# SuwoongHeo/neurecon

Hardware: AMD Instinct MI355X
Metric: rays/sec (4096 rays x 128 samples, 8-layer x256 SDF MLP) (higher is better)
Workload: dtype f16x3

## Files before the change

### include/neurecon_hip.h

```cpp
#ifndef NEURECON_HIP_H
#define NEURECON_HIP_H

#include <stddef.h>
#include <stdint.h>

#ifdef __cplusplus
extern "C" {
#endif

#define NR_OK 0
#define NR_ERR_ARG (-1)
#define NR_ERR_UNSUPPORTED (-2)
#define NR_ERR_HIP (-3)
#define NR_ERR_WORKSPACE (-4)

#define NR_PREC_FP32 0
#define NR_PREC_F16X3 1

#define NR_UPSAMPLE_OFFICIAL 0
#define NR_UPSAMPLE_DIRECT_USE 1
#define NR_UPSAMPLE_DIRECT_MORE 2

int nr_version(void);
const char* nr_last_error(void);
// ... 18 lines not shown
  int D;
  int W;
  int skip;
  int multires;
  int W_geo_feat;
  int precision;
  int siren;
} NrSdfDesc;

size_t nr_sdf_packed_bytes(const NrSdfDesc* d);
int nr_sdf_pack(const NrSdfDesc* d, const float* const* W, const float* const* b, void* packed, void* stream);
size_t nr_mlp_workspace_bytes(int with_backward);
int nr_sdf_forward(const NrSdfDesc* d, const void* packed, const float* pts, int64_t P, float* sdf, float* nabla,
                   float* feature, void* workspace, size_t workspace_bytes, void* stream);

typedef struct {
  int D;
  int W;
  int multires;
  int multires_view;
  int W_geo_feat;
  int precision;
  int no_view_dirs;
  int siren;
} NrRadDesc;

size_t nr_radiance_packed_bytes(const NrRadDesc* d);
int nr_radiance_pack(const NrRadDesc* d, const float* const* W, const float* const* b, void* packed, void* stream);
int nr_radiance_forward(const NrRadDesc* d, const void* packed, const float* x, const float* vdir, int64_t vdir_div,
                        const float* normals, const float* feature, int64_t P, float* rgb, void* stream);

typedef struct {
  const float* rays_o;
  const float* rays_d;
  int64_t n_rays;
  const NrSdfDesc* sdf;
  const void* sdf_packed;
  const NrRadDesc* rad;
  const void* rad_packed;
  float s;
  float obj_bounding_radius;
  float near_bypass;
  float far_bypass;
  int N_samples;
  int N_importance;
  int N_upsample_iters;
  int calc_normal;
  int white_bkgd;
  const float* t_coarse;
  const float* u_fine;
  float* rgb;
  float* depth;
  float* acc;
  float* normals;
  float* d_final;
  float* sdf_out;
  float* nablas_out;
  float* radiance_out;
  float* alpha_out;
  float* cdf_out;
  float* weights_out;
  const NrNerfDesc* nerf;
  const void* nerf_packed;
  int N_outside;
  const float* t_outside;
  float* sigma_out;
  float* radiance_bg_out;
  int upsample_algo;
  float fixed_s;
  int N_nograd_samples;
  const float* t_nograd;
  void* workspace;
  size_t workspace_bytes;
  const float* u_rand;
  const float* t_out_rand;
  const float* s_dev;
  int sample_only;
  float* d_all_out;
  int no_mid_skip;
  int no_defer;
  int64_t max_chunk_rays;
  size_t max_workspace_bytes;
  const void* fold_packed;
} NrNeusArgs;

#define NR_DEFAULT_WORKSPACE_BYTES ((size_t)4 << 30)
#define NR_MIN_CHUNK_RAYS 4096

size_t nr_neus_workspace_bytes(const NrNeusArgs* a);
int nr_neus_render(const NrNeusArgs* a, void* stream);

size_t nr_neus_fold_packed_bytes(const NrSdfDesc* sdf, const NrRadDesc* rad);
int nr_neus_fold_pack(const NrSdfDesc* sdf, const NrRadDesc* rad, const float* W8, const float* b8, const float* W0,
                      const float* b0, void* packed, void* stream);
int nr_neus_fold_forward(const NrSdfDesc* sdf, const void* sdf_packed, const NrRadDesc* rad, const void* rad_packed,
                         const void* fold_packed, const float* pts, const float* vdir, int64_t vdir_div,
                         const float* normals, int64_t P, float* u, float* sdf_out, float* rgb, void* stream);

typedef struct {
  const float* rays_o;
  const float* rays_d;
  int64_t n_rays;
  const NrSdfDesc* sdf;
  const void* sdf_packed;
  const NrRadDesc* rad;
  const void* rad_packed;
  float alpha_net, beta_net;
  float beta_plus_init;
  float eps;
  float near, far;
  float obj_bounding_radius;
  int use_sphere_bg;
  int N_samples, N_importance, max_upsample_steps, max_bisection_steps;
  int calc_normal, white_bkgd;
  const float* t_coarse;
  const float* t_init;
  const float* u_up;
  const float* u_fine;
  float* rgb;
  float* depth;
  float* acc;
  float* normals;
  float* d_vals;
  float* sdf_out;
  float* nablas_out;
  float* radiance_out;
  float* alpha_out;
  float* p_out;
  float* weights_out;
  float* sigma_out;
  float* beta_map;
  float* iter_usage;
  void* workspace;
  size_t workspace_bytes;
  int N_outside;
  const NrNerfDesc* nerf;
  const void* nerf_packed;
  const float* rs_out;
  float beta_plus_k;
  float* sigma_bg;
  float* radiance_bg;
  const float* u_rand;
  const float* u_out;
} NrVolsdfArgs;

size_t nr_volsdf_workspace_bytes(const NrVolsdfArgs* a);
int nr_volsdf_render(const NrVolsdfArgs* a, void* stream);

typedef struct {
  const float* rays_o;
  const float* rays_d;
  int64_t n_rays;
  int64_t rays_per_batch;
  const NrSdfDesc* sdf;
  const void* sdf_packed;
  const NrRadDesc* rad;
  const void* rad_packed;
  float logit_tau;
  float radius_of_interest;
  float interval;
  float too_close_threshold;
  float near_bypass, far_bypass;
  int N_steps, N_secant_steps, N_query, N_freespace;
  int normal_mode;
  int64_t rayschunk, netchunk;
  int calc_normal, white_bkgd;
  const float* t_march;
  const float* t_query;
  const float* t_free;
  float* rgb;
  float* depth;
  float* acc;
  float* normals;
  float* surface_points;
  uint8_t* mask_surface;
  float* depth_surface;
  float* radiance_out;
  float* sdf_out;
  float* nablas_out;
  float* alpha_out;
  float* weights_out;
  void* workspace;
  size_t workspace_bytes;
  const float* u_query;
  const float* u_free;
  int64_t shard_ray0;
  int64_t shard_row_rays;
  double* window_ss;
  int (*window_reduce)(void* user);
  void* window_user;
  int no_secant;
  float* d_all_out;
  int sample_only;
  int full_march;
} NrUnisurfArgs;

size_t nr_unisurf_workspace_bytes(const NrUnisurfArgs* a);
int nr_unisurf_render(const NrUnisurfArgs* a, void* stream);
int64_t nr_unisurf_window_count(const NrUnisurfArgs* a);

int nr_sample_pdf(const float* bins, const float* weights, int64_t R, int L, const float* u, int64_t u_stride, int N,
                  float* out, void* stream);

int nr_get_rays(const float* c2w, const float* K, int B, int H, int W, const int64_t* select_inds, int64_t N,
                float* rays_o, float* rays_d, void* stream);
int nr_gather_rows(const void* src, int64_t B, int64_t HW, int64_t row_bytes, const int64_t* idx, int64_t N, void* out,
                   void* stream);

size_t nr_sphere_trace_workspace_bytes(int64_t n_rays);
int nr_sphere_trace(const NrSdfDesc* d, const void* packed, const float* rays_o, const float* rays_d, int64_t n_rays,
                    float near, float far, const float* near_rays, const float* far_rays, int n_iters, float* d_pred,
                    float* pts, uint8_t* mask, void* workspace, size_t workspace_bytes, void* stream);
size_t nr_root_find_workspace_bytes(int64_t n_rays, int N_steps);
int nr_root_find(const NrSdfDesc* d, const void* packed, const float* rays_o, const float* rays_d, int64_t n_rays,
                 float near, float far, const float* near_rays, const float* far_rays, int N_steps,
                 const float* t_march, int N_secant_steps, int no_secant, float logit_tau, int fill_inf,
                 int full_march, float* d_pred, float* pts, uint8_t* mask, uint8_t* mask_sign_change, void* workspace,
                 size_t workspace_bytes, void* stream);
int nr_normalize3(const float* v, int64_t n, float* out, void* stream);
int nr_surface_finish(float* rgb, const float* nablas, const uint8_t* mask, int64_t n, float* normals, void* stream);

size_t nr_sdf_grid_workspace_bytes(int64_t n_points);
int nr_sdf_grid(const NrSdfDesc* d, const void* packed, double volume_size, int64_t N, int64_t i0, int64_t n,
                float* sdf, void* workspace, size_t workspace_bytes, void* stream);

int nr_mc_table(int8_t* tri, int32_t* counts);
size_t nr_mc_workspace_bytes(int64_t n0, int64_t n1, int64_t n2);
int nr_mc_count(const float* volume, int64_t n0, int64_t n1, int64_t n2, float level, void* workspace,
                size_t workspace_bytes, int64_t* totals, void* stream);
int nr_mc_emit(const float* volume, int64_t n0, int64_t n1, int64_t n2, float level, const double* spacing,
               const double* origin, double scale, const double* offset, void* workspace, size_t workspace_bytes,
               int64_t n_verts, int64_t n_faces, float* verts, int64_t verts_cap, int32_t* faces, int64_t faces_cap,
               void* stream);

size_t nr_mesh_workspace_bytes(int64_t V, int64_t F);
int nr_mesh_components(const int32_t* faces, int64_t F, int64_t V, int32_t* labels, int32_t* face_count,
                       int64_t* totals, void* workspace, size_t workspace_bytes, void* stream);
int nr_mesh_filter_count(const int32_t* faces, int64_t F, int64_t V, const uint8_t* vkeep, void* workspace,
                         size_t workspace_bytes, int64_t* totals, void* stream);
int nr_mesh_filter_emit(const int32_t* faces, int64_t F, int64_t V, const uint8_t* vkeep, void* workspace,
                        size_t workspace_bytes, int64_t Vk, int64_t Fk, int32_t* vsrc, int64_t vsrc_cap,
                        int32_t* faces_out, int64_t faces_cap, void* stream);

int nr_embed(const float* x, int64_t P, int nfreq, float* out, void* stream);
int nr_embed_jvp(const float* x, const float* v, int64_t P, int nfreq, float* out, void* stream);
int nr_embed_padded(const float* x, int64_t P, int nfreq, float* out, int ldo, void* stream);
int nr_embed_jvp_padded(const float* x, const float* v, int64_t P, int nfreq, float* out, int ldo, void* stream);
int nr_embed_vjp(const float* x, const float* e0, int ld0, const float* e1, int ld1, float s1, int64_t P, int nfreq,
                 float* out, void* stream);
int nr_softplus100(const float* z, int64_t n, float* h, float* s, void* stream);
int nr_scale_cols(const float* a, int64_t P, int lda, int col0, int ncols, const float* s, float scale, float* out,
                  void* stream);
int nr_softplus_adjoint(const float* hbar, int ldh, const float* s, const float* g, const float* zdot, int64_t P,
                        int n, float* zbar, void* stream);
size_t nr_colsum_workspace_bytes(int n);
int nr_colsum(const float* a, int64_t P, int n, float* out, void* workspace, size_t workspace_bytes, void* stream);
int nr_sine30(const float* z, int64_t n, float* h, float* s, void* stream);
int nr_sine_adjoint(const float* hbar, int ldh, const float* s, const float* h, const float* g, const float* zdot,
                    int64_t P, int n, float* zbar, void* stream);
int nr_mul(const float* a, const float* b, int64_t n, float* out, void* stream);
int nr_activation(float* y, float* g, int64_t n, int mode, void* stream);
#define NR_WN_MAX 16
typedef struct {
  const float* v;
  const float* g;
  float* w;
  float* norm;
  const float* grad_w;
  float* grad_v;
  float* grad_g;
  int rows;
  int cols;
} NrWnLayer;
int nr_weight_norm_fwd(const NrWnLayer* layers, int n, void* stream);
int nr_weight_norm_bwd(const NrWnLayer* layers, int n, void* stream);
#define NR_ADAM_MAX 64
typedef struct {
// ... 186 lines not shown
```

### neurecon_amd/_lib.py

```python
import ctypes
import os
import threading

import torch

HERE = os.path.dirname(os.path.abspath(__file__))
LIB_PATH = os.environ.get('NR_LIB', os.path.join(HERE, 'libnrhip.so'))

PREC_FP32 = 0
PREC_F16X3 = 1
UPSAMPLE = {'official_solution': 0, 'direct_use': 1, 'direct_more': 2}

_c_p = ctypes.c_void_p
_c_i = ctypes.c_int
_c_i64 = ctypes.c_int64
_c_f = ctypes.c_float
_c_d = ctypes.c_double
_c_sz = ctypes.c_size_t


class NrSdfDesc(ctypes.Structure):
    _fields_ = [('D', _c_i), ('W', _c_i), ('skip', _c_i), ('multires', _c_i), ('W_geo_feat', _c_i),
                ('precision', _c_i), ('siren', _c_i)]


class NrRadDesc(ctypes.Structure):
    _fields_ = [('D', _c_i), ('W', _c_i), ('multires', _c_i), ('multires_view', _c_i), ('W_geo_feat', _c_i),
                ('precision', _c_i), ('no_view_dirs', _c_i), ('siren', _c_i)]


class NrNerfDesc(ctypes.Structure):
    _fields_ = [('D', _c_i), ('W', _c_i), ('skip', _c_i), ('input_ch', _c_i), ('multires', _c_i),
                ('multires_view', _c_i), ('precision', _c_i)]


class NrNeusArgs(ctypes.Structure):
    _fields_ = [
        ('rays_o', _c_p), ('rays_d', _c_p), ('n_rays', _c_i64),
        ('sdf', ctypes.POINTER(NrSdfDesc)), ('sdf_packed', _c_p),
        ('rad', ctypes.POINTER(NrRadDesc)), ('rad_packed', _c_p),
        ('s', _c_f), ('obj_bounding_radius', _c_f), ('near_bypass', _c_f), ('far_bypass', _c_f),
        ('N_samples', _c_i), ('N_importance', _c_i), ('N_upsample_iters', _c_i), ('calc_normal', _c_i),
        ('white_bkgd', _c_i),
        ('t_coarse', _c_p), ('u_fine', _c_p),
        ('rgb', _c_p), ('depth', _c_p), ('acc', _c_p), ('normals', _c_p),
        ('d_final', _c_p), ('sdf_out', _c_p), ('nablas_out', _c_p), ('radiance_out', _c_p),
        ('alpha_out', _c_p), ('cdf_out', _c_p), ('weights_out', _c_p),
        ('nerf', ctypes.POINTER(NrNerfDesc)), ('nerf_packed', _c_p), ('N_outside', _c_i), ('t_outside', _c_p),
        ('sigma_out', _c_p), ('radiance_bg_out', _c_p),
        ('upsample_algo', _c_i), ('fixed_s', _c_f), ('N_nograd_samples', _c_i), ('t_nograd', _c_p),
        ('workspace', _c_p), ('workspace_bytes', _c_sz),
        ('u_rand', _c_p), ('t_out_rand', _c_p), ('s_dev', _c_p), ('sample_only', _c_i), ('d_all_out', _c_p),
        ('no_mid_skip', _c_i), ('no_defer', _c_i), ('max_chunk_rays', _c_i64), ('max_workspace_bytes', _c_sz),
        ('fold_packed', _c_p),
    ]


class NrVolsdfArgs(ctypes.Structure):
    _fields_ = [
        ('rays_o', _c_p), ('rays_d', _c_p), ('n_rays', _c_i64),
        ('sdf', ctypes.POINTER(NrSdfDesc)), ('sdf_packed', _c_p),
        ('rad', ctypes.POINTER(NrRadDesc)), ('rad_packed', _c_p),
        ('alpha_net', _c_f), ('beta_net', _c_f), ('beta_plus_init', _c_f), ('eps', _c_f),
        ('near', _c_f), ('far', _c_f), ('obj_bounding_radius', _c_f), ('use_sphere_bg', _c_i),
        ('N_samples', _c_i), ('N_importance', _c_i), ('max_upsample_steps', _c_i), ('max_bisection_steps', _c_i),
        ('calc_normal', _c_i), ('white_bkgd', _c_i),
        ('t_coarse', _c_p), ('t_init', _c_p), ('u_up', _c_p), ('u_fine', _c_p),
        ('rgb', _c_p), ('depth', _c_p), ('acc', _c_p), ('normals', _c_p),
        ('d_vals', _c_p), ('sdf_out', _c_p), ('nablas_out', _c_p), ('radiance_out', _c_p),
        ('alpha_out', _c_p), ('p_out', _c_p), ('weights_out', _c_p), ('sigma_out', _c_p),
        ('beta_map', _c_p), ('iter_usage', _c_p),
        ('workspace', _c_p), ('workspace_bytes', _c_sz),
        ('N_outside', _c_i), ('nerf', ctypes.POINTER(NrNerfDesc)), ('nerf_packed', _c_p), ('rs_out', _c_p),
        ('beta_plus_k', _c_f), ('sigma_bg', _c_p), ('radiance_bg', _c_p), ('u_rand', _c_p), ('u_out', _c_p),
    ]


class NrUnisurfArgs(ctypes.Structure):
    _fields_ = [
        ('rays_o', _c_p), ('rays_d', _c_p), ('n_rays', _c_i64), ('rays_per_batch', _c_i64),
        ('sdf', ctypes.POINTER(NrSdfDesc)), ('sdf_packed', _c_p),
        ('rad', ctypes.POINTER(NrRadDesc)), ('rad_packed', _c_p),
        ('logit_tau', _c_f), ('radius_of_interest', _c_f), ('interval', _c_f), ('too_close_threshold', _c_f),
        ('near_bypass', _c_f), ('far_bypass', _c_f),
        ('N_steps', _c_i), ('N_secant_steps', _c_i), ('N_query', _c_i), ('N_freespace', _c_i),
        ('normal_mode', _c_i), ('rayschunk', _c_i64), ('netchunk', _c_i64),
        ('calc_normal', _c_i), ('white_bkgd', _c_i),
        ('t_march', _c_p), ('t_query', _c_p), ('t_free', _c_p),
        ('rgb', _c_p), ('depth', _c_p), ('acc', _c_p), ('normals', _c_p),
        ('surface_points', _c_p), ('mask_surface', _c_p), ('depth_surface', _c_p),
        ('radiance_out', _c_p), ('sdf_out', _c_p), ('nablas_out', _c_p), ('alpha_out', _c_p), ('weights_out', _c_p),
        ('workspace', _c_p), ('workspace_bytes', _c_sz),
        ('u_query', _c_p), ('u_free', _c_p),
        ('shard_ray0', _c_i64), ('shard_row_rays', _c_i64), ('window_ss', _c_p), ('window_reduce', _c_p),
        ('window_user', _c_p), ('no_secant', _c_i), ('d_all_out', _c_p), ('sample_only', _c_i),
        ('full_march', _c_i),
    ]


WINDOW_REDUCE = ctypes.CFUNCTYPE(_c_i, _c_p)

TG_NONE, TG_SOFTPLUS, TG_MUL, TG_SPADJ, TG_RELUMASK = 0, 1, 3, 4, 5
BLK_X1, BLK_X2, BLK_Y, BLK_YB, BLK_Y2, BLK_Y3, BLK_A, BLK_G, BLK_ZD = 1, 2, 4, 8, 16, 32, 64, 128, 256
WG_BLK_A0, WG_BLK_A1, WG_BLK_B0, WG_BLK_B1 = 1, 2, 4, 8
WN_MAX = 16
ADAM_MAX = 64


class NrTrainGemm(ctypes.Structure):
    _fields_ = [
        ('op', _c_p), ('P', _c_i64),
        ('x1', _c_p), ('ld1', _c_i64), ('n1', _c_i),
        ('x2', _c_p), ('ld2', _c_i64), ('n2', _c_i),
        ('use_bias', _c_i), ('mode', _c_i), ('yscale', _c_f),
        ('y', _c_p), ('ldy', _c_i64), ('yb', _c_p), ('ldyb', _c_i64),
        ('y2', _c_p), ('ldy2', _c_i64), ('y3', _c_p), ('ldy3', _c_i64),
        ('a', _c_p), ('lda', _c_i64), ('g', _c_p), ('ldg', _c_i64), ('zd', _c_p), ('ldzd', _c_i64),
        ('g_row', _c_i), ('dot', _c_p), ('dot_bias', _c_f),
        ('head', _c_p), ('head_bias', _c_p), ('head_out', _c_p), ('blocked', _c_i),
        ('g_scaled', _c_i),
    ]


class NrWgrad(ctypes.Structure):
    _fields_ = [
        ('P', _c_i64), ('npairs', _c_i), ('a', _c_p * 2), ('lda', _c_i64 * 2), ('b', _c_p * 2), ('ldb', _c_i64 * 2),
        ('m', _c_i), ('n', _c_i), ('scale', _c_f), ('c', _c_p), ('ldc', _c_i64), ('colsum', _c_p),
        ('avec', _c_p), ('ldv', _c_i64), ('vec', _c_p), ('vec_scale', _c_f), ('workspace', _c_p),
        ('workspace_bytes', _c_sz), ('blocked', _c_i), ('fp32', _c_i),
    ]


class NrWnLayer(ctypes.Structure):
    _fields_ = [('v', _c_p), ('g', _c_p), ('w', _c_p), ('norm', _c_p), ('grad_w', _c_p), ('grad_v', _c_p),
                ('grad_g', _c_p), ('rows', _c_i), ('cols', _c_i)]


class NrAdamTensor(ctypes.Structure):
    _fields_ = [('param', _c_p), ('grad', _c_p), ('exp_avg', _c_p), ('exp_avg_sq', _c_p), ('n', _c_i64)]


class NrKernelStat(ctypes.Structure):
    _fields_ = [('name', ctypes.c_char * 32), ('launches', _c_i64), ('ms', ctypes.c_double),
                ('units', ctypes.c_double)]


_SIGS = {
    'nr_version': (_c_i, []),
    'nr_last_error': (ctypes.c_char_p, []),
    'nr_build_id': (ctypes.c_char_p, []),
    'nr_sdf_packed_bytes': (_c_sz, [ctypes.POINTER(NrSdfDesc)]),
    'nr_sdf_pack': (_c_i, [ctypes.POINTER(NrSdfDesc), ctypes.POINTER(_c_p), ctypes.POINTER(_c_p), _c_p, _c_p]),
    'nr_mlp_workspace_bytes': (_c_sz, [_c_i]),
    'nr_sdf_forward': (_c_i, [ctypes.POINTER(NrSdfDesc), _c_p, _c_p, _c_i64, _c_p, _c_p, _c_p, _c_p, _c_sz, _c_p]),
    'nr_radiance_packed_bytes': (_c_sz, [ctypes.POINTER(NrRadDesc)]),
    'nr_radiance_pack': (_c_i, [ctypes.POINTER(NrRadDesc), ctypes.POINTER(_c_p), ctypes.POINTER(_c_p), _c_p, _c_p]),
    'nr_radiance_forward': (_c_i, [ctypes.POINTER(NrRadDesc), _c_p, _c_p, _c_p, _c_i64, _c_p, _c_p, _c_i64, _c_p,
                                   _c_p]),
    'nr_nerf_packed_bytes': (_c_sz, [ctypes.POINTER(NrNerfDesc)]),
    'nr_nerf_pack': (_c_i, [ctypes.POINTER(NrNerfDesc), ctypes.POINTER(_c_p), ctypes.POINTER(_c_p), _c_p, _c_p]),
    'nr_nerf_forward': (_c_i, [ctypes.POINTER(NrNerfDesc), _c_p, _c_p, _c_p, _c_i64, _c_i64, _c_p, _c_p, _c_p]),
    'nr_nerf_train_fwd32': (_c_i, [ctypes.POINTER(NrNerfDesc), _c_p, _c_p, _c_p, _c_i64, ctypes.POINTER(_c_p), _c_p,
                                   _c_p, _c_p, _c_p, _c_p]),
    'nr_nerf_train_packed_bytes': (_c_sz, [ctypes.POINTER(NrNerfDesc)]),
    'nr_weight_norm_fwd': (_c_i, [ctypes.POINTER(NrWnLayer), _c_i, _c_p]),
    'nr_weight_norm_bwd': (_c_i, [ctypes.POINTER(NrWnLayer), _c_i, _c_p]),
    'nr_adam_step': (_c_i, [ctypes.POINTER(NrAdamTensor), _c_i, _c_i64, _c_d, _c_d, _c_d, _c_d, _c_d, _c_p]),
    'nr_nerf_train_pack': (_c_i, [ctypes.POINTER(NrNerfDesc), ctypes.POINTER(_c_p), ctypes.POINTER(_c_p), _c_p, _c_p]),
    'nr_nerf_train_bwd32': (_c_i, [ctypes.POINTER(NrNerfDesc), _c_p, _c_p, _c_p, ctypes.POINTER(_c_p), _c_p, _c_p,
                                   _c_i64, _c_p, _c_p, _c_p, ctypes.POINTER(_c_p), _c_p]),
    'nr_neus_workspace_bytes': (_c_sz, [ctypes.POINTER(NrNeusArgs)]),
    'nr_neus_render': (_c_i, [ctypes.POINTER(NrNeusArgs), _c_p]),
    'nr_neus_fold_packed_bytes': (_c_sz, [ctypes.POINTER(NrSdfDesc), ctypes.POINTER(NrRadDesc)]),
    'nr_neus_fold_pack': (_c_i, [ctypes.POINTER(NrSdfDesc), ctypes.POINTER(NrRadDesc), _c_p, _c_p, _c_p, _c_p, _c_p,
                                 _c_p]),
    'nr_neus_fold_forward': (_c_i, [ctypes.POINTER(NrSdfDesc), _c_p, ctypes.POINTER(NrRadDesc), _c_p, _c_p, _c_p, _c_p,
                                    _c_i64, _c_p, _c_i64, _c_p, _c_p, _c_p, _c_p]),
    'nr_volsdf_workspace_bytes': (_c_sz, [ctypes.POINTER(NrVolsdfArgs)]),
    'nr_volsdf_render': (_c_i, [ctypes.POINTER(NrVolsdfArgs), _c_p]),
    'nr_unisurf_workspace_bytes': (_c_sz, [ctypes.POINTER(NrUnisurfArgs)]),
    'nr_unisurf_render': (_c_i, [ctypes.POINTER(NrUnisurfArgs), _c_p]),
    'nr_unisurf_window_count': (_c_i64, [ctypes.POINTER(NrUnisurfArgs)]),
    'nr_sample_pdf': (_c_i, [_c_p, _c_p, _c_i64, _c_i, _c_p, _c_i64, _c_i, _c_p, _c_p]),
    'nr_get_rays': (_c_i, [_c_p, _c_p, _c_i, _c_i, _c_i, _c_p, _c_i64, _c_p, _c_p, _c_p]),
    'nr_gather_rows': (_c_i, [_c_p, _c_i64, _c_i64, _c_i64, _c_p, _c_i64, _c_p, _c_p]),
    'nr_sphere_trace_workspace_bytes': (_c_sz, [_c_i64]),
    'nr_sphere_trace': (_c_i, [ctypes.POINTER(NrSdfDesc), _c_p, _c_p, _c_p, _c_i64, ctypes.c_float, ctypes.c_float,
                               _c_p, _c_p, _c_i, _c_p, _c_p, _c_p, _c_p, _c_sz, _c_p]),
    'nr_radiance_train_fwd32': (_c_i, [ctypes.POINTER(NrRadDesc), _c_p, _c_p, _c_p, _c_i64, _c_i64, _c_p, _c_p, _c_p,
                                        _c_p, _c_p, _c_p]),
    'nr_root_find_workspace_bytes': (_c_sz, [_c_i64, _c_i]),
    'nr_root_find': (_c_i, [ctypes.POINTER(NrSdfDesc), _c_p, _c_p, _c_p, _c_i64, ctypes.c_float, ctypes.c_float, _c_p,
                            _c_p, _c_i, _c_p, _c_i, _c_i, ctypes.c_float, _c_i, _c_i, _c_p, _c_p, _c_p, _c_p, _c_p,
                            _c_sz, _c_p]),
    'nr_normalize3': (_c_i, [_c_p, _c_i64, _c_p, _c_p]),
    'nr_surface_finish': (_c_i, [_c_p, _c_p, _c_p, _c_i64, _c_p, _c_p]),
    'nr_sdf_grid_workspace_bytes': (_c_sz, [_c_i64]),
    'nr_sdf_grid': (_c_i, [ctypes.POINTER(NrSdfDesc), _c_p, ctypes.c_double, _c_i64, _c_i64, _c_i64, _c_p, _c_p,
                           _c_sz, _c_p]),
    'nr_mc_table': (_c_i, [_c_p, _c_p]),
    'nr_mc_workspace_bytes': (_c_sz, [_c_i64, _c_i64, _c_i64]),
    'nr_mc_count': (_c_i, [_c_p, _c_i64, _c_i64, _c_i64, _c_f, _c_p, _c_sz, _c_p, _c_p]),
    'nr_mc_emit': (_c_i, [_c_p, _c_i64, _c_i64, _c_i64, _c_f, ctypes.POINTER(_c_d), ctypes.POINTER(_c_d), _c_d,
                          ctypes.POINTER(_c_d), _c_p, _c_sz, _c_i64, _c_i64, _c_p, _c_i64, _c_p, _c_i64, _c_p]),
    'nr_mesh_workspace_bytes': (_c_sz, [_c_i64, _c_i64]),
    'nr_mesh_components': (_c_i, [_c_p, _c_i64, _c_i64, _c_p, _c_p, _c_p, _c_p, _c_sz, _c_p]),
    'nr_mesh_filter_count': (_c_i, [_c_p, _c_i64, _c_i64, _c_p, _c_p, _c_sz, _c_p, _c_p]),
    'nr_mesh_filter_emit': (_c_i, [_c_p, _c_i64, _c_i64, _c_p, _c_p, _c_sz, _c_i64, _c_i64, _c_p, _c_i64, _c_p,
                                   _c_i64, _c_p]),
    'nr_embed': (_c_i, [_c_p, _c_i64, _c_i, _c_p, _c_p]),
    'nr_embed_jvp': (_c_i, [_c_p, _c_p, _c_i64, _c_i, _c_p, _c_p]),
    'nr_embed_vjp': (_c_i, [_c_p, _c_p, _c_i, _c_p, _c_i, _c_f, _c_i64, _c_i, _c_p, _c_p]),
    'nr_embed_padded': (_c_i, [_c_p, _c_i64, _c_i, _c_p, _c_i, _c_p]),
    'nr_embed_jvp_padded': (_c_i, [_c_p, _c_p, _c_i64, _c_i, _c_p, _c_i, _c_p]),
    'nr_train_gemm': (_c_i, [ctypes.POINTER(NrTrainGemm), _c_i, _c_i, _c_i, _c_i, _c_p]),
    'nr_sdf_op_info': (_c_i, [ctypes.POINTER(NrSdfDesc), _c_i, ctypes.POINTER(_c_i64), ctypes.POINTER(_c_i),
                              ctypes.POINTER(_c_i)]),
    'nr_sdf_train_packed_bytes': (_c_sz, [ctypes.POINTER(NrSdfDesc)]),
    'nr_sdf_train_pack': (_c_i, [ctypes.POINTER(NrSdfDesc), ctypes.POINTER(_c_p), ctypes.POINTER(_c_p), _c_p, _c_p]),
    'nr_radiance_op_info': (_c_i, [ctypes.POINTER(NrRadDesc), _c_i, ctypes.POINTER(_c_i64), ctypes.POINTER(_c_i),
                                   ctypes.POINTER(_c_i)]),
    'nr_radiance_train_packed_bytes': (_c_sz, [ctypes.POINTER(NrRadDesc)]),
    'nr_radiance_train_pack': (_c_i, [ctypes.POINTER(NrRadDesc), ctypes.POINTER(_c_p), ctypes.POINTER(_c_p), _c_p,
                                      _c_p]),
    'nr_softplus100': (_c_i, [_c_p, _c_i64, _c_p, _c_p, _c_p]),
    'nr_scale_cols': (_c_i, [_c_p, _c_i64, _c_i, _c_i, _c_i, _c_p, _c_f, _c_p, _c_p]),
    'nr_softplus_adjoint': (_c_i, [_c_p, _c_i, _c_p, _c_p, _c_p, _c_i64, _c_i, _c_p, _c_p]),
    'nr_colsum_workspace_bytes': (_c_sz, [_c_i]),
    'nr_colsum': (_c_i, [_c_p, _c_i64, _c_i, _c_p, _c_p, _c_sz, _c_p]),
    'nr_sine30': (_c_i, [_c_p, _c_i64, _c_p, _c_p, _c_p]),
    'nr_sine_adjoint': (_c_i, [_c_p, _c_i, _c_p, _c_p, _c_p, _c_p, _c_i64, _c_i, _c_p, _c_p]),
    'nr_mul': (_c_i, [_c_p, _c_p, _c_i64, _c_p, _c_p]),
    'nr_activation': (_c_i, [_c_p, _c_p, _c_i64, _c_i, _c_p]),
    'nr_radiance_input': (_c_i, [_c_p, _c_p, _c_p, _c_p, _c_i64, _c_i, _c_i, _c_i, _c_p, _c_p]),
    'nr_neus_points': (_c_i, [_c_p, _c_p, _c_p, _c_i64, _c_i, _c_p, _c_p, _c_p, _c_p]),
    'nr_neus_composite_fwd': (_c_i, [_c_p, _c_p, _c_p, _c_p, _c_i64, _c_i, _c_i, _c_p, _c_p, _c_p, _c_p, _c_p, _c_p,
                                     _c_p]),
    'nr_neus_composite_bwd_workspace_bytes': (_c_sz, [_c_i64, _c_i]),
    'nr_neus_composite_bwd': (_c_i, [_c_p, _c_p, _c_p, _c_p, _c_i64, _c_i, _c_i, _c_p, _c_p, _c_p, _c_p, _c_p, _c_p,
                                     _c_p, _c_p, _c_sz, _c_p]),
    'nr_nerf_train_input': (_c_i, [_c_p, _c_p, _c_p, _c_i64, _c_i, _c_i, ctypes.c_float, _c_p, _c_p, _c_p, _c_p]),
    'nr_neus_composite_bg_fwd': (_c_i, [_c_p, _c_p, _c_p, _c_p, _c_p, _c_p, _c_p, _c_i64, _c_i, _c_i, _c_i, _c_p, _c_p,
                                        _c_p, _c_p, _c_p, _c_p, _c_p]),
    'nr_neus_composite_bg_bwd_workspace_bytes': (_c_sz, [_c_i64, _c_i, _c_i]),
    'nr_neus_composite_bg_bwd': (_c_i, [_c_p, _c_p, _c_p, _c_p, _c_p, _c_p, _c_p, _c_i64, _c_i, _c_i, _c_i, _c_p, _c_p,
                                        _c_p, _c_p, _c_p, _c_p, _c_p, _c_p, _c_p, _c_p, _c_sz, _c_p]),
    'nr_unisurf_composite_fwd': (_c_i, [_c_p, _c_p, _c_p, _c_i64, _c_i, _c_i, _c_p, _c_p, _c_p, _c_p, _c_p, _c_p]),
    'nr_unisurf_composite_bwd_workspace_bytes': (_c_sz, [_c_i64, _c_i]),
    'nr_unisurf_composite_bwd': (_c_i, [_c_p, _c_p, _c_p, _c_i64, _c_i, _c_i, _c_p, _c_p, _c_p, _c_p, _c_p, _c_p, _c_p,
                                        _c_sz, _c_p]),
    'nr_volsdf_composite_bg_fwd': (_c_i, [_c_p, _c_p, _c_p, _c_p, _c_p, _c_i64, _c_i, _c_i, _c_f, _c_i, _c_p, _c_p,
                                          _c_p, _c_i, _c_p, _c_p, _c_p, _c_p, _c_p, _c_p, _c_p, _c_p]),
    'nr_volsdf_composite_bg_bwd_workspace_bytes': (_c_sz, [_c_i64, _c_i, _c_i]),
    'nr_volsdf_composite_bg_bwd': (_c_i, [_c_p, _c_p, _c_p, _c_p, _c_p, _c_i64, _c_i, _c_i, _c_f, _c_i, _c_p, _c_p,
                                          _c_p, _c_i, _c_p, _c_p, _c_p, _c_p, _c_p, _c_p, _c_p, _c_p, _c_p, _c_p, _c_p,
                                          _c_sz, _c_p]),
    'nr_volsdf_nerf_input': (_c_i, [_c_p, _c_p, _c_p, _c_p, _c_i64, _c_i, _c_p, _c_p, _c_p]),
    'nr_volsdf_composite_fwd': (_c_i, [_c_p, _c_p, _c_p, _c_p, _c_p, _c_i64, _c_i, _c_i, _c_f, _c_i, _c_p, _c_p, _c_p,
                                       _c_p, _c_p, _c_p, _c_p, _c_p]),
    'nr_volsdf_composite_bwd_workspace_bytes': (_c_sz, [_c_i64, _c_i]),
# ... 96 lines not shown
```

### neurecon_amd/csrc/nr_capi.hip

```cpp
#include <algorithm>
#include <cmath>
#include <cstring>
#include <string>

#include "nr_common.h"
#include <cstdlib>
#include "nr_mlp.h"
#include "nr_tgemm.h"
#include "nr_neus.h"
#include "nr_volsdf.h"
#include "nr_unisurf.h"

namespace nr {

static thread_local std::string g_err;
void set_error(const std::string& msg) { g_err = msg; }

static size_t align256(size_t x) { return (x + 255) & ~(size_t)255; }
static int64_t chunk_bytes_host(int KB) { return (int64_t)(2 * KB + 1) * 1024; }

int check_sdf_desc(const NrSdfDesc* d) {
  NR_REQUIRE(d, NR_ERR_ARG, "null NrSdfDesc");
  if (d->siren) {
    NR_REQUIRE(d->D == 5 && d->W == 256 && d->skip < 0 && d->multires < 0 && d->W_geo_feat == 256,
// ... 11 lines not shown
  return NR_OK;
}

int check_rad_desc(const NrRadDesc* d) {
  NR_REQUIRE(d, NR_ERR_ARG, "null NrRadDesc");
  NR_REQUIRE((d->D == 4 || d->D == 5) && d->W == 256 && d->multires < 0 && d->W_geo_feat == 256 &&
                 d->multires_view <= 7,
             NR_ERR_UNSUPPORTED,
             "radiance net: only D=4 or 5, W=256, embed_multires=-1, embed_multires_view<=7, W_geo_feat=256");
  NR_REQUIRE(d->precision == NR_PREC_FP32 || d->precision == NR_PREC_F16X3, NR_ERR_UNSUPPORTED,
             "radiance net: unknown precision mode");
  return NR_OK;
}


SdfLayout sdf_layout(const NrSdfDesc& d) {
  SdfLayout L{};
  L.prec = d.precision;
  L.siren = d.siren ? 1 : 0;
  const int nops = L.siren ? kSirenOps : kSdfOps;
  const int* KB = L.siren ? kSirenKB : kSdfKB;
  const int* NBO = L.siren ? kSirenNBO : kSdfNBO;
  size_t off = 0;
  for (int i = 0; i < nops; ++i) {
    L.op_bytes[i] = (2 * KB[i] + 1) * 1024;
    L.op_off[i] = (uint32_t)off;
    off += (size_t)(NBO[i] / 2) * L.op_bytes[i];
  }
  static_assert(sdf_op_off(kSdfOps - 1) + (kSdfNBO[kSdfOps - 1] / 2) * (2 * kSdfKB[kSdfOps - 1] + 1) * 1024 > 0, "");
  L.scale_off = (uint32_t)off;
  off = align256(off + kSdfOps * 4);
  L.bound_off = (uint32_t)off;
  off = align256(off + kSdfOps * 8);
  L.w8row0_off = (uint32_t)off;
  off = align256(off + 256 * 4);
  L.misc_off = (uint32_t)off;
  off = align256(off + 16);
  L.total = (uint32_t)off;
  return L;
}

static int rad_small(const NrRadDesc& d) {
  return d.no_view_dirs ? 3 : 3 + (d.multires_view < 0 ? 3 : 3 + 6 * d.multires_view) + 3;
}

RadLayout rad_layout(const NrRadDesc& d) {
  RadLayout L{};
  L.prec = d.precision;
  L.n_small = rad_small(d);
  L.view = d.no_view_dirs ? 0 : 1;
  L.D = d.D;
  L.siren = d.siren ? 1 : 0;
  L.kbs = L.n_small <= 32 ? 2 : 4;
  size_t off = 0;
  for (int i = 0; i < L.D; ++i) {
    const int kb = i == 0 ? 16 + L.kbs : 16;
    L.op_bytes[i] = (2 * kb + 1) * 1024;
    L.op_off[i] = (uint32_t)off;
    off += 8 * (size_t)L.op_bytes[i];
  }
  L.scale_off = (uint32_t)off;
  off = align256(off + 5 * 4);
  L.bound_off = (uint32_t)off;
  off = align256(off + 5 * 2 * 4);
  L.head_off = (uint32_t)off;
  off = align256(off + (3 * 256 + 4) * 4);
  L.total = (uint32_t)off;
  return L;
}

bool fold_applies(const NrSdfDesc& sd, const NrRadDesc& rd) {
  return sd.precision == NR_PREC_F16X3 && !sd.siren && sd.W_geo_feat == 256 && rd.precision == NR_PREC_F16X3 &&
         !rd.siren && rd.D == 4 && rd.W_geo_feat == 256;
}

FoldLayout fold_layout(const RadLayout& RL) {
  FoldLayout F{};
  F.kbs = RL.kbs;
  size_t off = 0;
  F.f8_off = (uint32_t)off;
  off += 8 * (size_t)chunk_bytes_host(16);
  F.r0_off = (uint32_t)off;
  off += 8 * (size_t)chunk_bytes_host(RL.kbs);
  F.scale_off = (uint32_t)off;
  off = align256(off + 2 * 4);
  F.bound_off = (uint32_t)off;
  off = align256(off + 2 * 2 * 4);
  F.u_off = (uint32_t)off;
  off = align256(off + (256 * 256 + 256) * 4);
  F.total = (uint32_t)off;
  return F;
}

int check_nerf_desc(const NrNerfDesc* d) {
  NR_REQUIRE(d, NR_ERR_ARG, "null NrNerfDesc");
  NR_REQUIRE(d->D == 8 && d->W == 256 && d->skip == 4 && d->input_ch == 4 && d->multires == 10 &&
                 d->multires_view == 4,
             NR_ERR_UNSUPPORTED,
             "NeRF net: only the NeRF++ background configuration (D=8, W=256, skips=[4], input_ch=4, "
             "multires=10, multires_view=4, use_view_dirs) is implemented");
  NR_REQUIRE(d->precision == NR_PREC_FP32 || d->precision == NR_PREC_F16X3, NR_ERR_UNSUPPORTED,
             "NeRF net: unknown precision mode");
  return NR_OK;
}

static const int kNerfKB[kNerfOps] = {6, 16, 16, 16, 16, 22, 16, 16, 16, 18};
static const int kNerfNBO[kNerfOps] = {16, 16, 16, 16, 16, 16, 16, 16, 16, 8};

static int nerf_nbo(int i, int prec) { return (i == NF && prec == NR_PREC_F16X3) ? 18 : kNerfNBO[i]; }

NerfLayout nerf_layout(const NrNerfDesc& d) {
  NerfLayout L{};
  L.prec = d.precision;
  size_t off = 0;
  for (int i = 0; i < kNerfOps; ++i) {
    L.op_bytes[i] = (2 * kNerfKB[i] + 1) * 1024;
    L.op_off[i] = (uint32_t)off;
    off += (size_t)(nerf_nbo(i, d.precision) / 2) * L.op_bytes[i];
  }
  L.scale_off = (uint32_t)off;
  off = align256(off + kNerfOps * 4);
  L.bound_off = (uint32_t)off;
  off = align256(off + kNerfOps * 2 * 4);
  L.alpha_off = (uint32_t)off;
  off = align256(off + 257 * 4);
  L.rgb_off = (uint32_t)off;
  off = align256(off + (3 * 128 + 3) * 4);
  L.total = (uint32_t)off;
  return L;
}

static PackSeg seg(int nblk, int off, int nvalid) { return PackSeg{nblk, off, nvalid}; }
static PackOp mkop(const float* W, const float* bias, int rows, int ld, int tr, PackSeg o0, PackSeg o1, PackSeg i0,
                   PackSeg i1, float scale, int prec, float* wmax) {
  PackOp op{};
  op.W = W; op.bias = bias; op.wn = (int64_t)rows * ld; op.ld = ld; op.transpose = tr;
  op.out[0] = o0; op.out[1] = o1; op.in[0] = i0; op.in[1] = i1;
  op.scale = scale; op.prec = prec; op.wmax = wmax;
  return op;
}
static PackSeg none() { return PackSeg{0, 0, 0}; }

static size_t scratch_bytes() {
  int dev = 0, cus = 256;
  if (hipGetDevice(&dev) == hipSuccess) (void)hipDeviceGetAttribute(&cus, hipDeviceAttributeMultiprocessorCount, dev);
  return (size_t)cus * kScratchPerWG;
}

static int neus_chunk(const NrNeusArgs& a, const NeusPlan& pl, int64_t ray0, int R, hipStream_t st) {
  char* ws = (char*)a.workspace;
  const bool direct = a.upsample_algo != NR_UPSAMPLE_OFFICIAL;
  const int n_up = direct ? 0 : (a.N_upsample_iters > 0 ? a.N_importance / a.N_upsample_iters : 0);
  NeusChunk c{};
  c.R = R;
  c.N_samples = a.N_samples;
  c.n_up = n_up;
  c.n_iters = direct ? 0 : a.N_upsample_iters;
  c.S = direct ? a.N_samples + a.N_importance : a.N_samples + a.N_upsample_iters * n_up;
  c.n_imp = a.N_importance;
  c.n_nog = a.upsample_algo == NR_UPSAMPLE_DIRECT_MORE ? a.N_nograd_samples : 0;
  c.fixed_s = a.fixed_s;
  c.t_nog = a.t_nograd;
  auto F = [&](size_t o) { return (float*)(ws + o); };
  c.ro = F(pl.o_ro); c.rd = F(pl.o_rd); c.near = F(pl.o_near); c.far = F(pl.o_far);
  c.dv = F(pl.o_dv); c.sv = F(pl.o_sv); c.wtmp = F(pl.o_wtmp); c.dnew = F(pl.o_dnew); c.snew = F(pl.o_snew);
  c.pts = F(pl.o_pts); c.mids = F(pl.o_mids); c.dmid = F(pl.o_dmid);
  c.sdf_f = F(pl.o_sdf_f); c.nab_f = F(pl.o_nab_f);
  c.sdf_m = F(pl.o_sdf_m); c.nab_m = F(pl.o_nab_m); c.feat_m = F(pl.o_feat_m); c.rad_m = F(pl.o_rad_m);
  c.N_out = a.N_outside;
  c.r_obj = a.obj_bounding_radius;
  c.t_out = a.t_outside;
  c.d_out = F(pl.o_dout); c.x4 = F(pl.o_x4); c.sig_o = F(pl.o_sigo); c.rad_o = F(pl.o_rado);
// ... 41 lines not shown
    if ((rc = launch_sdf(SL, a.sdf_packed, c.pts_nog, (int64_t)c.n_nog * R, c.s_nog, nullptr, nullptr,
                         a.sdf->multires, nullptr, 0, st)))
      return rc;
  }
  if (direct) {
    ProfScope prof("neus_upsample", (double)R, st);
    const float* u = a.u_rand ? a.u_rand + ray0 * a.N_importance : a.u_fine;
    hipLaunchKernelGGL(neus_direct_upsample, grd, blk, 0, st, c, (int)(a.upsample_algo == NR_UPSAMPLE_DIRECT_MORE), u,
                       (int64_t)(a.u_rand ? a.N_importance : 0));
  }
  NR_HIP_CHECK(hipGetLastError());
  float* dvb[2] = {c.dv, F(pl.o_dv2)};
  float* svb[2] = {c.sv, F(pl.o_sv2)};
  int* idb[2] = {c.idv, fused ? (int*)(ws + pl.o_idv2) : nullptr};
  int cur = 0;
  auto merge = [&](int L) -> int {
    ProfScope prof("neus_merge", (double)R, st);
    const int64_t nt = (int64_t)(L + n_up) * R;
    hipLaunchKernelGGL(neus_merge, dim3((unsigned)((nt + 255) / 256)), dim3(256), 0, st, c, L, dvb[cur ^ 1],
                       svb[cur ^ 1], idb[cur ^ 1]);
    cur ^= 1;
    c.dv = dvb[cur];
    c.sv = svb[cur];
    c.idv = idb[cur];
    if (fused) c.sdf_f = c.sv;
    NR_HIP_CHECK(hipGetLastError());
    return NR_OK;
  };
  for (int it = 0; it < c.n_iters; ++it) {
    if (it > 0 && (rc = merge(a.N_samples + (it - 1) * n_up))) return rc;
    const int64_t slot0 = (int64_t)(a.N_samples + it * n_up) * R;
    NeusChunk cu = c;
    if (defer) cu.pts = c.pts + slot0 * 3;
    {
      ProfScope prof("neus_upsample", (double)R, st);
      const float* u = a.u_rand ? a.u_rand + ((int64_t)it * a.n_rays + ray0) * n_up : a.u_fine;
      const size_t lds1 = (5 * (size_t)c.S + 1) * sizeof(float);
      if (4 * lds1 <= 65536)
        hipLaunchKernelGGL((neus_upsample<4>), dim3((unsigned)((R + 3) / 4)), dim3(64), 4 * lds1, st, cu, it, u,
                           (int64_t)(a.u_rand ? n_up : 0));
      else
        hipLaunchKernelGGL((neus_upsample<1>), dim3((unsigned)R), dim3(64), lds1, st, cu, it, u,
                           (int64_t)(a.u_rand ? n_up : 0));
    }
    NR_HIP_CHECK(hipGetLastError());
    if ((rc = sample_sdf(cu.pts, (int64_t)n_up * R, c.snew, slot0))) return rc;
  }
  if (c.n_iters > 0 && (rc = merge(c.S - n_up))) return rc;
  if (defer) {
    const int64_t nslot = (int64_t)c.S * R;
    c.tshift = 0;
    NR_HIP_CHECK(hipMemsetAsync(c.nraw, 0, (size_t)nslot * 3 * sizeof(float), st));
    if (a.calc_normal && a.N_outside == 0) {
      NR_HIP_CHECK(hipMemsetAsync(c.tflag, 0, (size_t)nslot * sizeof(int), st));
      NR_HIP_CHECK(hipMemsetAsync(c.tcnt, 0, sizeof(int), st));
      const int64_t nq = (int64_t)(c.S - 1) * R;
      hipLaunchKernelGGL(neus_sample_need, dim3((unsigned)((nq + 255) / 256)), dim3(256), 0, st, c, a.s_dev, a.s);
      NR_HIP_CHECK(hipGetLastError());
      hipLaunchKernelGGL(neus_point_list, dim3((unsigned)((nslot + 1023) / 1024)), dim3(1024), 0, st, c, nslot);
      NR_HIP_CHECK(hipGetLastError());
      if ((rc = launch_sdf_deferred(SL, a.sdf_packed, c.pts, nslot, nullptr, c.nraw, a.sdf->multires, c.slabs, c.tiles,
                                    c.tcnt, 4, st)))
        return rc;
    }
  }
  if (a.sample_only) {
    hipLaunchKernelGGL(neus_write_dall, dim3((unsigned)(((int64_t)c.S * R + 255) / 256)), dim3(256), 0, st, c.dv,
                       (int64_t)R, c.S, ray0, a.d_all_out);
    NR_HIP_CHECK(hipGetLastError());
    return NR_OK;
  }
  {
    ProfScope prof("neus_points", (double)R, st);
    hipLaunchKernelGGL(neus_expand, dim3((unsigned)(((int64_t)c.S * R + 255) / 256)), dim3(256), 0, st, c,
                       (int)!(defer && a.N_outside > 0));
  }
  NR_HIP_CHECK(hipGetLastError());
  if (!fused && (rc = launch_sdf(SL, a.sdf_packed, c.pts, (int64_t)c.S * R, c.sdf_f, c.nab_f, nullptr,
                                 a.sdf->multires, mlp_ws, mlp_bytes, st)))
    return rc;
  const int64_t Pm = (int64_t)(c.S - 1) * R;
  const char* f8p = nullptr;
  const char* r0p = nullptr;
  if (a.fold_packed) {
    const FoldLayout FL = fold_layout(RL);
    f8p = (const char*)a.fold_packed + FL.f8_off;
    r0p = (const char*)a.fold_packed + FL.r0_off;
  }
  if (a.radiance_out || a.no_mid_skip) {
    if ((rc = launch_sdf(SL, a.sdf_packed, c.mids, Pm, c.sdf_m, c.nab_m, c.feat_m, a.sdf->multires, mlp_ws, mlp_bytes,
                         st, nullptr, 0, f8p)))
      return rc;
    if ((rc = launch_radiance(RL, a.rad_packed, c.mids, c.rd, 1, R, c.nab_m, c.feat_m, Pm, c.rad_m,
                              a.rad->multires_view, st, nullptr, r0p)))
      return rc;
  } else {
    char* wsb = (char*)a.workspace;
    int* cnt = (int*)(wsb + pl.o_mcnt);
    int* slot = (int*)(wsb + pl.o_mslot);
    float* midc = (float*)(wsb + pl.o_midc);
    float* vdc = (float*)(wsb + pl.o_mvd);
    float* radc = (float*)(wsb + pl.o_mrad);
    NR_HIP_CHECK(hipMemsetAsync(cnt, 0, sizeof(int), st));
    const dim3 g1((unsigned)((Pm + 255) / 256));
    hipLaunchKernelGGL(neus_mid_compact, dim3((unsigned)((Pm + 1023) / 1024)), dim3(1024), 0, st, c, a.s_dev, a.s, cnt,
                       slot, midc, vdc);
    NR_HIP_CHECK(hipGetLastError());
    if ((rc = launch_sdf(SL, a.sdf_packed, midc, Pm, c.sdf_m, c.nab_m, c.feat_m, a.sdf->multires, mlp_ws, mlp_bytes,
                         st, cnt, 1, f8p)))
      return rc;
    if ((rc = launch_radiance(RL, a.rad_packed, midc, vdc, 1, INT64_MAX, c.nab_m, c.feat_m, Pm, radc,
                              a.rad->multires_view, st, cnt, r0p)))
      return rc;
    hipLaunchKernelGGL(neus_mid_scatter, g1, dim3(256), 0, st, slot, radc, Pm, c.rad_m);
    NR_HIP_CHECK(hipGetLastError());
  }
  NeusOut o{ray0, a.rgb, a.depth, a.acc, a.normals, a.d_final, a.sdf_out, a.nablas_out,
            a.radiance_out, a.alpha_out, a.cdf_out, a.weights_out, a.sigma_out, a.radiance_bg_out};
  if (a.N_outside > 0) {
    hipLaunchKernelGGL(neus_outside_points, grd, blk, 0, st, c,
                       a.t_out_rand ? a.t_out_rand + ray0 * a.N_outside : (const float*)nullptr);
    NR_HIP_CHECK(hipGetLastError());
    const int64_t Po = (int64_t)(c.S - 1 + a.N_outside) * R;
    if (a.sigma_out || a.radiance_bg_out) {
      if ((rc = launch_nerf(nerf_layout(*a.nerf), a.nerf_packed, c.x4, c.rd, 1, R, Po, c.sig_o, c.rad_o, st)))
        return rc;
    } else {
      char* wsb = (char*)a.workspace;
      int* cnt = (int*)(wsb + pl.o_cnt);
      int* slot = (int*)(wsb + pl.o_slot);
      float* x4c = (float*)(wsb + pl.o_x4c);
      float* vdc = (float*)(wsb + pl.o_vdc);
      float* sigc = (float*)(wsb + pl.o_sigc);
      float* radc = (float*)(wsb + pl.o_radc);
      NR_HIP_CHECK(hipMemsetAsync(cnt, 0, sizeof(int), st));
      const dim3 g1((unsigned)((Po + 255) / 256));
      hipLaunchKernelGGL(neus_outside_compact, dim3((unsigned)((Po + 1023) / 1024)), dim3(1024), 0, st, c, cnt, slot,
                         x4c, vdc);
      NR_HIP_CHECK(hipGetLastError());
      if ((rc = launch_nerf(nerf_layout(*a.nerf), a.nerf_packed, x4c, vdc, 1, INT64_MAX, Po, sigc, radc, st, cnt)))
        return rc;
      hipLaunchKernelGGL(neus_outside_scatter, g1, dim3(256), 0, st, slot, sigc, radc, Po, c.sig_o, c.rad_o);
      NR_HIP_CHECK(hipGetLastError());
    }
    if (defer) {
      const int64_t nslot = (int64_t)c.S * R;
      c.tshift = 0;
      if (a.calc_normal) {
        NR_HIP_CHECK(hipMemsetAsync(c.tflag, 0, (size_t)nslot * sizeof(int), st));
        NR_HIP_CHECK(hipMemsetAsync(c.tcnt, 0, sizeof(int), st));
        hipLaunchKernelGGL(neus_sample_need_outside, dim3((unsigned)((nslot + 255) / 256)), dim3(256), 0, st, c,
                           a.s_dev, a.s);
        NR_HIP_CHECK(hipGetLastError());
        hipLaunchKernelGGL(neus_point_list, dim3((unsigned)((nslot + 1023) / 1024)), dim3(1024), 0, st, c, nslot);
        NR_HIP_CHECK(hipGetLastError());
        if ((rc = launch_sdf_deferred(SL, a.sdf_packed, c.pts, nslot, nullptr, c.nraw, a.sdf->multires, c.slabs,
                                      c.tiles, c.tcnt, 4, st)))
          return rc;
      }
      hipLaunchKernelGGL(neus_gather_nablas, dim3((unsigned)((nslot + 255) / 256)), dim3(256), 0, st, c);
      NR_HIP_CHECK(hipGetLastError());
    }
    ProfScope prof("neus_composite", (double)R, st);
    const int M = c.S - 1 + a.N_outside;
    const size_t lds1 = (6 * (size_t)M + 4 * (size_t)c.S) * sizeof(float);
    if (4 * lds1 <= 65536)
      hipLaunchKernelGGL((neus_composite_outside_w<4>), dim3((unsigned)((R + 3) / 4)), dim3(64), 4 * lds1, st, c, o,
                         a.s_dev, a.s, a.calc_normal, a.white_bkgd);
    else if (lds1 <= 65536)
      hipLaunchKernelGGL((neus_composite_outside_w<1>), dim3((unsigned)R), dim3(64), lds1, st, c, o, a.s_dev, a.s,
                         a.calc_normal, a.white_bkgd);
    else
      hipLaunchKernelGGL(neus_composite_outside, grd, blk, 0, st, c, o, a.s_dev, a.s, a.calc_normal, a.white_bkgd);
  } else {
    ProfScope prof("neus_composite", (double)R, st);
    const size_t lds1 = 9 * (size_t)c.S * sizeof(float);
    if (4 * lds1 <= 65536)
      hipLaunchKernelGGL((neus_composite<4>), dim3((unsigned)((R + 3) / 4)), dim3(64), 4 * lds1, st, c, o, a.s_dev, a.s,
                         a.calc_normal, a.white_bkgd);
    else
      hipLaunchKernelGGL((neus_composite<1>), dim3((unsigned)R), dim3(64), lds1, st, c, o, a.s_dev, a.s, a.calc_normal,
                         a.white_bkgd);
  }
  NR_HIP_CHECK(hipGetLastError());
  return NR_OK;
}

static int64_t neus_chunk_rays(const NrNeusArgs* a) {
  const int64_t n = a->n_rays > 0 ? a->n_rays : 1;
  int64_t cap = 16384;
  if (a->max_chunk_rays > 0)
    cap = std::min(cap, a->max_workspace_bytes ? a->max_chunk_rays : std::max<int64_t>(a->max_chunk_rays, NR_MIN_CHUNK_RAYS));
  const size_t budget = a->max_workspace_bytes ? a->max_workspace_bytes : NR_DEFAULT_WORKSPACE_BYTES;
  const bool defer = neus_deferred(*a, 16);
  NrNeusArgs q = *a;
  const size_t t1 = neus_plan(q, 1024).total, t2 = neus_plan(q, 2048).total;
  const size_t per_ray = (t2 - t1) / 1024 + 1, fixed = t1 > 1024 * per_ray ? t1 - 1024 * per_ray : 0;
  const int64_t fit = budget > fixed ? (int64_t)((budget - fixed) / per_ray) : 0;
  cap = std::min(cap, std::max<int64_t>(fit, 16));
  if (defer && n > 16 && n % 16) cap = std::min(cap, n / 16 * 16);
  if (n <= cap) return n;
  if (defer && cap >= 16) cap = cap / 16 * 16;
  return std::max<int64_t>(cap, 1);
}

static int volsdf_chunk(const NrVolsdfArgs& a, const VolPlan& pl, int64_t ray0, int R, hipStream_t st) {
  char* ws = (char*)a.workspace;
  auto F = [&](size_t o) { return (float*)(ws + o); };
  VolChunk c{};
  c.R = R;
  c.N0 = 4 * a.N_samples;
  c.N_up = 4 * a.N_samples;
  c.cap = c.N0 + a.max_upsample_steps * c.N_up;
  c.N_samples = a.N_samples;
  c.N_imp = a.N_importance;
  c.S = a.N_samples + a.N_importance;
  c.max_iter = a.max_upsample_steps;
  c.max_bisect = a.max_bisection_steps;
  c.alpha_net = a.alpha_net;
  c.beta_net = a.beta_net;
  c.beta_plus0 = a.beta_plus_init;
  c.eps = a.eps;
  c.near = a.near;
  c.far = a.far;
  c.r_bg = a.obj_bounding_radius;
  c.use_bg = a.use_sphere_bg;
  c.ro = F(pl.o_ro); c.rd = F(pl.o_rd);
  c.Ld[0] = F(pl.o_Ld0); c.Ld[1] = F(pl.o_Ld1); c.Ls[0] = F(pl.o_Ls0); c.Ls[1] = F(pl.o_Ls1);
  c.dnew[0] = F(pl.o_dn0); c.dnew[1] = F(pl.o_dn1);
  c.pts = F(pl.o_pts); c.sraw = F(pl.o_sraw);
  c.act[0] = (int*)(ws + pl.o_act0); c.act[1] = (int*)(ws + pl.o_act1); c.cnt = (int*)(ws + pl.o_cnt);
  c.beta = F(pl.o_beta); c.fine = F(pl.o_fine); c.usage = F(pl.o_usage); c.bmap = F(pl.o_bmap);
  c.d_all = F(pl.o_dall); c.pts_f = F(pl.o_ptsf); c.sdf_f = F(pl.o_sdff); c.nab_f = F(pl.o_nabf);
  c.feat_f = F(pl.o_featf); c.rad_f = F(pl.o_radf);
  c.t_coarse = a.t_coarse; c.t_init = a.t_init; c.u_up = a.u_up; c.u_fine = a.u_fine;
  c.N_out = a.N_outside > 0 ? a.N_outside : 0;
  c.u_rand = a.u_rand ? a.u_rand + ray0 * a.N_importance : nullptr;
  c.u_out = a.u_out && c.N_out > 0 ? a.u_out + ray0 * c.N_out : nullptr;
  c.beta_k = a.beta_plus_k;
  c.farr = F(pl.o_farr); c.bp0 = F(pl.o_bp0); c.rs_out = a.rs_out; c.d_out = F(pl.o_dout);
  c.x4 = F(pl.o_x4); c.sig_o = F(pl.o_sigo); c.rad_o = F(pl.o_rado);
  void* mlp_ws = ws + pl.o_mlp;
  const size_t mlp_bytes = a.workspace_bytes - pl.o_mlp;
  const SdfLayout SL = sdf_layout(*a.sdf);
  const RadLayout RL = rad_layout(*a.rad);
  const unsigned lds = (unsigned)pl.lds_bytes;
  const dim3 blk(64), grd((unsigned)R);
  int rc;
  NR_HIP_CHECK(hipMemsetAsync(c.cnt, 0, sizeof(int) * (a.max_upsample_steps + 1), st));
  {
    ProfScope prof("volsdf_prologue", (double)R, st);
    hipLaunchKernelGGL(volsdf_prologue, grd, blk, 0, st, c, a.rays_o + ray0 * 3, a.rays_d + ray0 * 3);
  }
  NR_HIP_CHECK(hipGetLastError());
  if ((rc = launch_sdf(SL, a.sdf_packed, c.pts, (int64_t)c.N0 * R, c.sraw, nullptr, nullptr, a.sdf->multires,
                       nullptr, 0, st)))
    return rc;
  {
    ProfScope prof("volsdf_first", (double)R, st);
    hipLaunchKernelGGL(volsdf_first, grd, blk, lds, st, c);
  }
  NR_HIP_CHECK(hipGetLastError());
  for (int it = 1; it <= a.max_upsample_steps; ++it) {
    if ((rc = launch_sdf(SL, a.sdf_packed, c.pts, (int64_t)c.N_up * R, c.sraw, nullptr, nullptr, a.sdf->multires,
                         nullptr, 0, st, c.cnt + (it - 1), c.N_up)))
      return rc;
    {
      ProfScope prof("volsdf_iter", (double)R, st);
      hipLaunchKernelGGL(volsdf_iter, grd, blk, lds, st, c, it);
    }
    NR_HIP_CHECK(hipGetLastError());
  }
  {
    ProfScope prof("volsdf_points", (double)R, st);
    hipLaunchKernelGGL(volsdf_points, grd, blk, lds, st, c);
  }
  NR_HIP_CHECK(hipGetLastError());
  const int64_t P = (int64_t)c.S * R;
  if ((rc = launch_sdf(SL, a.sdf_packed, c.pts_f, P, c.sdf_f, c.nab_f, c.feat_f, a.sdf->multires, mlp_ws, mlp_bytes,
                       st)))
    return rc;
  if ((rc = launch_radiance(RL, a.rad_packed, c.pts_f, c.rd, c.S, INT64_MAX, c.nab_f, c.feat_f, P, c.rad_f,
                            a.rad->multires_view, st)))
    return rc;
  if (c.N_out > 0) {
    {
      ProfScope prof("volsdf_outside", (double)R, st);
      hipLaunchKernelGGL(volsdf_outside, grd, blk, 0, st, c);
    }
    NR_HIP_CHECK(hipGetLastError());
    if ((rc = launch_nerf(nerf_layout(*a.nerf), a.nerf_packed, c.x4, c.rd, c.N_out, INT64_MAX,
                          (int64_t)c.N_out * R, c.sig_o, c.rad_o, st)))
      return rc;
  }
  VolOut o{ray0, a.rgb, a.depth, a.acc, a.normals, a.d_vals, a.sdf_out, a.nablas_out, a.radiance_out,
           a.alpha_out, a.p_out, a.weights_out, a.sigma_out, a.beta_map, a.iter_usage, a.sigma_bg, a.radiance_bg};
  {
    ProfScope prof("volsdf_composite", (double)R, st);
    hipLaunchKernelGGL(volsdf_composite, grd, blk, lds, st, c, o, a.calc_normal, a.white_bkgd);
  }
  NR_HIP_CHECK(hipGetLastError());
  return NR_OK;
}

static int64_t volsdf_chunk_rays(const NrVolsdfArgs* a) {
  const int64_t cap = 16384;
  return a->n_rays < cap ? (a->n_rays > 0 ? a->n_rays : 1) : cap;
}

static int check_volsdf(const NrVolsdfArgs* a) {
  NR_REQUIRE(a, NR_ERR_ARG, "nr_volsdf_render: null args");
  int rc = check_sdf_desc(a->sdf);
  if (rc) return rc;
  if ((rc = check_rad_desc(a->rad))) return rc;
  NR_REQUIRE(a->n_rays <= 0 || (a->rays_o && a->rays_d && a->rgb && a->depth && a->acc), NR_ERR_ARG,
             "nr_volsdf_render: null ray or output pointer");
  NR_REQUIRE(a->sdf_packed && a->rad_packed && a->t_coarse && a->t_init && a->u_up && a->u_fine, NR_ERR_ARG,
             "nr_volsdf_render: null argument");
  NR_REQUIRE(a->n_rays <= 0 || !a->calc_normal || a->normals, NR_ERR_ARG,
             "nr_volsdf_render: calc_normal needs normals output");
  NR_REQUIRE(a->N_samples >= 1 && a->N_importance >= 1 && a->max_upsample_steps >= 0 && a->max_bisection_steps >= 0,
             NR_ERR_ARG, "nr_volsdf_render: bad sample counts");
  NR_REQUIRE(4 * a->N_samples <= 1024 && a->N_importance <= 1024, NR_ERR_UNSUPPORTED,
             "nr_volsdf_render: 4*N_samples and N_importance must be <= 1024");
  NR_REQUIRE(a->beta_net > 0.f && (a->N_outside > 0 || a->beta_plus_init > 0.f), NR_ERR_ARG,
             "nr_volsdf_render: beta must be positive");
  if (a->N_outside > 0) {
    NR_REQUIRE(!a->use_sphere_bg, NR_ERR_ARG, "nr_volsdf_render: NeRF++ background excludes the builtin sphere");
    NR_REQUIRE(a->nerf && a->nerf_packed && a->rs_out && a->beta_plus_k > 0.f, NR_ERR_ARG,
               "nr_volsdf_render: N_outside > 0 needs nerf, nerf_packed, rs_out and beta_plus_k");
    if ((rc = check_nerf_desc(a->nerf))) return rc;
  }
  return NR_OK;
}

static int unisurf_chunk(const NrUnisurfArgs& a, const UniPlan& pl, int64_t ray0, int R, int64_t row_ray0, int nloc,
                         hipStream_t st) {
  char* ws = (char*)a.workspace;
  auto F = [&](size_t o) { return (float*)(ws + o); };
  UniChunk c{};
  c.R = R;
  c.N_steps = a.N_steps;
  c.N_query = a.N_query;
  c.N_free = a.N_freespace;
  c.P = a.N_query + a.N_freespace;
  c.logit_tau = a.logit_tau;
  c.interval = a.interval;
  c.too_close = a.too_close_threshold;
  c.near_bypass = a.near_bypass;
  c.far_bypass = a.far_bypass;
  c.r_interest = a.radius_of_interest;
  c.ro = F(pl.o_ro); c.rd = F(pl.o_rd); c.near = F(pl.o_near); c.far = F(pl.o_far); c.thr = F(pl.o_thr);
  c.pts_m = F(pl.o_ptsm); c.sm = F(pl.o_sm); c.sec = F(pl.o_sec); c.pts_s = F(pl.o_ptss); c.ss = F(pl.o_ss);
  c.d_all = F(pl.o_dall); c.pts_f = F(pl.o_ptsf); c.sdf_f = F(pl.o_sdff); c.nab_f = F(pl.o_nabf);
  c.feat_f = F(pl.o_featf); c.nrm_f = F(pl.o_nrmf); c.rad_f = F(pl.o_radf); c.wss = (double*)(ws + pl.o_wss);
  c.wsp = (double*)(ws + pl.o_wsp);
  c.netchunk = a.netchunk;
  const bool sharded = a.normal_mode == 1 && a.shard_row_rays > 0;
  if (a.normal_mode == 1) {
    unisurf_windows(a, c.rc_rays, c.nw_full, c.nw_row);
    c.row_rays = sharded ? a.shard_row_rays : (a.rays_per_batch > 0 ? a.rays_per_batch : a.n_rays);
    c.row_ray0 = row_ray0;
    c.nloc = nloc;
    if (sharded) c.wss = a.window_ss;
  }
  c.t_march = a.t_march; c.t_query = a.t_query; c.t_free = a.t_free;
  c.no_secant = a.no_secant;
  c.u_q = a.u_query ? a.u_query + ray0 * a.N_query : nullptr;
  c.u_f = a.u_free ? a.u_free + ray0 * a.N_freespace : nullptr;
  void* mlp_ws = ws + pl.o_mlp;
  const size_t mlp_bytes = a.workspace_bytes - pl.o_mlp;
  const SdfLayout SL = sdf_layout(*a.sdf);
  const RadLayout RL = rad_layout(*a.rad);
  const dim3 blk(64), grd((R + 63) / 64);
  const int64_t P = (int64_t)c.P * R;
  int rc;
  {
    ProfScope prof("unisurf_prologue", (double)R, st);
    hipLaunchKernelGGL(uni_prologue, grd, blk, 0, st, c, a.rays_o + ray0 * 3, a.rays_d + ray0 * 3);
  }
  NR_HIP_CHECK(hipGetLastError());
  if ((rc = run_march(SL, a.sdf_packed, a.sdf->multires, c, a.full_march != 0, (int*)(ws + pl.o_act0),
                      (int*)(ws + pl.o_act1), (int*)(ws + pl.o_acnt), F(pl.o_ptsc), F(pl.o_sc), st)))
    return rc;
  hipLaunchKernelGGL(uni_root, grd, blk, 0, st, c);
  NR_HIP_CHECK(hipGetLastError());
  for (int i = 0; i < (a.no_secant ? 0 : a.N_secant_steps); ++i) {
    if ((rc = launch_sdf(SL, a.sdf_packed, c.pts_s, R, c.ss, nullptr, nullptr, a.sdf->multires, nullptr, 0, st)))
      return rc;
    hipLaunchKernelGGL(uni_secant, grd, blk, 0, st, c, (int)(i == a.N_secant_steps - 1));
    NR_HIP_CHECK(hipGetLastError());
  }
  UniOut o{ray0, a.rgb, a.depth, a.acc, a.normals, a.surface_points, a.mask_surface, a.depth_surface,
           a.radiance_out, a.sdf_out, a.nablas_out, a.alpha_out, a.weights_out};
  hipLaunchKernelGGL(uni_samples, grd, blk, 0, st, c, o);
  NR_HIP_CHECK(hipGetLastError());
  if (a.d_all_out) {
    hipLaunchKernelGGL(neus_write_dall, dim3((unsigned)((P + 255) / 256)), dim3(256), 0, st, c.d_all, (int64_t)R, c.P,
                       ray0, a.d_all_out);
    NR_HIP_CHECK(hipGetLastError());
  }
  if (a.sample_only) return NR_OK;
  if ((rc = launch_sdf(SL, a.sdf_packed, c.pts_f, P, c.sdf_f, c.nab_f, c.feat_f, a.sdf->multires, mlp_ws, mlp_bytes,
                       st)))
    return rc;
  if (a.normal_mode == 1) {
    hipLaunchKernelGGL(uni_window_ss_part, dim3((unsigned)c.nw_row, (unsigned)(R / nloc), kWinSlices), dim3(256), 0,
                       st, c);
    NR_HIP_CHECK(hipGetLastError());
    hipLaunchKernelGGL(uni_window_ss_sum, dim3((unsigned)c.nw_row, (unsigned)(R / nloc)), dim3(64), 0, st, c);
    NR_HIP_CHECK(hipGetLastError());
    if (sharded) {
      const int rr = a.window_reduce(a.window_user);
      NR_REQUIRE(rr == 0, NR_ERR_ARG, "nr_unisurf_render: window_reduce callback failed");
    }
  }
  hipLaunchKernelGGL(uni_normalize, dim3((unsigned)((P + 255) / 256)), dim3(256), 0, st, c, a.normal_mode);
  NR_HIP_CHECK(hipGetLastError());
  if ((rc = launch_radiance(RL, a.rad_packed, c.pts_f, c.rd, 1, R, c.nrm_f, c.feat_f, P, c.rad_f,
                            a.rad->multires_view, st)))
    return rc;
  {
    ProfScope prof("unisurf_composite", (double)R, st);
    hipLaunchKernelGGL(uni_composite, grd, blk, 0, st, c, o, a.calc_normal, a.white_bkgd);
  }
  NR_HIP_CHECK(hipGetLastError());
  return NR_OK;
}

static int check_unisurf(const NrUnisurfArgs* a) {
  NR_REQUIRE(a, NR_ERR_ARG, "nr_unisurf_render: null args");
  int rc = check_sdf_desc(a->sdf);
  if (rc) return rc;
  if ((rc = check_rad_desc(a->rad))) return rc;
  NR_REQUIRE(a->n_rays <= 0 || (a->rays_o && a->rays_d && (a->sample_only ? a->d_all_out != nullptr
                                                                            : (a->rgb && a->depth && a->acc))),
             NR_ERR_ARG, "nr_unisurf_render: null ray or output pointer");
  NR_REQUIRE(!a->sample_only || a->shard_row_rays <= 0, NR_ERR_ARG,
             "nr_unisurf_render: sample_only is not a sharded render");
  NR_REQUIRE(a->sdf_packed && a->rad && (a->rad_packed || a->sample_only) && a->t_march && a->t_query && a->t_free,
             NR_ERR_ARG, "nr_unisurf_render: null argument");
  NR_REQUIRE(a->n_rays <= 0 || a->sample_only || !a->calc_normal || a->normals, NR_ERR_ARG,
             "nr_unisurf_render: calc_normal needs normals output");
  NR_REQUIRE(a->N_steps >= 2 && a->N_secant_steps >= 0 && a->N_query >= 1 && a->N_freespace >= 1, NR_ERR_ARG,
             "nr_unisurf_render: bad sample counts");
  NR_REQUIRE(a->normal_mode == 0 || a->normal_mode == 1, NR_ERR_ARG, "nr_unisurf_render: normal_mode must be 0|1");
  NR_REQUIRE(!a->u_query == !a->u_free, NR_ERR_ARG, "nr_unisurf_render: u_query and u_free go together");
  NR_REQUIRE(a->normal_mode == 0 || (a->rayschunk > 0 && a->netchunk > 0), NR_ERR_ARG,
             "nr_unisurf_render: rayschunk/netchunk must be positive");
  if (a->rays_per_batch > 0)
    NR_REQUIRE(a->n_rays % a->rays_per_batch == 0, NR_ERR_ARG, "nr_unisurf_render: n_rays % rays_per_batch != 0");
  NR_REQUIRE(unisurf_chunk_rays(*a) > 0, NR_ERR_UNSUPPORTED,
             "nr_unisurf_render: rayschunk too large for windowed normalisation unless netchunk % P == 0");
  if (a->shard_row_rays > 0) {
    NR_REQUIRE(a->normal_mode == 1 && a->window_ss && a->window_reduce, NR_ERR_ARG,
               "nr_unisurf_render: a sharded render needs normal_mode 1, window_ss and window_reduce");
    const int64_t nloc = a->rays_per_batch > 0 ? a->rays_per_batch : a->n_rays;
    NR_REQUIRE(a->shard_ray0 >= 0 && a->shard_ray0 + nloc <= a->shard_row_rays, NR_ERR_ARG,
               "nr_unisurf_render: shard outside its batch row");
  }
  return NR_OK;
}

}

using namespace nr;

extern "C" {

int nr_version(void) { return 1; }
#ifndef NR_BUILD_ID
#define NR_BUILD_ID "unknown-source00"
#endif
__attribute__((used)) static const char kBuildIdMarker[] = "NR_BUILD_ID=" NR_BUILD_ID;
const char* nr_build_id(void) { return kBuildIdMarker + 12; }
const char* nr_last_error(void) { return g_err.c_str(); }

size_t nr_sdf_packed_bytes(const NrSdfDesc* d) {
  if (check_sdf_desc(d)) return 0;
  return sdf_layout(*d).total;
}

int nr_sdf_pack(const NrSdfDesc* d, const float* const* W, const float* const* b, void* packed, void* stream) {
  int rc = check_sdf_desc(d);
  if (rc) return rc;
  NR_REQUIRE(W && b && packed, NR_ERR_ARG, "nr_sdf_pack: null argument");
  for (int l = 0; l <= d->D; ++l) NR_REQUIRE(W[l] && b[l], NR_ERR_ARG, "nr_sdf_pack: null layer pointer");
  hipStream_t st = (hipStream_t)stream;
  const SdfLayout L = sdf_layout(*d);
  char* P = (char*)packed;
  if (L.siren) {
    const int prec = d->precision;
    float* wmax = (float*)(P + L.scale_off);
    float* bound = (float*)(P + L.bound_off);
    PackOp ops[kSirenOps];
    ops[S0] = mkop(W[0], b[0], 256, 3, 0, seg(16, 0, 256), none(), seg(4, 0, 3), none(), 1.0f, prec, wmax + S0);
    for (int l = 1; l < 5; ++l)
      ops[S0 + l] = mkop(W[l], b[l], 256, 256, 0, seg(16, 0, 256), none(), seg(16, 0, 256), none(), 1.0f, prec,
                         wmax + S0 + l);
    ops[SF] = mkop(W[5], b[5], 257, 256, 0, seg(16, 1, 256), none(), seg(16, 0, 256), none(), 1.0f, prec, wmax + SF);
    for (int l = 4; l >= 1; --l)
      ops[SB4 + (4 - l)] = mkop(W[l], nullptr, 256, 256, 1, seg(16, 0, 256), none(), seg(16, 0, 256), none(), 1.0f,
                                prec, wmax + SB4 + (4 - l));
    ops[SB0] = mkop(W[0], nullptr, 256, 3, 1, seg(4, 0, 3), none(), seg(16, 0, 256), none(), 1.0f, prec, wmax + SB0);
    char* dst[kSirenOps];
    for (int i = 0; i < kSirenOps; ++i) {
      ops[i].bound = bound + 2 * i;
      dst[i] = P + L.op_off[i];
    }
    if ((rc = launch_pack_ops(ops, dst, kSirenOps, st))) return rc;
    if ((rc = launch_pack_vec(W[5], 0, 256, 256, P + L.w8row0_off, st))) return rc;
    return launch_pack_vec(b[5], 0, 1, 4, P + L.misc_off, st);
  }
  const int in0 = 39, n3 = 217;
  const float isq2 = 1.0f / 1.41421356237309504880f;
  const int prec = d->precision;
  float* wmax = (float*)(P + L.scale_off);
// ... 362 lines not shown
int nr_neus_render(const NrNeusArgs* a, void* stream) {
  NR_REQUIRE(a, NR_ERR_ARG, "nr_neus_render: null args");
  int rc = check_sdf_desc(a->sdf);
  if (rc) return rc;
  if ((rc = check_rad_desc(a->rad))) return rc;
  NR_REQUIRE(a->n_rays <= 0 || (a->rays_o && a->rays_d && (a->sample_only ? a->d_all_out != nullptr
                                                                            : (a->rgb && a->depth && a->acc))),
             NR_ERR_ARG, "nr_neus_render: null ray or output pointer");
  NR_REQUIRE(a->sdf_packed && a->rad && (a->rad_packed || a->sample_only) && a->t_coarse, NR_ERR_ARG,
             "nr_neus_render: null argument");
  NR_REQUIRE(!a->fold_packed || fold_applies(*a->sdf, *a->rad), NR_ERR_ARG,
             "nr_neus_render: a fold pack needs the f16x3 softplus SDF net and a f16x3 ReLU D=4 radiance net");
  NR_REQUIRE(a->N_samples >= 2, NR_ERR_ARG, "nr_neus_render: N_samples must be >= 2");
  NR_REQUIRE(a->n_rays <= 0 || a->sample_only || !a->calc_normal || a->normals, NR_ERR_ARG,
             "nr_neus_render: calc_normal needs normals output");
  NR_REQUIRE(a->N_outside >= 0, NR_ERR_ARG, "nr_neus_render: N_outside must be >= 0");
  if (a->N_outside > 0) {
    if ((rc = check_nerf_desc(a->nerf))) return rc;
    NR_REQUIRE(a->nerf_packed && a->t_outside, NR_ERR_ARG, "nr_neus_render: N_outside > 0 needs the NeRF++ net");
  }
  NR_REQUIRE(a->upsample_algo >= NR_UPSAMPLE_OFFICIAL && a->upsample_algo <= NR_UPSAMPLE_DIRECT_MORE, NR_ERR_ARG,
             "nr_neus_render: unknown upsample_algo");
  if (a->upsample_algo != NR_UPSAMPLE_OFFICIAL) {
    NR_REQUIRE(a->N_importance >= 1 && a->u_fine && a->fixed_s > 0.f, NR_ERR_ARG,
               "nr_neus_render: direct upsampling needs N_importance >= 1, u_fine and fixed_s > 0");
    NR_REQUIRE(a->upsample_algo != NR_UPSAMPLE_DIRECT_MORE || (a->N_nograd_samples >= 2 && a->t_nograd), NR_ERR_ARG,
               "nr_neus_render: direct_more needs N_nograd_samples >= 2 and t_nograd");
  } else if (a->N_upsample_iters > 0) {
    const int n_up = a->N_importance / a->N_upsample_iters;
    NR_REQUIRE(n_up >= 1 && n_up <= kMaxUp && a->u_fine, NR_ERR_UNSUPPORTED,
               "nr_neus_render: N_importance/N_upsample_iters must be in [1, 32]");
  }
  if (a->n_rays <= 0) return NR_OK;
  const int64_t Rc = neus_chunk_rays(a);
  const NeusPlan pl = neus_plan(*a, Rc);
  NR_REQUIRE(a->workspace && a->workspace_bytes >= pl.total, NR_ERR_WORKSPACE, "nr_neus_render: workspace too small");
  {
    const bool direct = a->upsample_algo != NR_UPSAMPLE_OFFICIAL;
    const int S = direct ? a->N_samples + a->N_importance
                         : a->N_samples + a->N_upsample_iters * (a->N_upsample_iters > 0 ? a->N_importance / a->N_upsample_iters : 0);
    int dev = 0, lds_max = 65536;
    NR_HIP_CHECK(hipGetDevice(&dev));
    NR_HIP_CHECK(hipDeviceGetAttribute(&lds_max, hipDeviceAttributeMaxSharedMemoryPerBlock, dev));
    NR_REQUIRE((size_t)9 * S * sizeof(float) <= (size_t)lds_max, NR_ERR_UNSUPPORTED,
               "nr_neus_render: N_samples + N_importance too large for the per-ray LDS staging of the compositing");
  }
  for (int64_t r0 = 0; r0 < a->n_rays; r0 += Rc) {
    const int R = (int)((a->n_rays - r0) < Rc ? (a->n_rays - r0) : Rc);
    if ((rc = neus_chunk(*a, pl, r0, R, (hipStream_t)stream))) return rc;
  }
  return NR_OK;
}

static int check_fold(const NrSdfDesc* sd, const NrRadDesc* rd) {
  int rc = check_sdf_desc(sd);
  if (rc) return rc;
  if ((rc = check_rad_desc(rd))) return rc;
  NR_REQUIRE(fold_applies(*sd, *rd), NR_ERR_UNSUPPORTED,
             "NeuS fold: needs the f16x3 softplus SDF net and a f16x3 ReLU D=4 radiance net");
  return NR_OK;
}

size_t nr_neus_fold_packed_bytes(const NrSdfDesc* sd, const NrRadDesc* rd) {
  if (!sd || !rd || check_sdf_desc(sd) || check_rad_desc(rd) || !fold_applies(*sd, *rd)) return 0;
  return fold_layout(rad_layout(*rd)).total;
}

int nr_neus_fold_pack(const NrSdfDesc* sd, const NrRadDesc* rd, const float* W8, const float* b8, const float* W0,
                      const float* b0, void* packed, void* stream) {
  int rc = check_fold(sd, rd);
  if (rc) return rc;
  NR_REQUIRE(W8 && b8 && W0 && b0 && packed, NR_ERR_ARG, "nr_neus_fold_pack: null argument");
  hipStream_t st = (hipStream_t)stream;
  const RadLayout RL = rad_layout(*rd);
  const FoldLayout F = fold_layout(RL);
  char* P = (char*)packed;
  const int ns = RL.n_small, ld0 = ns + 256;
  float* U = (float*)(P + F.u_off);
  float* bu = U + 256 * 256;
  if ((rc = nr_gemm32(W0 + ns, ld0, W8 + 256, 256, 0, nullptr, U, 256, 256, 256, 256, 0, stream))) return rc;
  if ((rc = nr_gemm32(b8 + 1, 256, W0 + ns, ld0, 1, b0, bu, 256, 1, 256, 256, 0, stream))) return rc;
  float* wmax = (float*)(P + F.scale_off);
  float* bound = (float*)(P + F.bound_off);
  PackOp ops[2];
  ops[0] = mkop(U, bu, 256, 256, 0, seg(16, 0, 256), none(), seg(16, 0, 256), none(), 1.0f, NR_PREC_F16X3, wmax);
  ops[1] = mkop(W0, nullptr, 256, ld0, 0, seg(16, 0, 256), none(), seg(RL.kbs, 0, ns), none(), 1.0f, NR_PREC_F16X3,
                wmax + 1);
  char* dst[2] = {P + F.f8_off, P + F.r0_off};
  for (int i = 0; i < 2; ++i) ops[i].bound = bound + 2 * i;
  return launch_pack_ops(ops, dst, 2, st);
}

int nr_neus_fold_forward(const NrSdfDesc* sd, const void* sdf_packed, const NrRadDesc* rd, const void* rad_packed,
                         const void* fold_packed, const float* pts, const float* vdir, int64_t vdir_div,
                         const float* normals, int64_t P, float* u, float* sdf_out, float* rgb, void* stream) {
  int rc = check_fold(sd, rd);
  if (rc) return rc;
  NR_REQUIRE(sdf_packed && rad_packed && fold_packed && pts && (rd->no_view_dirs || (vdir && normals)) && u &&
                 sdf_out && rgb && vdir_div > 0 && P >= 0,
             NR_ERR_ARG, "nr_neus_fold_forward: bad argument");
  const RadLayout RL = rad_layout(*rd);
  const FoldLayout F = fold_layout(RL);
  const char* fp = (const char*)fold_packed;
  if ((rc = launch_sdf(sdf_layout(*sd), sdf_packed, pts, P, sdf_out, nullptr, u, sd->multires, nullptr, 0,
                       (hipStream_t)stream, nullptr, 0, fp + F.f8_off)))
    return rc;
  return launch_radiance(RL, rad_packed, pts, vdir, vdir_div, INT64_MAX, normals, u, P, rgb, rd->multires_view,
                         (hipStream_t)stream, nullptr, fp + F.r0_off);
}

size_t nr_volsdf_workspace_bytes(const NrVolsdfArgs* a) {
  if (!a || check_volsdf(a)) return 0;
  return volsdf_plan(*a, volsdf_chunk_rays(a)).total;
}

int nr_volsdf_render(const NrVolsdfArgs* a, void* stream) {
  int rc = check_volsdf(a);
  if (rc) return rc;
  if (a->n_rays <= 0) return NR_OK;
  const int64_t Rc = volsdf_chunk_rays(a);
  const VolPlan pl = volsdf_plan(*a, Rc);
  NR_REQUIRE(a->workspace && a->workspace_bytes >= pl.total, NR_ERR_WORKSPACE,
             "nr_volsdf_render: workspace too small");
  int dev = 0, lds_max = 65536;
  NR_HIP_CHECK(hipGetDevice(&dev));
  NR_HIP_CHECK(hipDeviceGetAttribute(&lds_max, hipDeviceAttributeMaxSharedMemoryPerBlock, dev));
  NR_REQUIRE(pl.lds_bytes <= (size_t)lds_max, NR_ERR_UNSUPPORTED,
             "nr_volsdf_render: per-ray sample list does not fit in LDS (reduce N_samples or max_upsample_steps)");
  for (int64_t r0 = 0; r0 < a->n_rays; r0 += Rc) {
    const int R = (int)((a->n_rays - r0) < Rc ? (a->n_rays - r0) : Rc);
    if ((rc = volsdf_chunk(*a, pl, r0, R, (hipStream_t)stream))) return rc;
  }
  return NR_OK;
}

size_t nr_unisurf_workspace_bytes(const NrUnisurfArgs* a) {
  if (!a || check_unisurf(a)) return 0;
  return unisurf_plan(*a, unisurf_chunk_rays(*a)).total;
}

int64_t nr_unisurf_window_count(const NrUnisurfArgs* a) {
  if (!a || a->normal_mode != 1) return 0;
  int64_t rc_rays, nw_full, nw_row;
  unisurf_windows(*a, rc_rays, nw_full, nw_row);
  return nw_row;
}

int nr_unisurf_render(const NrUnisurfArgs* a, void* stream) {
  int rc = check_unisurf(a);
  if (rc) return rc;
  const bool sharded = a->shard_row_rays > 0;
  if (a->n_rays <= 0) {
    if (sharded) NR_REQUIRE(a->window_reduce(a->window_user) == 0, NR_ERR_ARG, "nr_unisurf_render: window_reduce failed");
    return NR_OK;
  }
  const int64_t Rc = unisurf_chunk_rays(*a);
  const UniPlan pl = unisurf_plan(*a, Rc);
  NR_REQUIRE(a->workspace && a->workspace_bytes >= pl.total, NR_ERR_WORKSPACE,
             "nr_unisurf_render: workspace too small");
  if (sharded)
    return unisurf_chunk(*a, pl, 0, (int)a->n_rays, a->shard_ray0,
                         (int)(a->rays_per_batch > 0 ? a->rays_per_batch : a->n_rays), (hipStream_t)stream);
  const int64_t per_b = (a->normal_mode == 1 && a->rays_per_batch > 0) ? a->rays_per_batch : a->n_rays;
  const int64_t span = a->normal_mode == 1 ? (a->rayschunk < per_b ? a->rayschunk : per_b) : per_b;
  for (int64_t b0 = 0; b0 < a->n_rays; b0 += per_b) {
    const int64_t b1 = b0 + per_b < a->n_rays ? b0 + per_b : a->n_rays;
    for (int64_t c0 = b0; c0 < b1; c0 += span) {
      const int64_t c1 = c0 + span < b1 ? c0 + span : b1;
      for (int64_t r0 = c0; r0 < c1; r0 += Rc) {
        const int R = (int)((c1 - r0) < Rc ? (c1 - r0) : Rc);
        if ((rc = unisurf_chunk(*a, pl, r0, R, r0 - b0, R, (hipStream_t)stream))) return rc;
      }
    }
  }
  return NR_OK;
}

int nr_sample_pdf(const float* bins, const float* weights, int64_t R, int L, const float* u, int64_t u_stride, int N,
                  float* out, void* stream) {
  NR_REQUIRE(bins && weights && u && out && L >= 2 && N >= 1 && u_stride >= 0, NR_ERR_ARG,
             "nr_sample_pdf: bad argument");
  if (R <= 0) return NR_OK;
  hipLaunchKernelGGL(sample_pdf_kernel, dim3((unsigned)((R + 255) / 256)), dim3(256), 0, (hipStream_t)stream, bins,
                     weights, R, L, u, u_stride, N, out);
  NR_HIP_CHECK(hipGetLastError());
  return NR_OK;
}

}
```

### neurecon_amd/csrc/nr_mlp.h

```cpp
#pragma once
#include "nr_common.h"

namespace nr {

constexpr int kWaves = 8;
constexpr int kThreads = 64 * kWaves;
constexpr int kTile = 16;
constexpr int kPointsPerWG = kTile * kWaves;
constexpr int kMaxChunkBytes = 48 * 1024;
constexpr size_t kScratchPerWG = (size_t)kWaves * 8 * 16 * 64 * 16;
constexpr int kSlabVB = 12;
constexpr int kSlab24Chunk = 2 * 64 * kSlabVB;
constexpr int kSlab24Layer = 8 * kSlab24Chunk;
constexpr int kSlabColBytes = 7 * kSlab24Layer + 16 * 64 * 16;

enum SdfOp { F0, F1, F2, F3, F4, F5, F6, F7, F8, B7, B6, B5, B4, B3, B2, B1, B0, kSdfOps };

constexpr int kSdfKB[kSdfOps] = {4, 16, 16, 16, 18, 16, 16, 16, 16, 16, 16, 16, 16, 14, 16, 16, 16};
constexpr int kSdfNBO[kSdfOps] = {16, 16, 16, 14, 16, 16, 16, 16, 16, 16, 16, 16, 18, 16, 16, 16, 4};
__host__ __device__ constexpr uint32_t sdf_op_off(int i) {
  uint32_t off = 0;
  for (int k = 0; k < i; ++k) off += (uint32_t)(kSdfNBO[k] / 2) * (2 * kSdfKB[k] + 1) * 1024;
  return off;
}
// ... 5 lines not shown

struct SdfLayout {
  uint32_t op_off[kSdfOps];
  uint32_t op_bytes[kSdfOps];
  uint32_t scale_off;
  uint32_t bound_off;
  uint32_t w8row0_off;
  uint32_t misc_off;
  uint32_t total;
  int prec;
  int siren;
};

struct RadLayout {
  uint32_t op_off[5];
  uint32_t op_bytes[5];
  uint32_t head_off;
  uint32_t scale_off;
  uint32_t bound_off;
  uint32_t total;
  int prec;
  int kbs;
  int n_small;
  int view;
  int D;
  int siren;
};

enum NerfOp { N0, N1, N2, N3, N4, N5, N6, N7, NF, NV, kNerfOps };

struct NerfLayout {
  uint32_t op_off[kNerfOps];
  uint32_t op_bytes[kNerfOps];
  uint32_t scale_off;
  uint32_t bound_off;
  uint32_t alpha_off;
  uint32_t rgb_off;
  uint32_t total;
  int prec;
};

enum NerfBwdOp { NBV, NBF, NB7, NB6, NB5, NB4, NB3, NB2, NB1, kNerfBwdOps };

struct NerfBwdLayout {
  uint32_t op_off[kNerfBwdOps];
  uint32_t op_bytes[kNerfBwdOps];
  uint32_t scale_off;
  uint32_t wr_off;
  uint32_t wa_off;
  uint32_t total;
};

struct PackSeg {
  int nblk;
  int off;
  int nvalid;
};

struct PackOp {
  const float* W;
  const float* bias;
  int64_t wn;
  int ld;
  int transpose;
  PackSeg out[2];
  PackSeg in[2];
  float scale;
  int prec;
  float* wmax;
  const float* aux;
  float* bound;
  const float* W2;
  const float* bias2;
  int64_t wn2;
  int ld2;
};

int launch_pack_op(const PackOp& op, char* dst, hipStream_t stream);
int launch_pack_ops(const PackOp* ops, char* const* dst, int nops, hipStream_t stream);
int launch_pack_vec(const float* src, int off, int nvalid, int n, char* dst, hipStream_t stream);
int launch_sdf(const SdfLayout& L, const void* packed, const float* pts, int64_t P, float* sdf, float* nabla,
               float* feature, int nfreq, void* ws, size_t ws_bytes, hipStream_t stream,
               const int* P_dev = nullptr, int P_mult = 0,
               const void* f8_alt = nullptr);
int launch_sdf_deferred(const SdfLayout& L, const void* packed, const float* pts, int64_t P, float* sdf, float* nabla,
                        int nfreq, float4* slabs, const int* tiles, const int* n_tiles, int stage, hipStream_t stream);
int launch_nerf(const NerfLayout& L, const void* packed, const float* x4, const float* vdir, int64_t vdiv,
                int64_t vmod, int64_t P, float* sigma, float* rgb, hipStream_t stream,
                const int* P_dev = nullptr);
int launch_radiance(const RadLayout& L, const void* packed, const float* x, const float* vdir, int64_t vdiv,
                    int64_t vmod, const float* normals, const float* feature, int64_t P, float* rgb, int nfreq_view,
                    hipStream_t stream, const int* P_dev = nullptr,
                    const void* r0_fold = nullptr);

struct FoldLayout {
  uint32_t f8_off, r0_off;
  uint32_t scale_off;
  uint32_t bound_off;
  uint32_t u_off;
  uint32_t total;
  int kbs;
};
FoldLayout fold_layout(const RadLayout& RL);
bool fold_applies(const NrSdfDesc& sd, const NrRadDesc& rd);

int launch_radiance_train32(const RadLayout& L, const void* packed, const float* feat, const float* small,
                            int64_t ld_small, int n_small, int64_t P, float* const* h, float* rgb, hipStream_t stream);
int launch_nerf_train32_fwd(const NerfLayout& L, const void* packed, const float* xe, const float* ve, int64_t P,
                            float* const* h, float* feat, float* hv, float* sigma, float* rgb, hipStream_t stream);
int launch_nerf_train32_bwd(const NerfBwdLayout& B, const void* packed, const float* rgb, const float* hv,
                            const float* const* h, const float* g_rgb, const float* g_sigma, int64_t P, float* g3,
                            float* ghv, float* g_feat, float* const* gz, hipStream_t stream,
                            bool f16x3 = false);
SdfLayout sdf_layout(const NrSdfDesc& d);
RadLayout rad_layout(const NrRadDesc& d);
int check_sdf_desc(const NrSdfDesc* d);
int check_rad_desc(const NrRadDesc* d);

}
```

### neurecon_amd/csrc/nr_mlp.hip

```cpp
#include <algorithm>
#include <type_traits>
#include "nr_common.h"
#include "nr_mlp.h"
#include "nr_tgemm.h"

namespace nr {

using lds_ptr = __attribute__((address_space(3))) void*;

__device__ __forceinline__ void glds16(const char* gsrc, uint32_t lds_addr) {
  unsigned keep;
  asm volatile(
      "s_mov_b32 %0, m0\n\t"
      "s_mov_b32 m0, %2\n\t"
      "s_nop 0\n\t"
      "global_load_lds_dwordx4 %1, off\n\t"
      "s_mov_b32 m0, %0"
      : "=&s"(keep)
      : "v"(gsrc), "s"(lds_addr)
      : "memory");
}

__device__ __forceinline__ void glds16s(const char* sbase, uint32_t voff, uint32_t lds_addr) {
  unsigned keep;
// ... 635 lines not shown
  return __builtin_ldexpf(1.0f, 14 - __builtin_amdgcn_frexp_expf(M));
}
template <bool DERIV>
__device__ __forceinline__ void softplus3(float z, float& y, float& s) {
  const float t = z * 100.0f;
  const bool lin = t > 20.0f;
  const float ex = __builtin_amdgcn_exp2f(t * 1.44269504088896341f);
  const float u = 1.0f + ex;
  const float yy = __builtin_amdgcn_logf(u) * (0.693147180559945309f * 0.01f);
  y = lin ? z : yy;
  if constexpr (DERIV) s = lin ? 1.0f : ex * __builtin_amdgcn_rcpf(u);
}
__device__ __forceinline__ void softplus1(float z, float& y, float& s) {
  const float t = z * 144.269504088896341f;
  const float ex = __builtin_amdgcn_exp2f(t);
  const float u = ex + 1.0f;
  const bool lin = t > 28.8539008f;
  y = lin ? z : __builtin_amdgcn_logf(u) * (0.693147180559945309f * 0.01f);
  s = lin ? 1.0f : ex * __builtin_amdgcn_rcpf(u);
}
template <bool DERIV>
__device__ __forceinline__ void softplus_pk(float z0, float z1, float& y0, float& y1, float& s0, float& s1) {
  float d0, d1;
  softplus1(z0, y0, d0);
  softplus1(z1, y1, d1);
  if constexpr (DERIV) {
    s0 = d0;
    s1 = d1;
  }
}
__device__ __forceinline__ float4 fma4s(f32x4 a, float m, float4 b) {
  return make_float4(__builtin_fmaf(a[0], m, b.x), __builtin_fmaf(a[1], m, b.y), __builtin_fmaf(a[2], m, b.z),
                     __builtin_fmaf(a[3], m, b.w));
}

using gf4 = __attribute__((address_space(1))) f32x4;

constexpr int kNC = 1;
constexpr int kW4 = 8 / kNC;
constexpr int kT4 = 64 * kW4;
constexpr int kWPE = kW4 / 4;
constexpr int kSlabW = 2 * kNC * 1024;
constexpr int kSlab4 = kW4 * kSlabW;
constexpr int kLoad = 8;
static_assert(kLoad >= 1 && kLoad <= kW4, "loader waves");

typedef uint32_t u32x3 __attribute__((ext_vector_type(3)));
struct Pend4 {
  float4* base;
  uint32_t o[4];
  float4 v[4];
  int n;
  bool nt;
  bool b96;
  __device__ __forceinline__ int flush() {
    int issued = 0;
    if (base) {
      issued = n;
#pragma unroll
      for (int i = 0; i < 4; ++i) {
        if (i < n) {
          if (b96) {
            const uint32_t off = o[i];
            const u32x3 d = {__float_as_uint(v[i].x), __float_as_uint(v[i].y), __float_as_uint(v[i].z)};
            if (nt) asm volatile("global_store_dwordx3 %0, %1, %2 nt\n\ts_nop 1" : : "v"(off), "v"(d), "s"(base) : "memory");
            else asm volatile("global_store_dwordx3 %0, %1, %2\n\ts_nop 1" : : "v"(off), "v"(d), "s"(base) : "memory");
          } else {
            const uint32_t off = o[i] * 16u;
            const f32x4 d = tof(v[i]);
            if (nt) asm volatile("global_store_dwordx4 %0, %1, %2 nt\n\ts_nop 1" : : "v"(off), "v"(d), "s"(base) : "memory");
            else asm volatile("global_store_dwordx4 %0, %1, %2\n\ts_nop 1" : : "v"(off), "v"(d), "s"(base) : "memory");
          }
        }
      }
      base = nullptr;
    }
    return issued;
  }
  __device__ __forceinline__ void put(float4* b, int cnt, bool nontemporal, bool bytes96 = false) {
    base = b;
    n = cnt;
    nt = nontemporal;
    b96 = bytes96;
  }
};

constexpr int kSlabRing = 3;
constexpr int kFwdRing = 4;
constexpr bool kSlabNT = true;
constexpr bool kFeatNT = false;

template <int CBMAX, int RING = 3, int NW = kW4>
struct WStream4 {
  static_assert(RING == 3 || RING == 4, "weight ring depth");
  static constexpr int kRingN = RING;
  static constexpr int kLd = NW == kW4 ? kLoad : NW;
  char* lds;
  char* slab;
  int cur;
  int es;
  int er;
  int prev;
  __device__ __forceinline__ static int wave_id() { return __builtin_amdgcn_readfirstlane(threadIdx.x >> 6); }
  __device__ __forceinline__ static int next3(int i) { return i == 2 ? 0 : i + 1; }
  __device__ __forceinline__ static int nextr(int i) { return i == RING - 1 ? 0 : i + 1; }
  __device__ __forceinline__ int ahead_slot() const { return cur == 0 ? RING - 1 : cur - 1; }
  template <int BYTES>
  __device__ __forceinline__ static constexpr int pieces() { return (BYTES / 1024 + kLd - 1) / kLd; }
  __device__ __forceinline__ static int loader() { return wave_id() - (NW - kLd); }
  template <int BYTES>
  __device__ __forceinline__ static int npieces() { return loader() >= 0 ? pieces<BYTES>() : 0; }
  template <int BYTES>
  __device__ __forceinline__ void dma(const char* gsrc, int slot) {
    constexpr int NB = BYTES / 1024, NPW = pieces<BYTES>();
    const int wave = loader();
    if (wave < 0) return;
    const uint32_t voff = (threadIdx.x & 63) * 16;
    const int first = __builtin_amdgcn_readfirstlane(min(wave * NPW, NB - NPW));
    const char* g = uniform_ptr(gsrc) + first * 1024;
    const uint32_t base =
        __builtin_amdgcn_readfirstlane(lds_u32(lds) + (uint32_t)(slot * CBMAX) + (uint32_t)(first * 1024));
#pragma unroll
    for (int j = 0; j < NPW; j += 4) {
      const char* gj = g + j * 1024;
      const uint32_t mj = base + j * 1024;
      if (NPW - j >= 4)
        asm volatile(
            "s_mov_b32 m0, %2\n\ts_nop 0\n\t"
            "global_load_lds_dwordx4 %0, %1\n\t"
            "global_load_lds_dwordx4 %0, %1 offset:1024\n\t"
            "global_load_lds_dwordx4 %0, %1 offset:2048\n\t"
            "global_load_lds_dwordx4 %0, %1 offset:3072"
            :
            : "v"(voff), "s"(gj), "s"(mj)
            : "memory", "m0");
      else if (NPW - j == 3)
        asm volatile(
            "s_mov_b32 m0, %2\n\ts_nop 0\n\t"
            "global_load_lds_dwordx4 %0, %1\n\t"
            "global_load_lds_dwordx4 %0, %1 offset:1024\n\t"
            "global_load_lds_dwordx4 %0, %1 offset:2048"
            :
            : "v"(voff), "s"(gj), "s"(mj)
            : "memory", "m0");
      else if (NPW - j == 2)
        asm volatile(
            "s_mov_b32 m0, %2\n\ts_nop 0\n\t"
            "global_load_lds_dwordx4 %0, %1\n\t"
            "global_load_lds_dwordx4 %0, %1 offset:1024"
            :
            : "v"(voff), "s"(gj), "s"(mj)
            : "memory", "m0");
      else
        glds16m(gj, voff, mj);
    }
  }
  template <int B0, int B1>
  __device__ __forceinline__ void start(const char* g0, const char* g1) {
    static_assert(RING == 3, "start: the first RING - 1 chunks");
    cur = 0;
    es = 0;
    er = 0;
    prev = 0;
    dma<B0>(g0, 0);
    dma<B1>(g1, 1);
    wait_vmcnt(npieces<B1>());
// ... 38 lines not shown
    uint32_t off = er * kSlab4 + wave_id() * kSlabW;
    asm volatile("" : "+s"(off));
    return (const float4*)(slab + off);
  }
  __device__ __forceinline__ void slab_consumed() { er = next3(er); }
  __device__ __forceinline__ const float4* buf() const {
    uint32_t off = cur * CBMAX;
    asm volatile("" : "+s"(off));
    return (const float4*)(lds + off);
  }
  __device__ __forceinline__ void flip(int n) {
    if constexpr (RING == 4) {
      wait_vmcnt(n + prev);
      prev = n;
    } else {
      wait_vmcnt(n);
    }
    __syncthreads();
    cur = nextr(cur);
  }
  __device__ __forceinline__ void flip_nowait() {
    __syncthreads();
    cur = nextr(cur);
  }
};

__device__ __forceinline__ f16x8 rd_frag(const float4* __restrict__ A, int i, int lane) {
  return as_h8(A[i * 64 + lane]);
}
template <int NS, class Stage>
__device__ __forceinline__ void mma4(const float4* __restrict__ A, const f16x8 (&bh)[kNC][12],
                                     const f16x8 (&bl)[kNC][12], f32x4 (&acc)[kNC][2], int lane, Stage&& stage) {
  f16x8 nh0 = rd_frag(A, 0, lane), nl0 = rd_frag(A, 1, lane);
  f16x8 nh1 = rd_frag(A, NS * 2, lane), nl1 = rd_frag(A, NS * 2 + 1, lane);
#pragma unroll
  for (int s = 0; s < NS; ++s) {
    const f16x8 h0 = nh0, l0 = nl0, h1 = nh1, l1 = nl1;
    if (s + 1 < NS) {
      nh0 = rd_frag(A, (s + 1) * 2, lane);
      nl0 = rd_frag(A, (s + 1) * 2 + 1, lane);
      nh1 = rd_frag(A, (NS + s + 1) * 2, lane);
      nl1 = rd_frag(A, (NS + s + 1) * 2 + 1, lane);
    }
    stage(s);
#pragma unroll
    for (int q = 0; q < kNC; ++q) {
      acc[q][0] = mfma16h(l0, bh[q][s], acc[q][0]);
      acc[q][1] = mfma16h(l1, bh[q][s], acc[q][1]);
      acc[q][0] = mfma16h(h0, bl[q][s], acc[q][0]);
      acc[q][1] = mfma16h(h1, bl[q][s], acc[q][1]);
      acc[q][0] = mfma16h(h0, bh[q][s], acc[q][0]);
      acc[q][1] = mfma16h(h1, bh[q][s], acc[q][1]);
    }
    if (s + 1 < NS) __builtin_amdgcn_sched_group_barrier(0x100, 4, 0);
    __builtin_amdgcn_sched_group_barrier(0x008, 6 * kNC, 0);
    __builtin_amdgcn_sched_barrier(0);
  }
}

struct Z4 {
  float4 z[kNC][2];
  float4 aux[2];
};

constexpr float kT = 144.26944f;
constexpr float kC = 0.0069314749f;

#ifdef NR_EXP_STAMPS
constexpr int kStampPh = 6;
__device__ unsigned long long g_nr_stamps[2048 * 8 * kStampPh];
__device__ __forceinline__ unsigned long long* stamp_lds() {
  __shared__ unsigned long long s_stamp[kW4 * kStampPh];
  return s_stamp;
}
__device__ __forceinline__ uint64_t stamp_now() { return __builtin_amdgcn_s_memtime(); }
__device__ __forceinline__ void stamp_add(int ph, uint64_t dt) {
  if ((threadIdx.x & 63) == 0) stamp_lds()[(threadIdx.x >> 6) * kStampPh + ph] += dt;
}
#define NR_STAMP(var) const uint64_t var = stamp_now()
#else
#define NR_STAMP(var)
#endif

template <int KB, int NBO, int NXT_CB, bool AUX, bool TS, class WS, class Pre, class Epi>
__device__ __forceinline__ void op4(WS& ws, const char* __restrict__ op, const char* nxt, const f16x8 (&bh)[kNC][12],
                                    const f16x8 (&bl)[kNC][12], const float (&xinv)[kNC], Pend4& pd, Pre&& pre,
                                    Epi&& epi, int lane) {
  constexpr int CB = chunk_bytes(KB);
  constexpr int NCH = NBO / 2;
  constexpr int LA = WS::kRingN - 1;
  static_assert(NCH >= 2, "the 2-ahead stream needs >= 2 chunks per op");
  const int g = lane >> 4;
  Z4 zq{};
#pragma unroll
  for (int c = 0; c < NCH; ++c) {
    const char* opc = op;
    const char* nxc = nxt;
    asm volatile("" : "+s"(opc), "+s"(nxc));
    NR_STAMP(t0);
    int npend = 0;
    if (c + LA < NCH) {
      ws.template issue<CB>(opc + (c + LA) * CB);
      npend = WS::template npieces<CB>();
    } else if (nxc) {
      ws.template issue<NXT_CB>(nxc + (c + LA - NCH) * NXT_CB);
      npend = WS::template npieces<NXT_CB>();
    }
    npend += pre(c);
    npend += pd.flush();
    NR_STAMP(t1);
    const float4* A = ws.buf();
    f32x4 acc[kNC][2] = {};
    mma4<KB / 2>(A, bh, bl, acc, lane, [&](int st) {
      if (c > 0) {
#pragma unroll
        for (int e = 0; e < 8; ++e)
          if (e * (KB / 2) / 8 == st) epi(c - 1, zq, e);
      }
    });
    NR_STAMP(t2);
    float wi = A[2 * KB * 64 + 8].x;
    if constexpr (TS) wi *= kT;
    const float4 b0 = A[2 * KB * 64 + (TS ? 24 : 0) + g], b1 = A[2 * KB * 64 + (TS ? 28 : 4) + g];
#pragma unroll
    for (int q = 0; q < kNC; ++q) {
      const float inv = xinv[q] * wi;
      zq.z[q][0] = fma4s(acc[q][0], inv, b0);
      zq.z[q][1] = fma4s(acc[q][1], inv, b1);
    }
    if constexpr (AUX) {
      zq.aux[0] = A[2 * KB * 64 + 16 + g];
      zq.aux[1] = A[2 * KB * 64 + 20 + g];
    }
#ifdef NR_EXP_STAMPS
    wait_vmcnt(npend);
    NR_STAMP(t3);
    ws.flip(npend);
    NR_STAMP(t4);
    stamp_add(0, t1 - t0);
    stamp_add(1, t2 - t1);
    stamp_add(2, t3 - t2);
    stamp_add(3, t4 - t3);
    stamp_add(4, 1);
#else
    ws.flip(npend);
#endif
  }
  pd.flush();
#pragma unroll
  for (int e = 0; e < 8; ++e) epi(NCH - 1, zq, e);
}

template <bool NABLA>
__device__ __forceinline__ void sp_pair(const Z4& zz, int q, int k, float4 (&y)[2], float4& s0, float4& s1) {
  const int o = k >> 1;
  const float4 z = zz.z[q][o];
  float4& s = o ? s1 : s0;
  if ((k & 1) == 0) softplus_pk<NABLA>(z.x, z.y, y[o].x, y[o].y, s.x, s.y);
  else softplus_pk<NABLA>(z.z, z.w, y[o].z, y[o].w, s.z, s.w);
}
__device__ __forceinline__ float4 mul4(float4 a, float4 b) { return make_float4(a.x * b.x, a.y * b.y, a.z * b.z, a.w * b.w); }
__device__ __forceinline__ uint32_t opaque_lane(int lane) {
  uint32_t l = (uint32_t)lane;
  asm volatile("" : "+v"(l));
  return l;
}
__device__ __forceinline__ void pend_chunk(Pend4& pd, float4* base, int first_blk, int lane, bool nt) {
  const uint32_t l = opaque_lane(lane);
#pragma unroll
// ... 14 lines not shown
}
__device__ __forceinline__ float4 unpack24_mul(uint32_t w0, uint32_t w1, uint32_t w2, float4 g) {
  const float u0 = (float)(w0 & 0xFFFFFFu);
  const float u1 = (float)(__builtin_amdgcn_alignbit(w1, w0, 24) & 0xFFFFFFu);
  const float u2 = (float)(__builtin_amdgcn_alignbit(w2, w1, 16) & 0xFFFFFFu);
  const float u3 = (float)(w2 >> 8);
  constexpr float k = 1.0f / 8388608.0f;
  return make_float4(__builtin_fmaf(-(g.x * k), u0, g.x), __builtin_fmaf(-(g.y * k), u1, g.y),
                     __builtin_fmaf(-(g.z * k), u2, g.z), __builtin_fmaf(-(g.w * k), u3, g.w));
}


template <bool NABLA>
struct FwdEpi4 {
  static constexpr int NV = 8 * kNC;
  f16x8 (&oh)[kNC][12];
  f16x8 (&ol)[kNC][12];
  const float (&sc)[kNC];
  float4* sl;
  float (&mrun)[kNC];
  Pend4& pd;
  int lane;
  float e[NV], L[NV], m[NV];
  __device__ __forceinline__ static float zval(const Z4& zz, int i) {
    const float4 v = zz.z[i >> 3][(i >> 2) & 1];
    const int r = i & 3;
    return r == 0 ? v.x : (r == 1 ? v.y : (r == 2 ? v.z : v.w));
  }
  __device__ __forceinline__ void operator()(int c, const Z4& zz, int st) {
    if (st == 0) {
#pragma unroll
      for (int i = 0; i < NV; ++i) e[i] = fminf(zval(zz, i), 126.0f);
    } else if (st == 1) {
#pragma unroll
      for (int i = 0; i < NV; ++i) e[i] = __builtin_amdgcn_exp2f(e[i]);
    } else if (st == 2) {
#pragma unroll
      for (int i = 0; i < NV; ++i) e[i] = e[i] + 1.0f;
#pragma unroll
      for (int i = 0; i < NV / 2; ++i) L[i] = __builtin_amdgcn_logf(e[i]);
    } else if (st == 3) {
#pragma unroll
      for (int i = NV / 2; i < NV; ++i) L[i] = __builtin_amdgcn_logf(e[i]);
      if constexpr (NABLA) {
#pragma unroll
        for (int i = 0; i < NV / 2; ++i) e[i] = __builtin_amdgcn_rcpf(e[i]);
      }
    } else if (st == 4) {
#pragma unroll
      for (int i = 0; i < NV; ++i) m[i] = fmaxf(L[i], zval(zz, i));
      if constexpr (NABLA) {
#pragma unroll
        for (int i = NV / 2; i < NV; ++i) e[i] = __builtin_amdgcn_rcpf(e[i]);
      }
    } else if (st == 5) {
#pragma unroll
      for (int q = 0; q < kNC; ++q) {
        const int i = 8 * q;
        float r = mrun[q];
        r = __builtin_fmaxf(r, __builtin_fmaxf(m[i + 0], m[i + 1]));
        r = __builtin_fmaxf(r, __builtin_fmaxf(m[i + 2], m[i + 3]));
        r = __builtin_fmaxf(r, __builtin_fmaxf(m[i + 4], m[i + 5]));
        r = __builtin_fmaxf(r, __builtin_fmaxf(m[i + 6], m[i + 7]));
        mrun[q] = r;
      }
      if constexpr (NABLA) {
#pragma unroll
        for (int q = 0; q < kNC; ++q)
#pragma unroll
          for (int o = 0; o < 2; ++o) {
            const int i = (2 * q + o) * 4;
            pd.v[kNC * o + q] = pack24(e[i], e[i + 1], e[i + 2], e[i + 3]);
          }
      }
    } else if (st == 6) {
      split8a(make_float4(m[0], m[1], m[2], m[3]), make_float4(m[4], m[5], m[6], m[7]), sc[0] * kC, oh[0][c],
              ol[0][c]);
    } else {
      if constexpr (NABLA) pend_chunk24(pd, sl, c, lane, kSlabNT);
    }
  }
};

template <bool NABLA, bool FEAT>
struct F7Epi4 {
  f16x8 (&oh)[kNC][12];
  f16x8 (&ol)[kNC][12];
  const float (&sc)[kNC];
  float4* g7;
  float (&mrun)[kNC];
  float (&sdf_part)[kNC];
  Pend4& pd;
  int lane;
  float4 y[kNC][2], s[kNC][2];
  __device__ __forceinline__ void operator()(int c, const Z4& zz, int st) {
    const int q = st >> 2, k = st & 3;
    if (q < kNC) sp_pair<NABLA>(zz, q, k, y[q], s[q][0], s[q][1]);
    if (q < kNC && k == 3) {
      const float4 w0 = zz.aux[0], w1 = zz.aux[1];
      float sp = sdf_part[q];
      sp = fmaf(y[q][0].x, w0.x, sp); sp = fmaf(y[q][0].y, w0.y, sp);
      sp = fmaf(y[q][0].z, w0.z, sp); sp = fmaf(y[q][0].w, w0.w, sp);
      sp = fmaf(y[q][1].x, w1.x, sp); sp = fmaf(y[q][1].y, w1.y, sp);
      sp = fmaf(y[q][1].z, w1.z, sp); sp = fmaf(y[q][1].w, w1.w, sp);
      sdf_part[q] = sp;
      if constexpr (NABLA) {
        pd.v[q] = mul4(w0, s[q][0]);
        pd.v[kNC + q] = mul4(w1, s[q][1]);
      }
      if constexpr (FEAT) {
        mrun[q] = amax8(mrun[q], y[q][0], y[q][1]);
        split8a(y[q][0], y[q][1], sc[q], oh[q][c], ol[q][c]);
      }
    }
    if constexpr (NABLA)
      if (st == 7) pend_chunk(pd, g7, 2 * c, lane, kFeatNT);
  }
};

template <int NMAIN, class WS>
struct BwdEpi4 {
  f16x8 (&oh)[kNC][12];
  f16x8 (&ol)[kNC][12];
  const float (&sc)[kNC];
  WS& ws;
  float4* park;
  int park_blk;
  float (&mrun)[kNC];
  Pend4& pd;
  int lane;
  int plane;
  float4 y[kNC][2];
  __device__ __forceinline__ void operator()(int c, const Z4& zz, int st) {
    if (2 * c < NMAIN) {
      const int q = st >> 2, k = st & 3;
      if (q >= kNC) return;
      if (k < 2) {
        const uint4 sw = *(const uint4*)((const char*)ws.slab_read() + ((kNC * k + q) * 64 + lane) * 16);
        y[q][k] = unpack24_mul(sw.x, sw.y, sw.z, zz.z[q][k]);
      } else if (k == 2) {
        mrun[q] = amax8(mrun[q], y[q][0], y[q][1]);
      } else {
        split8a(y[q][0], y[q][1], sc[q], oh[q][c], ol[q][c]);
        if (q == kNC - 1) ws.slab_consumed();
      }
    } else if (st == 7) {
#pragma unroll
      for (int q = 0; q < kNC; ++q) {
        pd.v[q] = zz.z[q][0];
        pd.v[kNC + q] = zz.z[q][1];
      }
      pend_chunk(pd, park, park_blk + 2 * c - NMAIN, plane, false);
    }
  }
};

struct NoPre4 {
  __device__ __forceinline__ int operator()(int) const { return 0; }
};

template <bool NABLA, bool FEAT, int STAGE_>
__global__ __attribute__((amdgpu_flat_work_group_size(STAGE_ == 3 ? 256 : kT4, STAGE_ == 3 ? 256 : kT4),
                          amdgpu_waves_per_eu(kWPE, kWPE)))
void sdf4_kernel(SdfKArgs a) {
  constexpr int STAGE = STAGE_ == 3 ? 0 : (STAGE_ == 4 ? 2 : STAGE_);
  constexpr bool COMPACT = STAGE_ == 4;
  constexpr int NW = STAGE_ == 3 ? 4 : kW4;
  static_assert(STAGE_ != 3 || (!NABLA && !FEAT), "narrow tiles: forward-only launches");
  static_assert(STAGE == 0 || (NABLA && !FEAT), "deferred nablas: no feature");
  constexpr int PPW = 16 * kNC * NW;
  constexpr int CB = chunk_bytes(18);
  constexpr int C16 = chunk_bytes(16), C4 = chunk_bytes(4), C14 = chunk_bytes(14), C18 = chunk_bytes(18);
  static_assert((size_t)kW4 * kNC * kSlabColBytes <= kScratchPerWG, "per-workgroup slab scratch");
  constexpr bool SLABS = NABLA && STAGE != 1;
  constexpr int RING = SLABS ? 3 : kFwdRing;
  __shared__ __attribute__((aligned(16))) char smem[RING * CB + (SLABS ? kSlabRing * kSlab4 : 0)];
  static_assert(RING * CB + (SLABS ? kSlabRing * kSlab4 : 0) <= 160 * 1024, "LDS budget");
  WStream4<CB, RING, NW> ws{smem, SLABS ? smem + RING * CB : nullptr, 0, 0, 0, 0};
  const int lane = threadIdx.x & 63, wave = __builtin_amdgcn_readfirstlane(threadIdx.x >> 6);
  const int j = lane & 15, g = lane >> 4;
  const char* W = a.packed;
  auto OP = [&](int i) {
    const char* w = W;
    asm volatile("" : "+s"(w));
    return w + sdf_op_off(i);
  };
  auto OPF8 = [&]() {
    const char* w = a.f8_alt;
    asm volatile("" : "+s"(w));
    return w ? w : OP(F8);
  };
  const float b8 = *(const float*)(W + a.L.misc_off);
  float4* escr = uniform_ptr((float4*)((char*)a.scratch + (size_t)(blockIdx.x * kW4 + wave) * (kNC * kSlabColBytes)));
  auto slab = [&](int l) {
    char* e = (char*)escr;
    asm volatile("" : "+s"(e));
    return (float4*)(e + l * kNC * kSlab24Layer);
  };

#ifdef NR_EXP_STAMPS
  if ((threadIdx.x & 63) == 0)
    for (int i = 0; i < kStampPh; ++i) stamp_lds()[wave * kStampPh + i] = 0;
#endif
  if constexpr (STAGE == 2) ws.template start<C16, C16>(OP(B7), OP(B7) + C16);
  else if constexpr (RING == 4) ws.template start<C4, C4, C4>(OP(F0), OP(F0) + C4, OP(F0) + 2 * C4);
  else ws.template start<C4, C4>(OP(F0), OP(F0) + C4);
  Pend4 pd{};
  NoPre4 nopre;
  const float kSpSlack = 0.0070f;

  const int64_t Pn = COMPACT      ? ((int64_t)(*a.n_tiles) + 15) / 16 * 16
                     : STAGE == 2 ? (int64_t)(*a.n_tiles) * kPointsPerWG / kW4
                                  : (a.P_dev ? min(a.P, (int64_t)(*a.P_dev) * a.P_mult) : a.P);
  for (int64_t base = (int64_t)blockIdx.x * PPW; base < Pn; base += (int64_t)gridDim.x * PPW) {
    const bool has_next = base + (int64_t)gridDim.x * PPW < Pn;
    int64_t p0 = base + wave * 16 * kNC;
    int plane = lane;
    uint32_t soff = 0;
    int64_t pl = 0;
    bool listed = true;
    if constexpr (COMPACT) {
      const int64_t n = *a.n_tiles;
      const int64_t w0 = p0 < n ? p0 : n - 16;
      const int e = a.tiles[w0 + j];
      const int e0 = __builtin_amdgcn_readfirstlane(a.tiles[w0]);
      listed = p0 < n && e >= 0;
      pl = e >= 0 ? e : e0;
      const uint32_t rt = (uint32_t)((pl >> 4) - (e0 >> 4)), js = (uint32_t)(pl & 15);
      plane = (int)(rt * (uint32_t)(kSlabColBytes / 16) + js + 16u * (uint32_t)g);
      soff = rt * (uint32_t)kSlabColBytes + (js + 16u * (uint32_t)g) * (uint32_t)kSlabVB;
      escr = uniform_ptr((float4*)((char*)a.slabs + (size_t)(e0 >> 4) * kSlabColBytes));
    } else if constexpr (STAGE == 2) {
      const int64_t ti = min(p0 / 16, (int64_t)(*a.n_tiles) - 1);
      const int64_t tile = a.tiles[ti];
      escr = uniform_ptr((float4*)((char*)a.slabs + (size_t)tile * kSlabColBytes));
      p0 = p0 / 16 < (int64_t)(*a.n_tiles) ? tile * 16 : a.P;
    } else if constexpr (STAGE == 1) {
      escr = uniform_ptr((float4*)((char*)a.slabs + (size_t)(p0 / 16) * kSlabColBytes));
    }
    const int64_t Pv = STAGE == 2 ? a.P : Pn;
    int64_t pq[kNC];
    bool valid[kNC];
    float xs[kNC][3];
#pragma unroll
    for (int q = 0; q < kNC; ++q) {
      const int64_t p = p0 + 16 * q + j;
      if constexpr (COMPACT) {
        valid[q] = listed;
        pq[q] = pl;
      } else {
        valid[q] = p < Pv;
        pq[q] = valid[q] ? p : Pv - 1;
      }
      xs[q][0] = a.pts[pq[q] * 3 + 0];
      xs[q][1] = a.pts[pq[q] * 3 + 1];
      xs[q][2] = a.pts[pq[q] * 3 + 2];
    }
    float4 E[kNC][4];
    float mE[kNC], xinv[kNC];
    f16x8 Uh[kNC][12], Ul[kNC][12], Vh[kNC][12], Vl[kNC][12];
    float mrun[kNC], m_in[kNC];
    auto next_scales = [&](int kb, float extra, const float (&floor_max)[kNC], float (&sc)[kNC]) {
      const float4 v = ws.buf()[2 * kb * 64 + 8];
#pragma unroll
      for (int q = 0; q < kNC; ++q) sc[q] = bound_scale(fmaxf(fmaf(v.y, m_in[q], v.z) + extra, floor_max[q]));
    };
    auto finish = [&](const float (&sc)[kNC], float mscale = 1.0f) {
#pragma unroll
      for (int q = 0; q < kNC; ++q) {
        m_in[q] = max4_groups(mrun[q]) * mscale;
        mrun[q] = 0.0f;
        xinv[q] = 1.0f / sc[q];
      }
    };
    float zero2[kNC];
#pragma unroll
    for (int q = 0; q < kNC; ++q) zero2[q] = 0.0f;
    if constexpr (STAGE != 2) {
#pragma unroll
    for (int q = 0; q < kNC; ++q) {
#pragma unroll
      for (int b = 0; b < 4; ++b) {
        const int f = 16 * b + 4 * g;
        E[q][b] = make_float4(embed_feature(f + 0, xs[q][0], xs[q][1], xs[q][2], a.nfreq),
                              embed_feature(f + 1, xs[q][0], xs[q][1], xs[q][2], a.nfreq),
                              embed_feature(f + 2, xs[q][0], xs[q][1], xs[q][2], a.nfreq),
                              embed_feature(f + 3, xs[q][0], xs[q][1], xs[q][2], a.nfreq));
      }
      mE[q] = max4_groups(amax8(amax8(0.0f, E[q][0], E[q][1]), E[q][2], E[q][3]));
      const float sE = bound_scale(mE[q]);
// ... 3 lines not shown
    }
    float4* epark = slab(7);
    if constexpr (NABLA) {
      const uint32_t l = opaque_lane(lane);
#pragma unroll
      for (int q = 0; q < kNC; ++q)
#pragma unroll
        for (int b = 0; b < 4; ++b) {
          const uint32_t off = (((12 + b) * kNC + q) * 64 + l) * 16u;
          const f32x4 d = tof(E[q][b]);
          asm volatile("global_store_dwordx4 %0, %1, %2\n\ts_nop 1" : : "v"(off), "v"(d), "s"(epark) : "memory");
        }
    }
#pragma unroll
    for (int q = 0; q < kNC; ++q) {
      mrun[q] = 0.0f;
      m_in[q] = mE[q];
    }
    auto fwd_epi = [&](f16x8(&oh)[kNC][12], f16x8(&ol)[kNC][12], const float (&sc)[kNC], float4* sl) {
      return FwdEpi4<NABLA>{oh, ol, sc, sl, mrun, pd, lane};
    };

    {
      float sc[kNC];
      next_scales(4, kSpSlack, zero2, sc);
      op4<4, 16, C16, false, true>(ws, OP(F0), OP(F1), Uh, Ul, xinv, pd, nopre, fwd_epi(Vh, Vl, sc, slab(0)), lane);
      finish(sc, kC);
    }
    {
      float sc[kNC];
      next_scales(16, kSpSlack, zero2, sc);
      op4<16, 16, C16, false, true>(ws, OP(F1), OP(F2), Vh, Vl, xinv, pd, nopre, fwd_epi(Uh, Ul, sc, slab(1)), lane);
      finish(sc, kC);
    }
    {
      float sc[kNC];
      next_scales(16, kSpSlack, zero2, sc);
      op4<16, 16, C16, false, true>(ws, OP(F2), OP(F3), Uh, Ul, xinv, pd, nopre, fwd_epi(Vh, Vl, sc, slab(2)), lane);
      finish(sc, kC);
    }
    {
      float sc[kNC];
      next_scales(16, kSpSlack, mE, sc);
      op4<16, 14, C18, false, true>(ws, OP(F3), OP(F4), Vh, Vl, xinv, pd, nopre, fwd_epi(Uh, Ul, sc, slab(3)), lane);
      if constexpr (NABLA) {
        asm volatile("s_waitcnt vmcnt(0)" ::: "memory");
#pragma unroll
        for (int q = 0; q < kNC; ++q)
#pragma unroll
          for (int b = 0; b < 4; ++b) E[q][b] = fromf(*((const gf4*)epark + ((12 + b) * kNC + q) * 64 + lane));
      }
#pragma unroll
      for (int q = 0; q < kNC; ++q) {
        split8a(E[q][0], E[q][1], sc[q], Uh[q][7], Ul[q][7]);
        split8a(E[q][2], E[q][3], sc[q], Uh[q][8], Ul[q][8]);
        mrun[q] = fmaxf(mrun[q], mE[q] * (1.0f / kC));
      }
      finish(sc, kC);
    }
    {
      float sc[kNC];
      next_scales(18, kSpSlack, zero2, sc);
      op4<18, 16, C16, false, true>(ws, OP(F4), OP(F5), Uh, Ul, xinv, pd, nopre, fwd_epi(Vh, Vl, sc, slab(4)), lane);
      finish(sc, kC);
    }
    {
      float sc[kNC];
      next_scales(16, kSpSlack, zero2, sc);
      op4<16, 16, C16, false, true>(ws, OP(F5), OP(F6), Vh, Vl, xinv, pd, nopre, fwd_epi(Uh, Ul, sc, slab(5)), lane);
      finish(sc, kC);
    }
    {
      float sc[kNC];
      next_scales(16, kSpSlack, zero2, sc);
      op4<16, 16, C16, false, true>(ws, OP(F6), OP(F7), Uh, Ul, xinv, pd, nopre, fwd_epi(Vh, Vl, sc, slab(6)), lane);
      finish(sc, kC);
    }
    float sdf_part[kNC];
#pragma unroll
    for (int q = 0; q < kNC; ++q) sdf_part[q] = 0.0f;
    {
      float sc[kNC];
      next_scales(16, kSpSlack, zero2, sc);
      F7Epi4<NABLA, FEAT> epi{Uh, Ul, sc, slab(7), mrun, sdf_part, pd, lane};
      constexpr int NXT = ((NABLA && STAGE == 0) || FEAT) ? C16 : C4;
      const char* n;
      if constexpr (FEAT) n = OPF8();
      else n = (NABLA && STAGE == 0) ? OP(B7) : (has_next ? OP(F0) : nullptr);
      op4<16, 16, NXT, true, false>(ws, OP(F7), n, Vh, Vl, xinv, pd, nopre, epi, lane);
      finish(sc);
    }
#pragma unroll
    for (int q = 0; q < kNC; ++q) {
      const float sdf = wave_sum4(sdf_part[q]) + b8;
      if (valid[q] && g == 0) a.sdf[p0 + 16 * q + j] = sdf;
    }
    if constexpr (FEAT) {
      const int64_t pf = p0 < Pn ? p0 : Pn - 1;
      float4* fb = uniform_ptr((float4*)(a.feature + pf * 256));
      uint32_t frow[kNC];
#pragma unroll
      for (int q = 0; q < kNC; ++q) frow[q] = (uint32_t)(pq[q] - pf);
      auto epi = [&](int c, const Z4& zz, int st) {
        if (st != 7) return;
#pragma unroll
        for (int q = 0; q < kNC; ++q) {
          pd.v[2 * q] = zz.z[q][0];
          pd.v[2 * q + 1] = zz.z[q][1];
          const uint32_t r = opaque_lane(frow[q] * 64 + g);
          pd.o[2 * q] = r + (2 * c) * 4;
          pd.o[2 * q + 1] = r + (2 * c + 1) * 4;
        }
        pd.put(fb, 2 * kNC, kFeatNT);
      };
      constexpr int NXT = NABLA ? C16 : C4;
      const char* n = NABLA ? OP(B7) : (has_next ? OP(F0) : nullptr);
      op4<16, 16, NXT, false, false>(ws, OPF8(), n, Uh, Ul, xinv, pd, nopre, epi, lane);
    }
    }
    if constexpr (NABLA && STAGE == 1) {
      pd.flush();
    }
    if constexpr (NABLA && STAGE != 1) {
      pd.flush();
      asm volatile("s_waitcnt vmcnt(0)" ::: "memory");
      float4* g7 = slab(7);
#pragma unroll
      for (int q = 0; q < kNC; ++q) {
        float4 G[16];
#pragma unroll
        for (int b = 0; b < 16; ++b) G[b] = fromf(*((const gf4*)g7 + (kNC * b + q) * 64 + (COMPACT ? plane : lane)));
        float m = 0.0f;
#pragma unroll
        for (int b = 0; b < 16; b += 2) m = amax8(m, G[b], G[b + 1]);
        m_in[q] = max4_groups(m);
        mrun[q] = 0.0f;
        const float sc = bound_scale(m_in[q]);
#pragma unroll
        for (int s = 0; s < 8; ++s) split8a(G[2 * s], G[2 * s + 1], sc, Uh[q][s], Ul[q][s]);
        xinv[q] = 1.0f / sc;
      }
      float4* park = slab(7);
      if constexpr (COMPACT) ws.stage_slab(slab(6), 0, soff);
      else ws.stage_slab(slab(6), 0);
      auto bwd = [&](auto kb_tag, auto nbo_tag, auto nmain_tag, auto nxt_tag, int opi, const char* nxt,
                     f16x8(&ih)[kNC][12], f16x8(&il)[kNC][12], f16x8(&oh)[kNC][12], f16x8(&ol)[kNC][12], int lcur,
                     int park_blk, int lnext) {
        constexpr int KBo = decltype(kb_tag)::value, NBOo = decltype(nbo_tag)::value;
        constexpr int NMAIN = decltype(nmain_tag)::value, NXC = decltype(nxt_tag)::value;
        float sc[kNC];
        next_scales(KBo, 0.0f, zero2, sc);
        auto pre = [&](int c) -> int {
          if constexpr (COMPACT) {
            if (2 * (c + 1) < NMAIN) return ws.stage_slab(slab(lcur), c + 1, soff);
            if (c + 1 == NBOo / 2 && lnext >= 0) return ws.stage_slab(slab(lnext), 0, soff);
          } else {
            if (2 * (c + 1) < NMAIN) return ws.stage_slab(slab(lcur), c + 1);
            if (c + 1 == NBOo / 2 && lnext >= 0) return ws.stage_slab(slab(lnext), 0);
          }
          return 0;
        };
        BwdEpi4<NMAIN, decltype(ws)> epi{oh, ol, sc, ws, park, park_blk, mrun, pd, lane, COMPACT ? plane : lane};
        op4<KBo, NBOo, NXC, false, false>(ws, OP(opi), nxt, ih, il, xinv, pd, pre, epi, lane);
        finish(sc);
      };
      using I0 = std::integral_constant<int, 0>;
      using I4 = std::integral_constant<int, 4>;
// ... 338 lines not shown
    const int q = st >> 2, k = st & 3;
    if (q >= kNC) return;
    if (k < 2) {
      const float4 z = zz.z[q][k];
      y[q][k] = make_float4(fmaxf(z.x, 0.0f), fmaxf(z.y, 0.0f), fmaxf(z.z, 0.0f), fmaxf(z.w, 0.0f));
    } else if (k == 2) {
      mrun[q] = amax8(mrun[q], y[q][0], y[q][1]);
    } else {
      split8a(y[q][0], y[q][1], sc[q], oh[q][c], ol[q][c]);
    }
  }
};

struct HeadEpi4 {
  const float* head;
  float (&part)[kNC][3];
  int g;
  float4 y[kNC][2];
  __device__ __forceinline__ void operator()(int c, const Z4& zz, int st) {
    const int q = st >> 2, k = st & 3;
    if (q >= kNC) return;
    if (k < 2) {
      const float4 z = zz.z[q][k];
      y[q][k] = make_float4(fmaxf(z.x, 0.0f), fmaxf(z.y, 0.0f), fmaxf(z.z, 0.0f), fmaxf(z.w, 0.0f));
    } else {
#pragma unroll
      for (int o = 0; o < 3; ++o) {
        if ((o == 0) != (k == 2)) continue;
        float p = part[q][o];
        const uint32_t lo = opaque_lane(4 * g);
#pragma unroll
        for (int b = 0; b < 2; ++b) {
          const float4 w = *(const float4*)(head + lo + o * 256 + 16 * (2 * c + b));
          p = fmaf(y[q][b].x, w.x, p);
          p = fmaf(y[q][b].y, w.y, p);
          p = fmaf(y[q][b].z, w.z, p);
          p = fmaf(y[q][b].w, w.w, p);
        }
        asm volatile("" : "+v"(p));
        part[q][o] = p;
      }
    }
  }
};

struct FoldEpi4 {
  f16x8 (&oh)[kNC][12];
  f16x8 (&ol)[kNC][12];
  const float (&sc)[kNC];
  float (&mrun)[kNC];
  const float4 (&u)[kNC][16];
  float4 y[kNC][2];
  __device__ __forceinline__ void operator()(int c, const Z4& zz, int st) {
    const int q = st >> 2, k = st & 3;
    if (q >= kNC) return;
    if (k < 2) {
      const float4 z = zz.z[q][k], v = u[q][2 * c + k];
      y[q][k] = make_float4(fmaxf(z.x + v.x, 0.0f), fmaxf(z.y + v.y, 0.0f), fmaxf(z.z + v.z, 0.0f),
                            fmaxf(z.w + v.w, 0.0f));
    } else if (k == 2) {
      mrun[q] = amax8(mrun[q], y[q][0], y[q][1]);
    } else {
      split8a(y[q][0], y[q][1], sc[q], oh[q][c], ol[q][c]);
    }
  }
};

template <int KBS, bool FOLD>
__global__ __attribute__((amdgpu_flat_work_group_size(kT4, kT4), amdgpu_waves_per_eu(kWPE, kWPE)))
void rad4_kernel(RadKArgs a) {
  constexpr int KF = FOLD ? 0 : 16;
  constexpr int K0 = KF + KBS;
  constexpr int C0 = chunk_bytes(K0), C16 = chunk_bytes(16);
  constexpr int CM = C0 > C16 ? C0 : C16;
  __shared__ __attribute__((aligned(16))) char smem[kRing * CM + (3 * 256 + 4) * 4];
  static_assert(kRing * CM + (3 * 256 + 4) * 4 <= 160 * 1024, "LDS budget");
  WStream4<CM> ws{smem, nullptr, 0, 0, 0};
  float* head = (float*)(smem + kRing * CM);
  const int lane = threadIdx.x & 63, wave = __builtin_amdgcn_readfirstlane(threadIdx.x >> 6);
  const int j = lane & 15, g = lane >> 4;
  const RadLayout& L = a.L;
  const char* W = a.packed;
  auto OP = [&](int i) {
    const char* w = FOLD && i == 0 ? a.r0_fold : W;
    asm volatile("" : "+s"(w));
    return FOLD && i == 0 ? w : w + L.op_off[i];
  };
  const bool view = L.view != 0;
  {
    const float* hsrc = (const float*)(W + L.head_off);
    for (int i = threadIdx.x; i < 3 * 256 + 4; i += kT4) head[i] = hsrc[i];
  }
  ws.template start<C0, C0>(OP(0), OP(0) + C0);
  Pend4 pd{};
  NoPre4 nopre;
  const int64_t Pn = a.P_dev ? min(a.P, (int64_t)*a.P_dev) : a.P;
  for (int64_t base = (int64_t)blockIdx.x * kPointsPerWG; base < Pn; base += (int64_t)gridDim.x * kPointsPerWG) {
    const bool has_next = base + (int64_t)gridDim.x * kPointsPerWG < Pn;
    const int64_t p0 = base + wave * 16 * kNC;
    f16x8 Uh[kNC][12], Ul[kNC][12], Vh[kNC][12], Vl[kNC][12];
    float m_in[kNC], xinv[kNC], mrun[kNC];
    float4 ufold[kNC][FOLD ? 16 : 1];
    float umax[kNC];
    bool valid[kNC];
#pragma unroll
    for (int q = 0; q < kNC; ++q) {
      const int64_t p = p0 + 16 * q + j;
      valid[q] = p < Pn;
      const int64_t pc = valid[q] ? p : Pn - 1;
      const int64_t pv = (pc / a.vdiv) % a.vmod;
      float xs[3], vs[3] = {0.f, 0.f, 0.f}, ns[3] = {0.f, 0.f, 0.f};
#pragma unroll
      for (int c = 0; c < 3; ++c) {
        xs[c] = a.x[pc * 3 + c];
        if (view) {
          vs[c] = a.vdir[pv * 3 + c];
          ns[c] = a.normals[pc * 3 + c];
        }
      }
      float4 X[K0];
      const int gq = (int)opaque_lane(g);
#pragma unroll
      for (int b = 0; b < KBS; ++b) {
        const int f = 16 * b + 4 * gq;
        X[KF + b] = make_float4(rad_small_feature(f, xs, vs, ns, a.nfreq_view, view),
                                rad_small_feature(f + 1, xs, vs, ns, a.nfreq_view, view),
                                rad_small_feature(f + 2, xs, vs, ns, a.nfreq_view, view),
                                rad_small_feature(f + 3, xs, vs, ns, a.nfreq_view, view));
      }
      if constexpr (FOLD) {
#pragma unroll
        for (int b = 0; b < 16; ++b) ufold[q][b] = *(const float4*)(a.feature + pc * 256 + 16 * b + 4 * g);
        float mu = 0.0f;
#pragma unroll
        for (int b = 0; b < 16; b += 2) mu = amax8(mu, ufold[q][b], ufold[q][b + 1]);
        umax[q] = max4_groups(mu);
      } else {
#pragma unroll
        for (int b = 0; b < 16; ++b) X[b] = *(const float4*)(a.feature + pc * 256 + 16 * b + 4 * g);
        umax[q] = 0.0f;
      }
      float m = 0.0f;
#pragma unroll
      for (int b = 0; b < K0; b += 2) m = amax8(m, X[b], X[b + 1]);
      m_in[q] = max4_groups(m);
      const float s = bound_scale(m_in[q]);
#pragma unroll
      for (int k = 0; k < K0 / 2; ++k) split8a(X[2 * k], X[2 * k + 1], s, Uh[q][k], Ul[q][k]);
      xinv[q] = 1.0f / s;
      mrun[q] = 0.0f;
    }
    auto next_scales = [&](int kb, float (&sc)[kNC]) {
      const float4 v = ws.buf()[2 * kb * 64 + 8];
#pragma unroll
      for (int q = 0; q < kNC; ++q) sc[q] = bound_scale(fmaf(v.y, m_in[q], v.z));
    };
    auto finish = [&](const float (&sc)[kNC]) {
#pragma unroll
      for (int q = 0; q < kNC; ++q) {
        m_in[q] = max4_groups(mrun[q]);
        mrun[q] = 0.0f;
        xinv[q] = 1.0f / sc[q];
      }
    };
    {
      float sc[kNC];
      if constexpr (FOLD) {
        const float4 v = ws.buf()[2 * K0 * 64 + 8];
#pragma unroll
// ... 1159 lines not shown
  for (int off = 32; off > 0; off >>= 1) {
    best = fmaxf(best, __shfl_xor(best, off));
    bb = fmaxf(bb, __shfl_xor(bb, off));
    m = fmaxf(m, __shfl_xor(m, off));
  }
  if (lane == 0) {
    red[0][wave] = m;
    red[1][wave] = best;
    red[2][wave] = bb;
  }
  __syncthreads();
  if (threadIdx.x == 0) {
    float a = 0.0f, b = 0.0f, c = 0.0f;
    for (int w = 0; w < 4; ++w) {
      a = fmaxf(a, red[0][w]);
      b = fmaxf(b, red[1][w]);
      c = fmaxf(c, red[2][w]);
    }
    if (op.prec == NR_PREC_F16X3) *op.wmax = a;
    if (op.bound) {
      op.bound[0] = b;
      op.bound[1] = c;
    }
  }
}

__global__ void pack_vec_kernel(const float* __restrict__ src, int off, int nvalid, int n, float* __restrict__ dst) {
  const int e = blockIdx.x * blockDim.x + threadIdx.x;
  if (e >= n) return;
  dst[e] = e < nvalid ? src[off + e] : 0.0f;
}

int launch_pack_ops(const PackOp* ops, char* const* dst, int nops, hipStream_t stream) {
  for (int b0 = 0; b0 < nops; b0 += kPackBatch) {
    const int nb = std::min(kPackBatch, nops - b0);
    PackBatch pb{};
    int64_t nmax = 0;
    for (int i = 0; i < nb; ++i) {
      const PackOp& op = ops[b0 + i];
      NR_REQUIRE(op.prec != NR_PREC_F16X3 || op.wmax, NR_ERR_ARG, "pack: f16x3 needs a max-|W| word");
      const int KB = op.in[0].nblk + op.in[1].nblk;
      const int NBO = op.out[0].nblk + op.out[1].nblk;
      pb.op[i] = op;
      pb.dst[i] = (uint32_t*)dst[b0 + i];
      pb.n[i] = (int64_t)(NBO / 2) * (2 * KB + 1) * 256;
      nmax = std::max(nmax, pb.n[i]);
    }
    int gmax = 1;
    for (int i = 0; i < nb; ++i)
      gmax = std::max(gmax, ((pb.op[i].out[0].nblk + pb.op[i].out[1].nblk) * 16 + kPackRowsPerWG - 1) / kPackRowsPerWG);
    NR_REQUIRE(gmax <= 32, NR_ERR_UNSUPPORTED, "pack: more than 512 output rows in one op");
    hipLaunchKernelGGL(pack_rows_kernel, dim3(gmax, nb), dim3(1024), 0, stream, pb);
    NR_HIP_CHECK(hipGetLastError());
    hipLaunchKernelGGL(pack_final_kernel, dim3(nb), dim3(256), 0, stream, pb);
    NR_HIP_CHECK(hipGetLastError());
    hipLaunchKernelGGL(pack_ops_kernel, dim3((unsigned)((nmax + 255) / 256), nb), dim3(256), 0, stream, pb);
    NR_HIP_CHECK(hipGetLastError());
  }
  return NR_OK;
}

int launch_pack_op(const PackOp& op, char* dst, hipStream_t stream) { return launch_pack_ops(&op, &dst, 1, stream); }

int launch_pack_vec(const float* src, int off, int nvalid, int n, char* dst, hipStream_t stream) {
  hipLaunchKernelGGL(pack_vec_kernel, dim3((n + 255) / 256), dim3(256), 0, stream, src, off, nvalid, n, (float*)dst);
  NR_HIP_CHECK(hipGetLastError());
  return NR_OK;
}

static int cu_count() {
  int dev = 0, cus = 256;
  if (hipGetDevice(&dev) == hipSuccess) (void)hipDeviceGetAttribute(&cus, hipDeviceAttributeMultiprocessorCount, dev);
  return cus;
}

static int grid_for(int64_t P, int ppw = kPointsPerWG) {
  const int cus = cu_count();
  const int64_t need = (P + ppw - 1) / ppw;
  return (int)(need < cus ? (need > 0 ? need : 1) : cus);
}

int launch_sdf(const SdfLayout& L, const void* packed, const float* pts, int64_t P, float* sdf, float* nabla,
               float* feature, int nfreq, void* ws, size_t ws_bytes, hipStream_t stream, const int* P_dev,
               int P_mult, const void* f8_alt) {
  if (P <= 0) return NR_OK;
  const int grid = grid_for(P);
  NR_REQUIRE(!f8_alt || (feature && L.prec == NR_PREC_F16X3 && !L.siren), NR_ERR_ARG,
             "sdf: an op in F8's place needs the f16x3 softplus net and a feature buffer");
  SdfKArgs a{(const char*)packed, L, pts, P, sdf, nabla, feature, (float4*)ws, nfreq, P_dev, P_mult, nullptr, nullptr,
             nullptr, (const char*)f8_alt};
  ProfScope prof(nabla ? (feature ? "sdf_nabla_feat" : "sdf_nabla") : (feature ? "sdf_feat" : "sdf_fwd"), (double)P,
                 stream, P_dev, P_mult);
  if (L.siren) {
    if (nabla) {
      const size_t need = (size_t)grid * kScratchPerWG;
      NR_REQUIRE(ws && ws_bytes >= need, NR_ERR_WORKSPACE, "sdf nabla workspace too small");
      if (L.prec == NR_PREC_F16X3)
        hipLaunchKernelGGL((siren_sdf_kernel<NR_PREC_F16X3, true>), dim3(grid), dim3(kThreads), 0, stream, a);
      else hipLaunchKernelGGL((siren_sdf_kernel<NR_PREC_FP32, true>), dim3(grid), dim3(kThreads), 0, stream, a);
    } else {
      if (L.prec == NR_PREC_F16X3)
        hipLaunchKernelGGL((siren_sdf_kernel<NR_PREC_F16X3, false>), dim3(grid), dim3(kThreads), 0, stream, a);
      else hipLaunchKernelGGL((siren_sdf_kernel<NR_PREC_FP32, false>), dim3(grid), dim3(kThreads), 0, stream, a);
    }
    NR_HIP_CHECK(hipGetLastError());
    return NR_OK;
  }
  if (nabla) {
    const size_t need = (size_t)grid * kScratchPerWG;
    NR_REQUIRE(ws && ws_bytes >= need, NR_ERR_WORKSPACE, "sdf nabla workspace too small");
    if (L.prec == NR_PREC_F16X3) {
      if (feature) hipLaunchKernelGGL((sdf4_kernel<true, true, 0>), dim3(grid), dim3(kT4), 0, stream, a);
      else hipLaunchKernelGGL((sdf4_kernel<true, false, 0>), dim3(grid), dim3(kT4), 0, stream, a);
    }
    else hipLaunchKernelGGL((sdf_kernel<NR_PREC_FP32, true>), dim3(grid), dim3(kThreads), 0, stream, a);
  } else {
    if (L.prec == NR_PREC_F16X3) {
      if (feature) hipLaunchKernelGGL((sdf4_kernel<false, true, 0>), dim3(grid), dim3(kT4), 0, stream, a);
      else if (P <= (int64_t)64 * cu_count())
        hipLaunchKernelGGL((sdf4_kernel<false, false, 3>), dim3(grid_for(P, 64)), dim3(256), 0, stream, a);
      else hipLaunchKernelGGL((sdf4_kernel<false, false, 0>), dim3(grid), dim3(kT4), 0, stream, a);
    }
    else hipLaunchKernelGGL((sdf_kernel<NR_PREC_FP32, false>), dim3(grid), dim3(kThreads), 0, stream, a);
  }
  NR_HIP_CHECK(hipGetLastError());
  return NR_OK;
}

int launch_sdf_deferred(const SdfLayout& L, const void* packed, const float* pts, int64_t P, float* sdf, float* nabla,
                        int nfreq, float4* slabs, const int* tiles, const int* n_tiles, int stage, hipStream_t stream) {
  if (P <= 0) return NR_OK;
  NR_REQUIRE(L.prec == NR_PREC_F16X3 && !L.siren, NR_ERR_UNSUPPORTED, "deferred nablas: f16x3 softplus nets");
  SdfKArgs a{(const char*)packed, L, pts, P, sdf, nabla, nullptr, nullptr, nfreq, nullptr, 0, slabs, tiles, n_tiles};
  if (stage == 1) {
    ProfScope prof("sdf_nabla_fwd", (double)P, stream);
    hipLaunchKernelGGL((sdf4_kernel<true, false, 1>), dim3(grid_for(P)), dim3(kT4), 0, stream, a);
  } else if (stage == 2) {
    ProfScope prof("sdf_nabla_bwd", (double)P, stream, n_tiles, 16);
    hipLaunchKernelGGL((sdf4_kernel<true, false, 2>), dim3(grid_for(P)), dim3(kT4), 0, stream, a);
  } else {
    NR_REQUIRE(stage == 4, NR_ERR_ARG, "deferred nablas: bad stage");
    ProfScope prof("sdf_nabla_bwd", (double)P, stream, n_tiles, 1);
    hipLaunchKernelGGL((sdf4_kernel<true, false, 4>), dim3(grid_for(P)), dim3(kT4), 0, stream, a);
  }
  NR_HIP_CHECK(hipGetLastError());
  return NR_OK;
}

int launch_nerf(const NerfLayout& L, const void* packed, const float* x4, const float* vdir, int64_t vdiv,
                int64_t vmod, int64_t P, float* sigma, float* rgb, hipStream_t stream, const int* P_dev) {
  if (P <= 0) return NR_OK;
  const int grid = grid_for(P);
  NerfKArgs a{(const char*)packed, L, x4, vdir, vdiv, vmod, P, sigma, rgb, P_dev};
  ProfScope prof("nerf", (double)P, stream, P_dev, 1);
  if (L.prec == NR_PREC_F16X3) hipLaunchKernelGGL(nerf4_kernel, dim3(grid), dim3(kT4), 0, stream, a);
  else hipLaunchKernelGGL((nerf_kernel<NR_PREC_FP32>), dim3(grid), dim3(kThreads), 0, stream, a);
  NR_HIP_CHECK(hipGetLastError());
  return NR_OK;
}

int launch_nerf_train32_fwd(const NerfLayout& L, const void* packed, const float* xe, const float* ve, int64_t P,
                            float* const* h, float* feat, float* hv, float* sigma, float* rgb, hipStream_t stream) {
  if (P <= 0) return NR_OK;
  NR_REQUIRE(L.prec == NR_PREC_FP32, NR_ERR_ARG, "nerf train forward: needs the fp32 render pack");
  NerfTrainFwdArgs a{};
  a.packed = (const char*)packed;
  a.L = L;
  a.xe = xe;
  a.ve = ve;
  a.P = P;
  for (int i = 0; i < 8; ++i) a.h[i] = h[i];
  a.feat = feat;
  a.hv = hv;
  a.sigma = sigma;
  a.rgb = rgb;
  ProfScope prof("nerf_train32_fwd", (double)P, stream);
  hipLaunchKernelGGL(nerf_train32_fwd_kernel, dim3(grid_for(P)), dim3(kThreads), 0, stream, a);
  NR_HIP_CHECK(hipGetLastError());
  return NR_OK;
}

int launch_nerf_train32_bwd(const NerfBwdLayout& B, const void* packed, const float* rgb, const float* hv,
                            const float* const* h, const float* g_rgb, const float* g_sigma, int64_t P, float* g3,
                            float* ghv, float* g_feat, float* const* gz, hipStream_t stream,
                            bool f16x3) {
  if (P <= 0) return NR_OK;
  NerfTrainBwdArgs a{};
  a.packed = (const char*)packed;
  a.B = B;
  a.rgb = rgb;
  a.hv = hv;
  for (int i = 0; i < 8; ++i) a.h[i] = h[i];
  a.g_rgb = g_rgb;
  a.g_sigma = g_sigma;
  a.P = P;
  a.g3 = g3;
  a.ghv = ghv;
  a.g_feat = g_feat;
  for (int i = 0; i < 8; ++i) a.gz[i] = gz[i];
  ProfScope prof("nerf_train32_bwd", (double)P, stream);
  if (f16x3) hipLaunchKernelGGL(nerf_train32_bwd_kernel<NR_PREC_F16X3>, dim3(grid_for(P)), dim3(kThreads), 0, stream, a);
  else hipLaunchKernelGGL(nerf_train32_bwd_kernel<NR_PREC_FP32>, dim3(grid_for(P)), dim3(kThreads), 0, stream, a);
  NR_HIP_CHECK(hipGetLastError());
  return NR_OK;
}

int launch_radiance_train32(const RadLayout& L, const void* packed, const float* feat, const float* small,
                            int64_t ld_small, int n_small, int64_t P, float* const* h, float* rgb, hipStream_t stream) {
  if (P <= 0) return NR_OK;
  if (L.prec != NR_PREC_FP32 || L.siren || L.D != 4 || (L.kbs != 2 && L.kbs != 4)) {
    set_error("nr_radiance_train_fwd32: needs the fp32 pack of a ReLU D=4 radiance net");
    return NR_ERR_UNSUPPORTED;
  }
  RadTrainArgs a{(const char*)packed, L, feat, small, ld_small, n_small, P, {h[0], h[1], h[2], h[3]}, rgb};
  ProfScope prof("radiance_train32", (double)P, stream);
  if (L.kbs == 2) hipLaunchKernelGGL((radiance_train32_kernel<2>), dim3(grid_for(P)), dim3(kThreads), 0, stream, a);
  else hipLaunchKernelGGL((radiance_train32_kernel<4>), dim3(grid_for(P)), dim3(kThreads), 0, stream, a);
  NR_HIP_CHECK(hipGetLastError());
  return NR_OK;
}

int launch_radiance(const RadLayout& L, const void* packed, const float* x, const float* vdir, int64_t vdiv,
                    int64_t vmod, const float* normals, const float* feature, int64_t P, float* rgb, int nfreq_view,
                    hipStream_t stream, const int* P_dev, const void* r0_fold) {
  if (P <= 0) return NR_OK;
  const int grid = grid_for(P);
  NR_REQUIRE(!r0_fold || (L.prec == NR_PREC_F16X3 && !L.siren && L.D == 4), NR_ERR_ARG,
             "radiance: the folded layer 0 needs the f16x3 ReLU D=4 net");
  RadKArgs a{(const char*)packed, L, x, vdir, vdiv, vmod, normals, feature, P, rgb, nfreq_view, P_dev,
             (const char*)r0_fold};
  ProfScope prof("radiance", (double)P, stream, P_dev, 1);
  const bool h3 = L.prec == NR_PREC_F16X3;
#define NR_RAD_LAUNCH(KBS, ACT, D)                                                                            \
  do {                                                                                                        \
    if (h3) hipLaunchKernelGGL((radiance_kernel<NR_PREC_F16X3, KBS, ACT, D>), dim3(grid), dim3(kThreads), 0, \
                               stream, a);                                                                    \
    else hipLaunchKernelGGL((radiance_kernel<NR_PREC_FP32, KBS, ACT, D>), dim3(grid), dim3(kThreads), 0,     \
                            stream, a);                                                                       \
  } while (0)
  if (L.kbs != 2 && L.kbs != 4) {
    set_error("radiance: unsupported small-input block count");
    return NR_ERR_UNSUPPORTED;
  }
  if (h3 && !L.siren && L.D == 4) {
    if (r0_fold) {
      if (L.kbs == 2) hipLaunchKernelGGL((rad4_kernel<2, true>), dim3(grid), dim3(kT4), 0, stream, a);
      else hipLaunchKernelGGL((rad4_kernel<4, true>), dim3(grid), dim3(kT4), 0, stream, a);
    } else if (L.kbs == 2) hipLaunchKernelGGL((rad4_kernel<2, false>), dim3(grid), dim3(kT4), 0, stream, a);
    else hipLaunchKernelGGL((rad4_kernel<4, false>), dim3(grid), dim3(kT4), 0, stream, a);
  } else if (!L.siren && L.D == 4) {
    if (L.kbs == 2) NR_RAD_LAUNCH(2, ACT_RELU, 4); else NR_RAD_LAUNCH(4, ACT_RELU, 4);
  } else if (!L.siren && L.D == 5) {
    if (L.kbs == 2) NR_RAD_LAUNCH(2, ACT_RELU, 5); else NR_RAD_LAUNCH(4, ACT_RELU, 5);
  } else if (L.D == 4) {
    if (L.kbs == 2) NR_RAD_LAUNCH(2, ACT_SINE, 4); else NR_RAD_LAUNCH(4, ACT_SINE, 4);
  } else {
    if (L.kbs == 2) NR_RAD_LAUNCH(2, ACT_SINE, 5); else NR_RAD_LAUNCH(4, ACT_SINE, 5);
  }
#undef NR_RAD_LAUNCH
  NR_HIP_CHECK(hipGetLastError());
  return NR_OK;
}

}

#ifdef NR_EXP_STAMPS
extern "C" int nr_exp_stamps(unsigned long long* out, int n) {
  return hipMemcpyFromSymbol(out, HIP_SYMBOL(nr::g_nr_stamps), sizeof(unsigned long long) * (size_t)n) == hipSuccess
             ? nr::kW4 * nr::kStampPh
             : -1;
}
#endif
```

### neurecon_amd/frameworks/neus.py

```python
import copy
import ctypes
import math
from collections import OrderedDict

import numpy as np
import torch
import torch.nn as nn
import torch.nn.functional as F

from .. import _lib as L
from ..base import ImplicitSurface, NeRF, RadianceNet, _no_training, check_view_dirs, wants_graph
from .. import rend_util


class NeuS(nn.Module):

    def __init__(self, variance_init=0.05, speed_factor=1.0, input_ch=3, W_geo_feat=-1, use_outside_nerf=False,
                 obj_bounding_radius=1.0, surface_cfg=dict(), radiance_cfg=dict()):
        super().__init__()
        self.ln_s = nn.Parameter(data=torch.Tensor([-np.log(variance_init) / speed_factor]), requires_grad=True)
        self.speed_factor = speed_factor
        self.implicit_surface = ImplicitSurface(W_geo_feat=W_geo_feat, input_ch=input_ch,
                                                obj_bounding_size=obj_bounding_radius, **surface_cfg)
        if W_geo_feat < 0:
# ... 29 lines not shown

def _neus_uniforms(B, N, batched, rayschunk, direct, n_iters, n_up, N_importance, N_outside, dev):
    pre = [B] if batched else []
    rd = 1 + len(pre) if not direct else len(pre)
    ups, outs = [], []
    for r0 in range(0, N, rayschunk):
        nc = min(rayschunk, N - r0)
        if direct:
            ups.append(rend_util.uniform([*pre, nc, N_importance], dev))
        elif n_iters > 0:
            ups.append(torch.stack([rend_util.uniform([*pre, nc, n_up], dev) for _ in range(n_iters)], 0))
        if N_outside > 0:
            outs.append(rend_util.to_device(rend_util.uniform([*pre, nc, N_outside]).float(), dev))
    u = None
    if ups:
        u = torch.cat(ups, rd)
        u = (u.reshape(B * N, N_importance) if direct else u.reshape(n_iters, B * N, n_up)).contiguous()
    t_out = torch.cat(outs, len(pre)).reshape(B * N, N_outside).contiguous() if outs else None
    return u, t_out


def volume_render(rays_o, rays_d, model, obj_bounding_radius=1.0, batched=False, batched_info={},
                  calc_normal=False, use_view_dirs=True, rayschunk=65536, netchunk=1048576, white_bkgd=False,
                  near_bypass=None, far_bypass=None, detailed_output=True, show_progress=False, perturb=False,
                  fixed_s_recp=1 / 64., N_samples=64, N_importance=64, N_outside=0,
                  upsample_algo='official_solution', N_nograd_samples=2048, N_upsample_iters=4,
                  skip_zero_alpha=True, defer_sample_nablas=True, max_workspace_gb=None, fold_feature=True,
                  **dummy_kwargs):
    L.require_gpu(rays_o, 'rays_o')
    if wants_graph(model):
        return _train_render(rays_o, rays_d, model, obj_bounding_radius=obj_bounding_radius, batched=batched,
                             calc_normal=calc_normal, use_view_dirs=use_view_dirs, rayschunk=rayschunk,
                             white_bkgd=white_bkgd, near_bypass=near_bypass, far_bypass=far_bypass,
                             detailed_output=detailed_output, perturb=perturb, fixed_s_recp=fixed_s_recp,
                             N_samples=N_samples, N_importance=N_importance, N_outside=N_outside,
                             upsample_algo=upsample_algo, N_nograd_samples=N_nograd_samples,
                             N_upsample_iters=N_upsample_iters)
    if upsample_algo not in L.UPSAMPLE:
        raise NotImplementedError(upsample_algo)
    direct = upsample_algo != 'official_solution'
    check_view_dirs(model, use_view_dirs)
    dev = rays_o.device
    if batched:
        B = rays_d.shape[0]
        prefix = [B, -1]
    else:
        prefix = [-1]
    ro = rays_o.reshape(-1, 3).float().contiguous()
    rd = rays_d.reshape(-1, 3).float().contiguous()
    n = ro.shape[0]
    if direct:
        n_up = N_importance
        S = N_samples + N_importance
    else:
        n_up = N_importance // N_upsample_iters if N_upsample_iters > 0 else 0
        S = N_samples + N_upsample_iters * n_up
    M = S - 1 + N_outside

    sdf_desc, sdf_packed = model.implicit_surface.nr_packed(dev)
    rad_desc, rad_packed = model.radiance_net.nr_packed(dev)
    s_dev = model.forward_s().detach().float().reshape(-1)[:1].contiguous()
    t_coarse = _linspace_table(N_samples, dev)
    u_fine = _linspace_table(max(n_up, 1), dev)

    rgb = torch.empty(n, 3, device=dev)
    depth = torch.empty(n, device=dev)
    acc = torch.empty(n, device=dev)
    normals = torch.empty(n, 3, device=dev) if calc_normal else None
    det = {}
    if detailed_output:
        det = dict(implicit_nablas=torch.empty(n, S, 3, device=dev), implicit_surface=torch.empty(n, S, device=dev),
                   radiance=torch.empty(n, M, 3, device=dev), alpha=torch.empty(n, M, device=dev),
                   cdf=torch.empty(n, S, device=dev), visibility_weights=torch.empty(n, M, device=dev),
                   d_final=torch.empty(n, M, device=dev))
        if N_outside > 0:
            det['sigma_out'] = torch.empty(n, M, device=dev)
            det['radiance_out'] = torch.empty(n, M, 3, device=dev)
    a = L.NrNeusArgs()
    a.rays_o, a.rays_d, a.n_rays = L.ptr(ro), L.ptr(rd), n
    a.sdf, a.sdf_packed = ctypes.pointer(sdf_desc), L.ptr(sdf_packed)
    a.rad, a.rad_packed = ctypes.pointer(rad_desc), L.ptr(rad_packed)
    fold_packed = model.radiance_net.nr_fold_packed(model.implicit_surface, dev) if fold_feature else None
    a.fold_packed = L.ptr(fold_packed)
    a.s, a.s_dev = 0.0, L.ptr(s_dev)
    a.no_mid_skip = 0 if skip_zero_alpha else 1
    a.no_defer = 0 if defer_sample_nablas else 1
    a.max_chunk_rays = int(rayschunk) if rayschunk else 0
    a.max_workspace_bytes = L.workspace_budget_bytes(max_workspace_gb)
    a.obj_bounding_radius = float(obj_bounding_radius)
    a.near_bypass = float('nan') if near_bypass is None else float(near_bypass)
    a.far_bypass = float('nan') if far_bypass is None else float(far_bypass)
    a.N_samples, a.N_importance, a.N_upsample_iters = N_samples, N_importance, N_upsample_iters
    a.calc_normal, a.white_bkgd = int(bool(calc_normal)), int(bool(white_bkgd))
    a.t_coarse, a.u_fine = L.ptr(t_coarse), L.ptr(u_fine)
    a.upsample_algo = L.UPSAMPLE[upsample_algo]
    a.fixed_s = 1. / fixed_s_recp
    if upsample_algo == 'direct_more':
        t_nograd = _linspace_table(N_nograd_samples, dev)
        a.N_nograd_samples, a.t_nograd = N_nograd_samples, L.ptr(t_nograd)
    a.rgb, a.depth, a.acc, a.normals = L.ptr(rgb), L.ptr(depth), L.ptr(acc), L.ptr(normals)
    a.d_final = L.ptr(det.get('d_final'))
    a.sdf_out = L.ptr(det.get('implicit_surface'))
    a.nablas_out = L.ptr(det.get('implicit_nablas'))
    a.radiance_out = L.ptr(det.get('radiance'))
    a.alpha_out = L.ptr(det.get('alpha'))
    a.cdf_out = L.ptr(det.get('cdf'))
    a.weights_out = L.ptr(det.get('visibility_weights'))
    if N_outside > 0:
        if not hasattr(model, 'nerf_outside'):
            raise ValueError('N_outside > 0 needs a model built with use_outside_nerf=True')
        nerf_desc, nerf_packed = model.nerf_outside.nr_packed(dev)
        t_out = _linspace_table(N_outside + 2, dev)
        a.nerf, a.nerf_packed = ctypes.pointer(nerf_desc), L.ptr(nerf_packed)
        a.N_outside, a.t_outside = N_outside, L.ptr(t_out)
        a.sigma_out, a.radiance_bg_out = L.ptr(det.get('sigma_out')), L.ptr(det.get('radiance_out'))
    if perturb:
        B = rays_d.shape[0] if batched else 1
        u_rand, t_out_rand = _neus_uniforms(B, n // B, batched, int(rayschunk), direct, N_upsample_iters, n_up,
                                            N_importance, N_outside, dev)
        a.u_rand, a.t_out_rand = L.ptr(u_rand), L.ptr(t_out_rand)
    lib = L.lib()
    ws_bytes = lib.nr_neus_workspace_bytes(ctypes.byref(a))
    ws = L.workspace(dev, ws_bytes)
    a.workspace, a.workspace_bytes = L.ptr(ws), ws_bytes
    L.check(lib.nr_neus_render(ctypes.byref(a), L.stream_of(dev)))

    ret = OrderedDict([('rgb', rgb.reshape(*prefix, 3)), ('depth_volume', depth.reshape(prefix)),
                       ('mask_volume', acc.reshape(prefix))])
    if calc_normal:
        ret['normals_volume'] = normals.reshape(*prefix, 3)
    if detailed_output:
        ret['implicit_nablas'] = det['implicit_nablas'].reshape(*prefix, S, 3)
        ret['implicit_surface'] = det['implicit_surface'].reshape(*prefix, S)
        ret['radiance'] = det['radiance'].reshape(*prefix, M, 3)
        ret['alpha'] = det['alpha'].reshape(*prefix, M)
        ret['cdf'] = det['cdf'].reshape(*prefix, S)
        ret['visibility_weights'] = det['visibility_weights'].reshape(*prefix, M)
        ret['d_final'] = det['d_final'].reshape(*prefix, M)
        if N_outside > 0:
            ret['sigma_out'] = det['sigma_out'].reshape(*prefix, M)
            ret['radiance_out'] = det['radiance_out'].reshape(*prefix, M, 3)
    return ret['rgb'], ret['depth_volume'], ret


def _sample_depths(ro, rd, model, dev, obj_bounding_radius, batched, B, rayschunk, near_bypass, far_bypass, perturb,
                   fixed_s_recp, N_samples, N_importance, upsample_algo, N_nograd_samples, N_upsample_iters,
                   N_outside=0):
    direct = upsample_algo != 'official_solution'
    n = ro.shape[0]
    n_up = N_importance if direct else (N_importance // N_upsample_iters if N_upsample_iters > 0 else 0)
    S = N_samples + (N_importance if direct else N_upsample_iters * n_up)
    sdf_desc, sdf_packed = model.implicit_surface.nr_packed(dev)
    rad_desc = model.radiance_net.nr_desc()
    d_all = torch.empty(n, S, device=dev)
    a = L.NrNeusArgs()
    a.rays_o, a.rays_d, a.n_rays = L.ptr(ro), L.ptr(rd), n
    a.sdf, a.sdf_packed = ctypes.pointer(sdf_desc), L.ptr(sdf_packed)
    a.rad, a.rad_packed = ctypes.pointer(rad_desc), None
    a.obj_bounding_radius = float(obj_bounding_radius)
    a.near_bypass = float('nan') if near_bypass is None else float(near_bypass)
    a.far_bypass = float('nan') if far_bypass is None else float(far_bypass)
    a.N_samples, a.N_importance, a.N_upsample_iters = N_samples, N_importance, N_upsample_iters
    t_coarse = _linspace_table(N_samples, dev)
    u_fine = _linspace_table(max(n_up, 1), dev)
    a.t_coarse, a.u_fine = L.ptr(t_coarse), L.ptr(u_fine)
    a.upsample_algo = L.UPSAMPLE[upsample_algo]
# ... 226 lines not shown
```

### neurecon_amd/frameworks/unisurf.py

```python
import copy
import ctypes
from collections import OrderedDict

import numpy as np
import torch
import torch.nn as nn
import torch.nn.functional as F

from .. import _lib as L
from .. import rend_util
from ..base import ImplicitSurface, RadianceNet, check_view_dirs, wants_graph
from .neus import _linspace_table

N_STEPS = 256
N_SECANT_STEPS = 8


class UNISURF(nn.Module):

    def __init__(self, input_ch=3, W_geo_feat=-1, surface_cfg=dict(), radiance_cfg=dict()):
        super().__init__()
        self.implicit_surface = ImplicitSurface(input_ch=input_ch, W_geo_feat=W_geo_feat, **surface_cfg)
        if W_geo_feat < 0:
            W_geo_feat = self.implicit_surface.W
        self.radiance_net = RadianceNet(W_geo_feat=W_geo_feat, **radiance_cfg)

    def forward(self, x, view_dirs):
        occ, nablas, geometry_feature = self.implicit_surface.forward_with_nablas(x)
        normals = F.normalize(nablas)
        radiances = self.radiance_net.forward(x, view_dirs, normals, geometry_feature)
        return radiances, occ, nablas

    @staticmethod
    def get_surface_from_opacity(opacity, eps=1e-4):
        if isinstance(opacity, torch.Tensor):
            opacity = torch.clamp(opacity, min=eps, max=1 - eps)
            imp_surface = torch.log(opacity / (1 - opacity))
        else:
            opacity = np.clip(opacity, a_min=eps, a_max=1 - eps)
            imp_surface = np.log(opacity / (1 - opacity))
        return (-1.) * imp_surface

    @staticmethod
    def get_opacity_from_surface(imp_surface):
        if isinstance(imp_surface, torch.Tensor):
            odds = torch.exp(-1. * imp_surface)
        else:
            odds = np.exp(-1. * imp_surface)
        return odds / (1 + odds)


def _unisurf_uniforms(B, N, batched, rayschunk, N_query, N_freespace, dev):
    pre = [B] if batched else []
    uq, uf = [], []
    for r0 in range(0, N, rayschunk):
        nc = min(rayschunk, N - r0)
        uq.append(rend_util.uniform([*pre, nc, N_query], dev))
        uf.append(rend_util.uniform([*pre, nc, N_freespace], dev))
    cat = lambda xs, k: torch.cat(xs, len(pre)).reshape(B * N, k).float().contiguous()
    return cat(uq, N_query), cat(uf, N_freespace)


def _window_reducer(window_ss, group=None):
    import torch.distributed as dist

    def cb(_user):
        try:
            dist.all_reduce(window_ss, op=dist.ReduceOp.SUM, group=group)
            return 0
        except Exception as e:
            print(f'neurecon_amd: window_reduce failed: {e!r}')
            return 1
    return L.WINDOW_REDUCE(cb)


def volume_render(rays_o, rays_d, model, batched=False, batched_info={}, calc_normal=False, logit_tau=0.0,
                  use_view_dirs=True, method='secant', rayschunk=65536, netchunk=1048576, white_bkgd=False,
                  near_bypass=None, far_bypass=None, detailed_output=True, show_progress=False,
                  radius_of_interest=4.0, perturb=False, interval=1.0, too_close_threshold=0.1, N_query=64,
                  N_freespace=32, shard=None, _sample_only=False, _full_march=False, **dummy_kwargs):
    L.require_gpu(rays_o, 'rays_o')
    if wants_graph(model) and not _sample_only:
        if shard is not None:
            raise NotImplementedError('neurecon_amd: a UNISURF training render runs on the whole batch per rank '
                                      '(DDP); shard= is for render-mode frame sharding')
        return _train_render(rays_o, rays_d, model, batched=batched, calc_normal=calc_normal, logit_tau=logit_tau,
                             use_view_dirs=use_view_dirs, method=method, rayschunk=rayschunk, netchunk=netchunk,
                             white_bkgd=white_bkgd, near_bypass=near_bypass, far_bypass=far_bypass,
                             detailed_output=detailed_output, radius_of_interest=radius_of_interest, perturb=perturb,
                             interval=interval, too_close_threshold=too_close_threshold, N_query=N_query,
                             N_freespace=N_freespace)
    check_view_dirs(model, use_view_dirs)
    dev = rays_o.device
    if batched:
        B, N = rays_d.shape[0], rays_d.reshape(rays_d.shape[0], -1, 3).shape[1]
        prefix = [B, -1]
    else:
        N = rays_d.reshape(-1, 3).shape[0]
        prefix = [-1]
    ro = rays_o.reshape(-1, 3).float().contiguous()
    rd = rays_d.reshape(-1, 3).float().contiguous()
    n = ro.shape[0]
    P = N_query + N_freespace

    sdf_desc, sdf_packed = model.implicit_surface.nr_packed(dev)
    rad_desc, rad_packed = model.radiance_net.nr_packed(dev)
    t_march = _linspace_table(N_STEPS, dev)
    t_query = _linspace_table(N_query + (1 if perturb else 0), dev)
    t_free = _linspace_table(N_freespace + (1 if perturb else 0), dev)

    rgb = torch.empty(n, 3, device=dev) if not _sample_only else None
    depth = torch.empty(n, device=dev) if not _sample_only else None
    acc = torch.empty(n, device=dev) if not _sample_only else None
    normals = torch.empty(n, 3, device=dev) if calc_normal and not _sample_only else None
    det = {}
    if _sample_only:
        det = dict(surface_points=torch.empty(n, 3, device=dev),
                   mask_surface=torch.empty(n, dtype=torch.bool, device=dev), depth_surface=torch.empty(n, device=dev),
                   d_all=torch.empty(n, P, device=dev))
    elif detailed_output:
        det = dict(surface_points=torch.empty(n, 3, device=dev), mask_surface=torch.empty(n, dtype=torch.bool,
                                                                                           device=dev),
                   depth_surface=torch.empty(n, device=dev), radiance=torch.empty(n, P, 3, device=dev),
                   implicit_surface=torch.empty(n, P, device=dev), implicit_nablas=torch.empty(n, P, 3, device=dev),
                   alpha=torch.empty(n, P, device=dev), visibility_weights=torch.empty(n, P, device=dev))
    a = L.NrUnisurfArgs()
    a.rays_o, a.rays_d, a.n_rays, a.rays_per_batch = L.ptr(ro), L.ptr(rd), n, N
    a.sdf, a.sdf_packed = ctypes.pointer(sdf_desc), L.ptr(sdf_packed)
    a.rad, a.rad_packed = ctypes.pointer(rad_desc), L.ptr(rad_packed)
    a.logit_tau = float(logit_tau)
    a.radius_of_interest, a.interval = float(radius_of_interest), float(interval)
    a.too_close_threshold = float(too_close_threshold)
    a.near_bypass = float('nan') if near_bypass is None else float(near_bypass)
    a.far_bypass = float('nan') if far_bypass is None else float(far_bypass)
    a.N_steps, a.N_secant_steps, a.N_query, a.N_freespace = N_STEPS, N_SECANT_STEPS, N_query, N_freespace
    a.no_secant = int(method != 'secant')
    a.normal_mode = 1 if batched else 0
    a.rayschunk, a.netchunk = int(rayschunk), int(netchunk)
    a.calc_normal, a.white_bkgd = int(bool(calc_normal)), int(bool(white_bkgd))
    a.full_march = int(bool(_full_march))
    a.t_march, a.t_query, a.t_free = L.ptr(t_march), L.ptr(t_query), L.ptr(t_free)
    a.rgb, a.depth, a.acc, a.normals = L.ptr(rgb), L.ptr(depth), L.ptr(acc), L.ptr(normals)
    a.surface_points = L.ptr(det.get('surface_points'))
    a.mask_surface = L.ptr(det.get('mask_surface'))
    a.depth_surface = L.ptr(det.get('depth_surface'))
    a.radiance_out = L.ptr(det.get('radiance'))
    a.sdf_out = L.ptr(det.get('implicit_surface'))
    a.nablas_out = L.ptr(det.get('implicit_nablas'))
    a.alpha_out = L.ptr(det.get('alpha'))
    a.weights_out = L.ptr(det.get('visibility_weights'))
    if _sample_only:
        a.d_all_out, a.sample_only = L.ptr(det['d_all']), 1
    if perturb:
        B = rays_d.shape[0] if batched else 1
        u_q, u_f = _unisurf_uniforms(B, n // B, batched, int(rayschunk), N_query, N_freespace, dev)
        a.u_query, a.u_free = L.ptr(u_q), L.ptr(u_f)
    lib = L.lib()
    keep = None
    if shard is not None and batched:
        ray0, row_rays, group = shard
        a.shard_ray0, a.shard_row_rays = int(ray0), int(row_rays)
        B = rays_d.shape[0]
        window_ss = torch.zeros(B, max(int(lib.nr_unisurf_window_count(ctypes.byref(a))), 1), 3,
                                dtype=torch.float64, device=dev)
        keep = _window_reducer(window_ss, group)
        a.window_ss, a.window_reduce = L.ptr(window_ss), ctypes.cast(keep, ctypes.c_void_p)
    ws_bytes = lib.nr_unisurf_workspace_bytes(ctypes.byref(a))
    if ws_bytes == 0:
        raise NotImplementedError('neurecon_amd: ' + lib.nr_last_error().decode())
    ws = L.workspace(dev, ws_bytes)
    a.workspace, a.workspace_bytes = L.ptr(ws), ws_bytes
    L.check(lib.nr_unisurf_render(ctypes.byref(a), L.stream_of(dev)))
    del keep
    if _sample_only:
        return det

    ret = OrderedDict([('rgb', rgb.reshape(*prefix, 3)), ('depth_volume', depth.reshape(prefix)),
                       ('mask_volume', acc.reshape(prefix))])
    if calc_normal:
        ret['normals_volume'] = normals.reshape(*prefix, 3)
    if detailed_output:
        ret['surface_points'] = det['surface_points'].reshape(*prefix, 3)
        ret['mask_surface'] = det['mask_surface'].reshape(prefix)
        ret['depth_surface'] = det['depth_surface'].reshape(prefix)
        ret['radiance'] = det['radiance'].reshape(*prefix, P, 3)
        ret['implicit_surface'] = det['implicit_surface'].reshape(*prefix, P)
        ret['implicit_nablas'] = det['implicit_nablas'].reshape(*prefix, P, 3)
        ret['alpha'] = det['alpha'].reshape(*prefix, P)
        ret['visibility_weights'] = det['visibility_weights'].reshape(*prefix, P)
    return ret['rgb'], ret['depth_volume'], ret


def _window_normalize(nab, batched, B, rayschunk, netchunk):
    if not batched:
        return F.normalize(nab, dim=-1)
    P = nab.shape[1]
    x = nab.reshape(B, -1, P, 3)
    outs = []
    for r0 in range(0, x.shape[1], rayschunk):
        seg = x[:, r0:r0 + rayschunk].reshape(B, -1, 3)
        parts = [F.normalize(seg[:, i:i + netchunk], dim=1) for i in range(0, seg.shape[1], netchunk)]
        outs.append(torch.cat(parts, 1).reshape(B, -1, P, 3))
    return torch.cat(outs, 1).reshape(-1, P, 3)


def _train_render(rays_o, rays_d, model, batched, calc_normal, logit_tau, use_view_dirs, method, rayschunk, netchunk,
                  white_bkgd, near_bypass, far_bypass, detailed_output, radius_of_interest, perturb, interval,
                  too_close_threshold, N_query, N_freespace):
    from .. import training as T
    check_view_dirs(model, use_view_dirs)
    dev = rays_o.device
    B = rays_d.shape[0] if batched else 1
# ... 139 lines not shown
```

### neurecon_amd/frameworks/volsdf.py

```python
import copy
import ctypes
from collections import OrderedDict

import numpy as np
import torch
import torch.nn as nn
import torch.nn.functional as F

from .. import _lib as L
from .. import rend_util
from ..base import ImplicitSurface, NeRF, RadianceNet, check_view_dirs, wants_graph
from .neus import _linspace_table


class VolSDF(nn.Module):

    def __init__(self, beta_init=0.1, speed_factor=1.0, input_ch=3, W_geo_feat=-1, obj_bounding_radius=3.0,
                 use_nerfplusplus=False, surface_cfg=dict(), radiance_cfg=dict()):
        super().__init__()
        self.speed_factor = speed_factor
        ln_beta_init = np.log(beta_init) / self.speed_factor
        self.ln_beta = nn.Parameter(data=torch.Tensor([ln_beta_init]), requires_grad=True)
        self.use_sphere_bg = not use_nerfplusplus
        self.obj_bounding_radius = obj_bounding_radius
        self.implicit_surface = ImplicitSurface(W_geo_feat=W_geo_feat, input_ch=input_ch,
                                                obj_bounding_size=obj_bounding_radius, **surface_cfg)
        if W_geo_feat < 0:
            W_geo_feat = self.implicit_surface.W
        self.radiance_net = RadianceNet(W_geo_feat=W_geo_feat, **radiance_cfg)
        if use_nerfplusplus:
            self.nerf_outside = NeRF(input_ch=4, multires=10, multires_view=4, use_view_dirs=True)

    def forward_ab(self):
        beta = torch.exp(self.ln_beta * self.speed_factor)
        return 1. / beta, beta

    def forward_surface(self, x):
        sdf = self.implicit_surface.forward(x)
        if self.use_sphere_bg:
            return torch.min(sdf, self.obj_bounding_radius - x.norm(dim=-1))
        return sdf

    def forward_surface_with_nablas(self, x):
        sdf, nablas, h = self.implicit_surface.forward_with_nablas(x)
        if self.use_sphere_bg:
            d_bg = self.obj_bounding_radius - x.norm(dim=-1)
            outside = d_bg < sdf
            sdf[outside] = d_bg[outside]
        return sdf, nablas, h

    def forward(self, x, view_dirs):
        sdf, nablas, geometry_feature = self.forward_surface_with_nablas(x)
        radiances = self.radiance_net.forward(x, view_dirs, nablas, geometry_feature)
        return radiances, sdf, nablas


def _host_ab(model):
    with torch.no_grad():
        beta = torch.exp(model.ln_beta.detach().float().cpu() * model.speed_factor)
        alpha = 1. / beta
    return float(alpha.reshape(-1)[0]), float(beta.reshape(-1)[0])


def _beta_plus_init(far, n_init, eps):
    far_t = far * torch.ones([1])
    return float(torch.sqrt((far_t ** 2) / (4 * (n_init - 1) * np.log(1 + eps))).reshape(-1)[0])


def _outside_radii(n, r, device):
    t = torch.linspace(0, 1, n + 2)[..., 1:-1].float()
    return (r / torch.flip(t, dims=[-1])).contiguous().to(device)


def _volsdf_uniforms(B, N, batched, rayschunk, N_importance, N_outside, dev):
    pre = [B] if batched else []
    uf, uo = [], []
    for r0 in range(0, N, rayschunk):
        nc = min(rayschunk, N - r0)
        uf.append(rend_util.uniform([(B if batched else 1) * nc, N_importance], dev).reshape(*pre, nc, N_importance))
        if N_outside > 0:
            uo.append(rend_util.uniform([*pre, nc, N_outside], dev))
    u_rand = rend_util.to_device(torch.cat(uf, len(pre)).reshape(-1, N_importance).float(), dev)
    u_rand = torch.sort(u_rand, dim=-1).values.contiguous()
    u_out = rend_util.to_device(torch.cat(uo, len(pre)).reshape(-1, N_outside).float(), dev).contiguous() if uo else None
    return u_rand, u_out


def volume_render(rays_o, rays_d, model, near=0.0, far=6.0, obj_bounding_radius=3.0, batched=False,
                  batched_info={}, calc_normal=False, use_view_dirs=True, rayschunk=65536, netchunk=1048576,
                  white_bkgd=False, use_nerfplusplus=False, detailed_output=True, show_progress=False,
                  perturb=False, N_samples=128, N_importance=64, N_outside=32, max_upsample_steps=5,
                  max_bisection_steps=10, epsilon=0.1, _uniforms=None, **dummy_kwargs):
    L.require_gpu(rays_o, 'rays_o')
    if wants_graph(model):
        return _train_render(rays_o, rays_d, model, near=near, far=far, obj_bounding_radius=obj_bounding_radius,
                             batched=batched, calc_normal=calc_normal, use_view_dirs=use_view_dirs, rayschunk=rayschunk,
                             white_bkgd=white_bkgd, use_nerfplusplus=use_nerfplusplus, detailed_output=detailed_output,
                             perturb=perturb, N_samples=N_samples, N_importance=N_importance, N_outside=N_outside,
                             max_upsample_steps=max_upsample_steps, max_bisection_steps=max_bisection_steps,
                             epsilon=epsilon)
    check_view_dirs(model, use_view_dirs)
    dev = rays_o.device
    prefix = [rays_d.shape[0], -1] if batched else [-1]
    ro = rays_o.reshape(-1, 3).float().contiguous()
    rd = rays_d.reshape(-1, 3).float().contiguous()
    n = ro.shape[0]
    S = N_samples + N_importance
    N0 = 4 * N_samples
    No = int(N_outside) if use_nerfplusplus else 0
    M = S + No

    sdf_desc, sdf_packed = model.implicit_surface.nr_packed(dev)
    rad_desc, rad_packed = model.radiance_net.nr_packed(dev)
    alpha_net, beta_net = _host_ab(model)
    t_coarse = _linspace_table(N_samples, dev)
    t_init = _linspace_table(N0, dev)
    u_up = _linspace_table(N0 + 2, dev)
    u_fine = _linspace_table(N_importance, dev)

    rgb = torch.empty(n, 3, device=dev)
    depth = torch.empty(n, device=dev)
    acc = torch.empty(n, device=dev)
    normals = torch.empty(n, 3, device=dev) if calc_normal else None
    det = {}
    if detailed_output:
        det = dict(implicit_surface=torch.empty(n, S, device=dev), implicit_nablas=torch.empty(n, S, 3, device=dev),
                   radiance=torch.empty(n, M, 3, device=dev), alpha=torch.empty(n, M - 1, device=dev),
                   p_i=torch.empty(n, M - 1, device=dev), visibility_weights=torch.empty(n, M - 1, device=dev),
                   d_vals=torch.empty(n, M, device=dev), sigma=torch.empty(n, M, device=dev),
                   beta_map=torch.empty(n, device=dev), iter_usage=torch.empty(n, device=dev))
        if No > 0:
            det['sigma_out'] = torch.empty(n, No, device=dev)
            det['radiance_out'] = torch.empty(n, No, 3, device=dev)
    a = L.NrVolsdfArgs()
    a.rays_o, a.rays_d, a.n_rays = L.ptr(ro), L.ptr(rd), n
    a.sdf, a.sdf_packed = ctypes.pointer(sdf_desc), L.ptr(sdf_packed)
    a.rad, a.rad_packed = ctypes.pointer(rad_desc), L.ptr(rad_packed)
    a.alpha_net, a.beta_net = alpha_net, beta_net
    a.beta_plus_init = _beta_plus_init(far, N0, epsilon) if No == 0 else 0.0
    if No > 0:
        nerf_desc, nerf_packed = model.nerf_outside.nr_packed(dev)
        a.N_outside = No
        a.nerf, a.nerf_packed = ctypes.pointer(nerf_desc), L.ptr(nerf_packed)
        rs_out = _outside_radii(No, float(obj_bounding_radius), dev)
        a.rs_out = L.ptr(rs_out)
        a.beta_plus_k = float(np.float32(4 * (N0 - 1) * np.log(1 + epsilon)))
    a.eps = float(epsilon)
    a.near, a.far = float(near), float(far)
    a.obj_bounding_radius = float(obj_bounding_radius) if No > 0 else float(model.obj_bounding_radius)
    a.use_sphere_bg = int(bool(model.use_sphere_bg))
    a.N_samples, a.N_importance = N_samples, N_importance
    a.max_upsample_steps, a.max_bisection_steps = max_upsample_steps, max_bisection_steps
    a.calc_normal, a.white_bkgd = int(bool(calc_normal)), int(bool(white_bkgd))
    a.t_coarse, a.t_init, a.u_up, a.u_fine = L.ptr(t_coarse), L.ptr(t_init), L.ptr(u_up), L.ptr(u_fine)
    a.rgb, a.depth, a.acc, a.normals = L.ptr(rgb), L.ptr(depth), L.ptr(acc), L.ptr(normals)
    a.d_vals = L.ptr(det.get('d_vals'))
    a.sdf_out = L.ptr(det.get('implicit_surface'))
    a.nablas_out = L.ptr(det.get('implicit_nablas'))
    a.radiance_out = L.ptr(det.get('radiance'))
    a.alpha_out = L.ptr(det.get('alpha'))
    a.p_out = L.ptr(det.get('p_i'))
    a.weights_out = L.ptr(det.get('visibility_weights'))
    a.sigma_out = L.ptr(det.get('sigma'))
    a.beta_map = L.ptr(det.get('beta_map'))
    a.iter_usage = L.ptr(det.get('iter_usage'))
    a.sigma_bg = L.ptr(det.get('sigma_out'))
    a.radiance_bg = L.ptr(det.get('radiance_out'))
    if perturb:
        if _uniforms is None:
            Bn = rays_d.shape[0] if batched else 1
            _uniforms = _volsdf_uniforms(Bn, n // Bn, batched, int(rayschunk), N_importance, No, dev)
        u_rand, u_out = _uniforms
        a.u_rand, a.u_out = L.ptr(u_rand), L.ptr(u_out)
    lib = L.lib()
    ws_bytes = lib.nr_volsdf_workspace_bytes(ctypes.byref(a))
    if ws_bytes == 0:
        raise NotImplementedError('neurecon_amd: ' + lib.nr_last_error().decode())
    ws = torch.empty(ws_bytes, dtype=torch.uint8, device=dev)
    a.workspace, a.workspace_bytes = L.ptr(ws), ws_bytes
    L.check(lib.nr_volsdf_render(ctypes.byref(a), L.stream_of(dev)))

    ret = OrderedDict([('rgb', rgb.reshape(*prefix, 3)), ('depth_volume', depth.reshape(prefix)),
                       ('mask_volume', acc.reshape(prefix))])
    if calc_normal:
        ret['normals_volume'] = normals.reshape(*prefix, 3)
    if detailed_output:
        ret['implicit_surface'] = det['implicit_surface'].reshape(*prefix, S)
        ret['implicit_nablas'] = det['implicit_nablas'].reshape(*prefix, S, 3)
        ret['radiance'] = det['radiance'].reshape(*prefix, M, 3)
        ret['alpha'] = det['alpha'].reshape(*prefix, M - 1)
        ret['p_i'] = det['p_i'].reshape(*prefix, M - 1)
        ret['visibility_weights'] = det['visibility_weights'].reshape(*prefix, M - 1)
        ret['d_vals'] = det['d_vals'].reshape(*prefix, M)
        ret['sigma'] = det['sigma'].reshape(*prefix, M)
        ret['beta_map'] = det['beta_map'].reshape(*prefix, 1)
        ret['iter_usage'] = det['iter_usage'].reshape(prefix)
        if No > 0:
            ret['sigma_out'] = det['sigma_out'].reshape(*prefix, No)
            ret['radiance_out'] = det['radiance_out'].reshape(*prefix, No, 3)
    return ret['rgb'], ret['depth_volume'], ret


def _train_render(rays_o, rays_d, model, near=0.0, far=6.0, obj_bounding_radius=3.0, batched=False, calc_normal=False,
                  use_view_dirs=True, rayschunk=65536, white_bkgd=False, use_nerfplusplus=False, detailed_output=True,
                  perturb=False, N_samples=128, N_importance=64, N_outside=32, max_upsample_steps=5,
                  max_bisection_steps=10, epsilon=0.1):
    from .. import training as T
    check_view_dirs(model, use_view_dirs)
    dev = rays_o.device
    prefix = [rays_d.shape[0], -1] if batched else [-1]
    No = int(N_outside) if use_nerfplusplus else 0
    ro = rays_o.reshape(-1, 3).float().contiguous()
    rd_raw = rays_d.reshape(-1, 3).float().contiguous()
    n = ro.shape[0]
    S = N_samples + N_importance
    uni = None
    if perturb:
        Bn = rays_d.shape[0] if batched else 1
        uni = _volsdf_uniforms(Bn, n // Bn, batched, int(rayschunk), N_importance, No, dev)
    with torch.no_grad():
# ... 172 lines not shown
```

Before: 718,000.

## Hand off SDF layer-7 activations and fold feature layer into radiance first layer

```diff
diff --git a/include/neurecon_hip.h b/include/neurecon_hip.h
--- a/include/neurecon_hip.h
+++ b/include/neurecon_hip.h
@@ -124,6 +124,7 @@
   int64_t max_chunk_rays;
   size_t max_workspace_bytes;
   const void* fold_packed;
+  int fold_h7;
 } NrNeusArgs;
 
 #define NR_DEFAULT_WORKSPACE_BYTES ((size_t)4 << 30)
@@ -138,6 +139,10 @@
 int nr_neus_fold_forward(const NrSdfDesc* sdf, const void* sdf_packed, const NrRadDesc* rad, const void* rad_packed,
                          const void* fold_packed, const float* pts, const float* vdir, int64_t vdir_div,
                          const float* normals, int64_t P, float* u, float* sdf_out, float* rgb, void* stream);
+int nr_fold_forward_h7(const NrSdfDesc* sdf, const void* sdf_packed, const NrRadDesc* rad, const void* rad_packed,
+                       const void* fold_packed, const float* pts, const float* vdir, int64_t vdir_div,
+                       const float* normals, int64_t P, const int* P_dev, float* sdf_out, float* nabla, float* h7,
+                       float* rgb, void* workspace, size_t workspace_bytes, void* stream);
 
 typedef struct {
   const float* rays_o;
@@ -184,6 +189,7 @@
   float* radiance_bg;
   const float* u_rand;
   const float* u_out;
+  const void* fold_packed;
 } NrVolsdfArgs;
 
 size_t nr_volsdf_workspace_bytes(const NrVolsdfArgs* a);
@@ -235,6 +241,7 @@
   float* d_all_out;
   int sample_only;
   int full_march;
+  const void* fold_packed;
 } NrUnisurfArgs;
 
 size_t nr_unisurf_workspace_bytes(const NrUnisurfArgs* a);
diff --git a/neurecon_amd/_lib.py b/neurecon_amd/_lib.py
--- a/neurecon_amd/_lib.py
+++ b/neurecon_amd/_lib.py
@@ -52,7 +52,7 @@
         ('workspace', _c_p), ('workspace_bytes', _c_sz),
         ('u_rand', _c_p), ('t_out_rand', _c_p), ('s_dev', _c_p), ('sample_only', _c_i), ('d_all_out', _c_p),
         ('no_mid_skip', _c_i), ('no_defer', _c_i), ('max_chunk_rays', _c_i64), ('max_workspace_bytes', _c_sz),
-        ('fold_packed', _c_p),
+        ('fold_packed', _c_p), ('fold_h7', _c_i),
     ]
 
 
@@ -73,6 +73,7 @@
         ('workspace', _c_p), ('workspace_bytes', _c_sz),
         ('N_outside', _c_i), ('nerf', ctypes.POINTER(NrNerfDesc)), ('nerf_packed', _c_p), ('rs_out', _c_p),
         ('beta_plus_k', _c_f), ('sigma_bg', _c_p), ('radiance_bg', _c_p), ('u_rand', _c_p), ('u_out', _c_p),
+        ('fold_packed', _c_p),
     ]
 
 
@@ -94,7 +95,7 @@
         ('u_query', _c_p), ('u_free', _c_p),
         ('shard_ray0', _c_i64), ('shard_row_rays', _c_i64), ('window_ss', _c_p), ('window_reduce', _c_p),
         ('window_user', _c_p), ('no_secant', _c_i), ('d_all_out', _c_p), ('sample_only', _c_i),
-        ('full_march', _c_i),
+        ('full_march', _c_i), ('fold_packed', _c_p),
     ]
 
 
@@ -176,6 +177,8 @@
                                  _c_p]),
     'nr_neus_fold_forward': (_c_i, [ctypes.POINTER(NrSdfDesc), _c_p, ctypes.POINTER(NrRadDesc), _c_p, _c_p, _c_p, _c_p,
                                     _c_i64, _c_p, _c_i64, _c_p, _c_p, _c_p, _c_p]),
+    'nr_fold_forward_h7': (_c_i, [ctypes.POINTER(NrSdfDesc), _c_p, ctypes.POINTER(NrRadDesc), _c_p, _c_p, _c_p, _c_p,
+                                  _c_i64, _c_p, _c_i64, _c_p, _c_p, _c_p, _c_p, _c_p, _c_p, _c_sz, _c_p]),
     'nr_volsdf_workspace_bytes': (_c_sz, [ctypes.POINTER(NrVolsdfArgs)]),
     'nr_volsdf_render': (_c_i, [ctypes.POINTER(NrVolsdfArgs), _c_p]),
     'nr_unisurf_workspace_bytes': (_c_sz, [ctypes.POINTER(NrUnisurfArgs)]),
diff --git a/neurecon_amd/csrc/nr_capi.hip b/neurecon_amd/csrc/nr_capi.hip
--- a/neurecon_amd/csrc/nr_capi.hip
+++ b/neurecon_amd/csrc/nr_capi.hip
@@ -117,12 +117,16 @@
   off += 8 * (size_t)chunk_bytes_host(16);
   F.r0_off = (uint32_t)off;
   off += 8 * (size_t)chunk_bytes_host(RL.kbs);
+  F.r0h_off = (uint32_t)off;
+  off += 8 * (size_t)chunk_bytes_host(16 + RL.kbs);
   F.scale_off = (uint32_t)off;
-  off = align256(off + 2 * 4);
+  off = align256(off + 3 * 4);
   F.bound_off = (uint32_t)off;
-  off = align256(off + 2 * 2 * 4);
+  off = align256(off + 3 * 2 * 4);
   F.u_off = (uint32_t)off;
   off = align256(off + (256 * 256 + 256) * 4);
+  F.w0h_off = (uint32_t)off;
+  off = align256(off + (size_t)256 * (RL.n_small + 256) * 4);
   F.total = (uint32_t)off;
   return F;
 }
@@ -330,17 +334,18 @@
   const int64_t Pm = (int64_t)(c.S - 1) * R;
   const char* f8p = nullptr;
   const char* r0p = nullptr;
+  const bool h7 = a.fold_packed && a.fold_h7;
   if (a.fold_packed) {
     const FoldLayout FL = fold_layout(RL);
-    f8p = (const char*)a.fold_packed + FL.f8_off;
-    r0p = (const char*)a.fold_packed + FL.r0_off;
+    f8p = h7 ? nullptr : (const char*)a.fold_packed + FL.f8_off;
+    r0p = (const char*)a.fold_packed + (h7 ? FL.r0h_off : FL.r0_off);
   }
   if (a.radiance_out || a.no_mid_skip) {
     if ((rc = launch_sdf(SL, a.sdf_packed, c.mids, Pm, c.sdf_m, c.nab_m, c.feat_m, a.sdf->multires, mlp_ws, mlp_bytes,
-                         st, nullptr, 0, f8p)))
+                         st, nullptr, 0, f8p, h7)))
       return rc;
     if ((rc = launch_radiance(RL, a.rad_packed, c.mids, c.rd, 1, R, c.nab_m, c.feat_m, Pm, c.rad_m,
-                              a.rad->multires_view, st, nullptr, r0p)))
+                              a.rad->multires_view, st, nullptr, r0p, h7)))
       return rc;
   } else {
     char* wsb = (char*)a.workspace;
@@ -355,10 +360,10 @@
                        slot, midc, vdc);
     NR_HIP_CHECK(hipGetLastError());
     if ((rc = launch_sdf(SL, a.sdf_packed, midc, Pm, c.sdf_m, c.nab_m, c.feat_m, a.sdf->multires, mlp_ws, mlp_bytes,
-                         st, cnt, 1, f8p)))
+                         st, cnt, 1, f8p, h7)))
       return rc;
     if ((rc = launch_radiance(RL, a.rad_packed, midc, vdc, 1, INT64_MAX, c.nab_m, c.feat_m, Pm, radc,
-                              a.rad->multires_view, st, cnt, r0p)))
+                              a.rad->multires_view, st, cnt, r0p, h7)))
       return rc;
     hipLaunchKernelGGL(neus_mid_scatter, g1, dim3(256), 0, st, slot, radc, Pm, c.rad_m);
     NR_HIP_CHECK(hipGetLastError());
@@ -525,11 +530,13 @@
   }
   NR_HIP_CHECK(hipGetLastError());
   const int64_t P = (int64_t)c.S * R;
+  const bool h7 = a.fold_packed != nullptr;
+  const char* r0h = h7 ? (const char*)a.fold_packed + fold_layout(RL).r0h_off : nullptr;
   if ((rc = launch_sdf(SL, a.sdf_packed, c.pts_f, P, c.sdf_f, c.nab_f, c.feat_f, a.sdf->multires, mlp_ws, mlp_bytes,
-                       st)))
+                       st, nullptr, 0, nullptr, h7)))
     return rc;
   if ((rc = launch_radiance(RL, a.rad_packed, c.pts_f, c.rd, c.S, INT64_MAX, c.nab_f, c.feat_f, P, c.rad_f,
-                            a.rad->multires_view, st)))
+                            a.rad->multires_view, st, nullptr, r0h, h7)))
     return rc;
   if (c.N_out > 0) {
     {
@@ -567,6 +574,8 @@
              "nr_volsdf_render: null argument");
   NR_REQUIRE(a->n_rays <= 0 || !a->calc_normal || a->normals, NR_ERR_ARG,
              "nr_volsdf_render: calc_normal needs normals output");
+  NR_REQUIRE(!a->fold_packed || fold_applies(*a->sdf, *a->rad), NR_ERR_ARG,
+             "nr_volsdf_render: a fold pack needs the f16x3 softplus SDF net and a f16x3 ReLU D=4 radiance net");
   NR_REQUIRE(a->N_samples >= 1 && a->N_importance >= 1 && a->max_upsample_steps >= 0 && a->max_bisection_steps >= 0,
              NR_ERR_ARG, "nr_volsdf_render: bad sample counts");
   NR_REQUIRE(4 * a->N_samples <= 1024 && a->N_importance <= 1024, NR_ERR_UNSUPPORTED,
@@ -649,8 +658,10 @@
     NR_HIP_CHECK(hipGetLastError());
   }
   if (a.sample_only) return NR_OK;
+  const bool h7 = a.fold_packed != nullptr;
+  const char* r0h = h7 ? (const char*)a.fold_packed + fold_layout(RL).r0h_off : nullptr;
   if ((rc = launch_sdf(SL, a.sdf_packed, c.pts_f, P, c.sdf_f, c.nab_f, c.feat_f, a.sdf->multires, mlp_ws, mlp_bytes,
-                       st)))
+                       st, nullptr, 0, nullptr, h7)))
     return rc;
   if (a.normal_mode == 1) {
     hipLaunchKernelGGL(uni_window_ss_part, dim3((unsigned)c.nw_row, (unsigned)(R / nloc), kWinSlices), dim3(256), 0,
@@ -666,7 +677,7 @@
   hipLaunchKernelGGL(uni_normalize, dim3((unsigned)((P + 255) / 256)), dim3(256), 0, st, c, a.normal_mode);
   NR_HIP_CHECK(hipGetLastError());
   if ((rc = launch_radiance(RL, a.rad_packed, c.pts_f, c.rd, 1, R, c.nrm_f, c.feat_f, P, c.rad_f,
-                            a.rad->multires_view, st)))
+                            a.rad->multires_view, st, nullptr, r0h, h7)))
     return rc;
   {
     ProfScope prof("unisurf_composite", (double)R, st);
@@ -681,6 +692,8 @@
   int rc = check_sdf_desc(a->sdf);
   if (rc) return rc;
   if ((rc = check_rad_desc(a->rad))) return rc;
+  NR_REQUIRE(!a->fold_packed || fold_applies(*a->sdf, *a->rad), NR_ERR_ARG,
+             "nr_unisurf_render: a fold pack needs the f16x3 softplus SDF net and a f16x3 ReLU D=4 radiance net");
   NR_REQUIRE(a->n_rays <= 0 || (a->rays_o && a->rays_d && (a->sample_only ? a->d_all_out != nullptr
                                                                             : (a->rgb && a->depth && a->acc))),
              NR_ERR_ARG, "nr_unisurf_render: null ray or output pointer");
@@ -1209,13 +1222,19 @@
   if ((rc = nr_gemm32(b8 + 1, 256, W0 + ns, ld0, 1, b0, bu, 256, 1, 256, 256, 0, stream))) return rc;
   float* wmax = (float*)(P + F.scale_off);
   float* bound = (float*)(P + F.bound_off);
-  PackOp ops[2];
+  float* W0h = (float*)(P + F.w0h_off);
+  NR_HIP_CHECK(hipMemcpyAsync(W0h, W0, (size_t)256 * ld0 * sizeof(float), hipMemcpyDeviceToDevice, st));
+  NR_HIP_CHECK(hipMemcpy2DAsync(W0h + ns, (size_t)ld0 * sizeof(float), U, 256 * sizeof(float), 256 * sizeof(float), 256,
+                                hipMemcpyDeviceToDevice, st));
+  PackOp ops[3];
   ops[0] = mkop(U, bu, 256, 256, 0, seg(16, 0, 256), none(), seg(16, 0, 256), none(), 1.0f, NR_PREC_F16X3, wmax);
   ops[1] = mkop(W0, nullptr, 256, ld0, 0, seg(16, 0, 256), none(), seg(RL.kbs, 0, ns), none(), 1.0f, NR_PREC_F16X3,
                 wmax + 1);
-  char* dst[2] = {P + F.f8_off, P + F.r0_off};
-  for (int i = 0; i < 2; ++i) ops[i].bound = bound + 2 * i;
-  return launch_pack_ops(ops, dst, 2, st);
+  ops[2] = mkop(W0h, bu, 256, ld0, 0, seg(16, 0, 256), none(), seg(16, ns, 256), seg(RL.kbs, 0, ns), 1.0f,
+                NR_PREC_F16X3, wmax + 2);
+  char* dst[3] = {P + F.f8_off, P + F.r0_off, P + F.r0h_off};
+  for (int i = 0; i < 3; ++i) ops[i].bound = bound + 2 * i;
+  return launch_pack_ops(ops, dst, 3, st);
 }
 
 int nr_neus_fold_forward(const NrSdfDesc* sd, const void* sdf_packed, const NrRadDesc* rd, const void* rad_packed,
@@ -1234,6 +1253,24 @@
     return rc;
   return launch_radiance(RL, rad_packed, pts, vdir, vdir_div, INT64_MAX, normals, u, P, rgb, rd->multires_view,
                          (hipStream_t)stream, nullptr, fp + F.r0_off);
+}
+
+int nr_fold_forward_h7(const NrSdfDesc* sd, const void* sdf_packed, const NrRadDesc* rd, const void* rad_packed,
+                       const void* fold_packed, const float* pts, const float* vdir, int64_t vdir_div,
+                       const float* normals, int64_t P, const int* P_dev, float* sdf_out, float* nabla, float* h7,
+                       float* rgb, void* workspace, size_t workspace_bytes, void* stream) {
+  int rc = check_fold(sd, rd);
+  if (rc) return rc;
+  NR_REQUIRE(sdf_packed && rad_packed && fold_packed && pts && (rd->no_view_dirs || (vdir && normals)) && sdf_out &&
+                 nabla && h7 && rgb && vdir_div > 0 && P >= 0,
+             NR_ERR_ARG, "nr_fold_forward_h7: bad argument");
+  const RadLayout RL = rad_layout(*rd);
+  const FoldLayout F = fold_layout(RL);
+  if ((rc = launch_sdf(sdf_layout(*sd), sdf_packed, pts, P, sdf_out, nabla, h7, sd->multires, workspace,
+                       workspace_bytes, (hipStream_t)stream, P_dev, 1, nullptr, true)))
+    return rc;
+  return launch_radiance(RL, rad_packed, pts, vdir, vdir_div, INT64_MAX, normals, h7, P, rgb, rd->multires_view,
+                         (hipStream_t)stream, P_dev, (const char*)fold_packed + F.r0h_off, true);
 }
 
 size_t nr_volsdf_workspace_bytes(const NrVolsdfArgs* a) {
diff --git a/neurecon_amd/csrc/nr_mlp.h b/neurecon_amd/csrc/nr_mlp.h
--- a/neurecon_amd/csrc/nr_mlp.h
+++ b/neurecon_amd/csrc/nr_mlp.h
@@ -111,7 +111,8 @@
 int launch_sdf(const SdfLayout& L, const void* packed, const float* pts, int64_t P, float* sdf, float* nabla,
                float* feature, int nfreq, void* ws, size_t ws_bytes, hipStream_t stream,
                const int* P_dev = nullptr, int P_mult = 0,
-               const void* f8_alt = nullptr);
+               const void* f8_alt = nullptr,
+               bool h7_out = false);
 int launch_sdf_deferred(const SdfLayout& L, const void* packed, const float* pts, int64_t P, float* sdf, float* nabla,
                         int nfreq, float4* slabs, const int* tiles, const int* n_tiles, int stage, hipStream_t stream);
 int launch_nerf(const NerfLayout& L, const void* packed, const float* x4, const float* vdir, int64_t vdiv,
@@ -120,13 +121,15 @@
 int launch_radiance(const RadLayout& L, const void* packed, const float* x, const float* vdir, int64_t vdiv,
                     int64_t vmod, const float* normals, const float* feature, int64_t P, float* rgb, int nfreq_view,
                     hipStream_t stream, const int* P_dev = nullptr,
-                    const void* r0_fold = nullptr);
+                    const void* r0_fold = nullptr,
+                    bool r0_full = false);
 
 struct FoldLayout {
-  uint32_t f8_off, r0_off;
+  uint32_t f8_off, r0_off, r0h_off;
   uint32_t scale_off;
   uint32_t bound_off;
   uint32_t u_off;
+  uint32_t w0h_off;
   uint32_t total;
   int kbs;
 };
diff --git a/neurecon_amd/csrc/nr_mlp.hip b/neurecon_amd/csrc/nr_mlp.hip
--- a/neurecon_amd/csrc/nr_mlp.hip
+++ b/neurecon_amd/csrc/nr_mlp.hip
@@ -741,6 +741,29 @@
     n = cnt;
     nt = nontemporal;
     b96 = bytes96;
+  }
+};
+struct Pend4H : Pend4 {
+  float4* base2;
+  bool nt2;
+  __device__ __forceinline__ int flush() {
+    int issued = 0;
+    if (base2) {
+#pragma unroll
+      for (int i = 2; i < 4; ++i) {
+        const uint32_t off = o[i] * 16u;
+        const f32x4 d = tof(v[i]);
+        if (nt2) asm volatile("global_store_dwordx4 %0, %1, %2 nt\n\ts_nop 1" : : "v"(off), "v"(d), "s"(base2) : "memory");
+        else asm volatile("global_store_dwordx4 %0, %1, %2\n\ts_nop 1" : : "v"(off), "v"(d), "s"(base2) : "memory");
+      }
+      issued = 2;
+      base2 = nullptr;
+    }
+    return issued + Pend4::flush();
+  }
+  __device__ __forceinline__ void put2(float4* b2, bool nontemporal) {
+    base2 = b2;
+    nt2 = nontemporal;
   }
 };
 
@@ -945,9 +968,9 @@
 #define NR_STAMP(var)
 #endif
 
-template <int KB, int NBO, int NXT_CB, bool AUX, bool TS, class WS, class Pre, class Epi>
+template <int KB, int NBO, int NXT_CB, bool AUX, bool TS, class WS, class PD, class Pre, class Epi>
 __device__ __forceinline__ void op4(WS& ws, const char* __restrict__ op, const char* nxt, const f16x8 (&bh)[kNC][12],
-                                    const f16x8 (&bl)[kNC][12], const float (&xinv)[kNC], Pend4& pd, Pre&& pre,
+                                    const f16x8 (&bl)[kNC][12], const float (&xinv)[kNC], PD& pd, Pre&& pre,
                                     Epi&& epi, int lane) {
   constexpr int CB = chunk_bytes(KB);
   constexpr int NCH = NBO / 2;
@@ -1128,17 +1151,24 @@
   }
 };
 
-template <bool NABLA, bool FEAT>
+struct H7Rows {
+  float4* hb;
+  uint32_t hrow;
+};
+struct NoRows {};
+template <bool NABLA, bool FEAT, bool H7 = false>
 struct F7Epi4 {
+  static_assert(!H7 || (NABLA && !FEAT && kNC == 1), "h7 hand-off: nabla launch without F8, slots 2..3 free");
   f16x8 (&oh)[kNC][12];
   f16x8 (&ol)[kNC][12];
   const float (&sc)[kNC];
   float4* g7;
   float (&mrun)[kNC];
   float (&sdf_part)[kNC];
-  Pend4& pd;
+  std::conditional_t<H7, Pend4H, Pend4>& pd;
   int lane;
   float4 y[kNC][2], s[kNC][2];
+  std::conditional_t<H7, H7Rows, NoRows> h;
   __device__ __forceinline__ void operator()(int c, const Z4& zz, int st) {
     const int q = st >> 2, k = st & 3;
     if (q < kNC) sp_pair<NABLA>(zz, q, k, y[q], s[q][0], s[q][1]);
@@ -1158,9 +1188,21 @@
         mrun[q] = amax8(mrun[q], y[q][0], y[q][1]);
         split8a(y[q][0], y[q][1], sc[q], oh[q][c], ol[q][c]);
       }
+      if constexpr (H7) {
+        pd.v[2] = y[q][0];
+        pd.v[3] = y[q][1];
+      }
     }
     if constexpr (NABLA)
-      if (st == 7) pend_chunk(pd, g7, 2 * c, lane, kFeatNT);
+      if (st == 7) {
+        pend_chunk(pd, g7, 2 * c, lane, kFeatNT);
+        if constexpr (H7) {
+          const uint32_t r = opaque_lane(h.hrow * 64 + (lane >> 4));
+          pd.o[2] = r + (2 * c) * 4;
+          pd.o[3] = r + (2 * c + 1) * 4;
+          pd.put2(h.hb, kFeatNT);
+        }
+      }
   }
 };
 
@@ -1205,7 +1247,7 @@
   __device__ __forceinline__ int operator()(int) const { return 0; }
 };
 
-template <bool NABLA, bool FEAT, int STAGE_>
+template <bool NABLA, bool FEAT, int STAGE_, bool H7 = false>
 __global__ __attribute__((amdgpu_flat_work_group_size(STAGE_ == 3 ? 256 : kT4, STAGE_ == 3 ? 256 : kT4),
                           amdgpu_waves_per_eu(kWPE, kWPE)))
 void sdf4_kernel(SdfKArgs a) {
@@ -1214,6 +1256,7 @@
   constexpr int NW = STAGE_ == 3 ? 4 : kW4;
   static_assert(STAGE_ != 3 || (!NABLA && !FEAT), "narrow tiles: forward-only launches");
   static_assert(STAGE == 0 || (NABLA && !FEAT), "deferred nablas: no feature");
+  static_assert(!H7 || (NABLA && !FEAT && STAGE_ == 0), "h7 hand-off: the nabla launch without F8");
   constexpr int PPW = 16 * kNC * NW;
   constexpr int CB = chunk_bytes(18);
   constexpr int C16 = chunk_bytes(16), C4 = chunk_bytes(4), C14 = chunk_bytes(14), C18 = chunk_bytes(18);
@@ -1251,7 +1294,7 @@
   if constexpr (STAGE == 2) ws.template start<C16, C16>(OP(B7), OP(B7) + C16);
   else if constexpr (RING == 4) ws.template start<C4, C4, C4>(OP(F0), OP(F0) + C4, OP(F0) + 2 * C4);
   else ws.template start<C4, C4>(OP(F0), OP(F0) + C4);
-  Pend4 pd{};
+  std::conditional_t<H7, Pend4H, Pend4> pd{};
   NoPre4 nopre;
   const float kSpSlack = 0.0070f;
 
@@ -1421,7 +1464,12 @@
     {
       float sc[kNC];
       next_scales(16, kSpSlack, zero2, sc);
-      F7Epi4<NABLA, FEAT> epi{Uh, Ul, sc, slab(7), mrun, sdf_part, pd, lane};
+      F7Epi4<NABLA, FEAT, H7> epi{Uh, Ul, sc, slab(7), mrun, sdf_part, pd, lane};
+      if constexpr (H7) {
+        const int64_t pf = p0 < Pn ? p0 : Pn - 1;
+        epi.h.hb = uniform_ptr((float4*)(a.feature + pf * 256));
+        epi.h.hrow = (uint32_t)(pq[0] - pf);
+      }
       constexpr int NXT = ((NABLA && STAGE == 0) || FEAT) ? C16 : C4;
       const char* n;
       if constexpr (FEAT) n = OPF8();
@@ -1926,9 +1974,10 @@
   const RadLayout& L = a.L;
   const char* W = a.packed;
   auto OP = [&](int i) {
-    const char* w = FOLD && i == 0 ? a.r0_fold : W;
+    const bool alt = i == 0 && (FOLD || a.r0_fold != nullptr);
+    const char* w = alt ? a.r0_fold : W;
     asm volatile("" : "+s"(w));
-    return FOLD && i == 0 ? w : w + L.op_off[i];
+    return alt ? w : w + L.op_off[i];
   };
   const bool view = L.view != 0;
   {
@@ -3254,11 +3303,13 @@
 
 int launch_sdf(const SdfLayout& L, const void* packed, const float* pts, int64_t P, float* sdf, float* nabla,
                float* feature, int nfreq, void* ws, size_t ws_bytes, hipStream_t stream, const int* P_dev,
-               int P_mult, const void* f8_alt) {
+               int P_mult, const void* f8_alt, bool h7_out) {
   if (P <= 0) return NR_OK;
   const int grid = grid_for(P);
   NR_REQUIRE(!f8_alt || (feature && L.prec == NR_PREC_F16X3 && !L.siren), NR_ERR_ARG,
              "sdf: an op in F8's place needs the f16x3 softplus net and a feature buffer");
+  NR_REQUIRE(!h7_out || (feature && nabla && !f8_alt && L.prec == NR_PREC_F16X3 && !L.siren), NR_ERR_ARG,
+             "sdf: the h7 hand-off needs the f16x3 softplus net, nablas, a feature buffer and no op in F8's place");
   SdfKArgs a{(const char*)packed, L, pts, P, sdf, nabla, feature, (float4*)ws, nfreq, P_dev, P_mult, nullptr, nullptr,
              nullptr, (const char*)f8_alt};
   ProfScope prof(nabla ? (feature ? "sdf_nabla_feat" : "sdf_nabla") : (feature ? "sdf_feat" : "sdf_fwd"), (double)P,
@@ -3282,7 +3333,8 @@
     const size_t need = (size_t)grid * kScratchPerWG;
     NR_REQUIRE(ws && ws_bytes >= need, NR_ERR_WORKSPACE, "sdf nabla workspace too small");
     if (L.prec == NR_PREC_F16X3) {
-      if (feature) hipLaunchKernelGGL((sdf4_kernel<true, true, 0>), dim3(grid), dim3(kT4), 0, stream, a);
+      if (h7_out) hipLaunchKernelGGL((sdf4_kernel<true, false, 0, true>), dim3(grid), dim3(kT4), 0, stream, a);
+      else if (feature) hipLaunchKernelGGL((sdf4_kernel<true, true, 0>), dim3(grid), dim3(kT4), 0, stream, a);
       else hipLaunchKernelGGL((sdf4_kernel<true, false, 0>), dim3(grid), dim3(kT4), 0, stream, a);
     }
     else hipLaunchKernelGGL((sdf_kernel<NR_PREC_FP32, true>), dim3(grid), dim3(kThreads), 0, stream, a);
@@ -3394,7 +3446,7 @@
 
 int launch_radiance(const RadLayout& L, const void* packed, const float* x, const float* vdir, int64_t vdiv,
                     int64_t vmod, const float* normals, const float* feature, int64_t P, float* rgb, int nfreq_view,
-                    hipStream_t stream, const int* P_dev, const void* r0_fold) {
+                    hipStream_t stream, const int* P_dev, const void* r0_fold, bool r0_full) {
   if (P <= 0) return NR_OK;
   const int grid = grid_for(P);
   NR_REQUIRE(!r0_fold || (L.prec == NR_PREC_F16X3 && !L.siren && L.D == 4), NR_ERR_ARG,
@@ -3415,7 +3467,7 @@
     return NR_ERR_UNSUPPORTED;
   }
   if (h3 && !L.siren && L.D == 4) {
-    if (r0_fold) {
+    if (r0_fold && !r0_full) {
       if (L.kbs == 2) hipLaunchKernelGGL((rad4_kernel<2, true>), dim3(grid), dim3(kT4), 0, stream, a);
       else hipLaunchKernelGGL((rad4_kernel<4, true>), dim3(grid), dim3(kT4), 0, stream, a);
     } else if (L.kbs == 2) hipLaunchKernelGGL((rad4_kernel<2, false>), dim3(grid), dim3(kT4), 0, stream, a);
diff --git a/neurecon_amd/frameworks/neus.py b/neurecon_amd/frameworks/neus.py
--- a/neurecon_amd/frameworks/neus.py
+++ b/neurecon_amd/frameworks/neus.py
@@ -135,6 +135,7 @@
     a.rad, a.rad_packed = ctypes.pointer(rad_desc), L.ptr(rad_packed)
     fold_packed = model.radiance_net.nr_fold_packed(model.implicit_surface, dev) if fold_feature else None
     a.fold_packed = L.ptr(fold_packed)
+    a.fold_h7 = 0 if fold_feature == 'u' else 1
     a.s, a.s_dev = 0.0, L.ptr(s_dev)
     a.no_mid_skip = 0 if skip_zero_alpha else 1
     a.no_defer = 0 if defer_sample_nablas else 1
diff --git a/neurecon_amd/frameworks/unisurf.py b/neurecon_amd/frameworks/unisurf.py
--- a/neurecon_amd/frameworks/unisurf.py
+++ b/neurecon_amd/frameworks/unisurf.py
@@ -78,7 +78,8 @@
                   use_view_dirs=True, method='secant', rayschunk=65536, netchunk=1048576, white_bkgd=False,
                   near_bypass=None, far_bypass=None, detailed_output=True, show_progress=False,
                   radius_of_interest=4.0, perturb=False, interval=1.0, too_close_threshold=0.1, N_query=64,
-                  N_freespace=32, shard=None, _sample_only=False, _full_march=False, **dummy_kwargs):
+                  N_freespace=32, shard=None, _sample_only=False, _full_march=False, fold_feature=True,
+                  **dummy_kwargs):
     L.require_gpu(rays_o, 'rays_o')
     if wants_graph(model) and not _sample_only:
         if shard is not None:
@@ -128,6 +129,10 @@
     a.rays_o, a.rays_d, a.n_rays, a.rays_per_batch = L.ptr(ro), L.ptr(rd), n, N
     a.sdf, a.sdf_packed = ctypes.pointer(sdf_desc), L.ptr(sdf_packed)
     a.rad, a.rad_packed = ctypes.pointer(rad_desc), L.ptr(rad_packed)
+    fold_packed = None
+    if fold_feature and not _sample_only:
+        fold_packed = model.radiance_net.nr_fold_packed(model.implicit_surface, dev)
+    a.fold_packed = L.ptr(fold_packed)
     a.logit_tau = float(logit_tau)
     a.radius_of_interest, a.interval = float(radius_of_interest), float(interval)
     a.too_close_threshold = float(too_close_threshold)
diff --git a/neurecon_amd/frameworks/volsdf.py b/neurecon_amd/frameworks/volsdf.py
--- a/neurecon_amd/frameworks/volsdf.py
+++ b/neurecon_amd/frameworks/volsdf.py
@@ -90,7 +90,7 @@
                   batched_info={}, calc_normal=False, use_view_dirs=True, rayschunk=65536, netchunk=1048576,
                   white_bkgd=False, use_nerfplusplus=False, detailed_output=True, show_progress=False,
                   perturb=False, N_samples=128, N_importance=64, N_outside=32, max_upsample_steps=5,
-                  max_bisection_steps=10, epsilon=0.1, _uniforms=None, **dummy_kwargs):
+                  max_bisection_steps=10, epsilon=0.1, _uniforms=None, fold_feature=True, **dummy_kwargs):
     L.require_gpu(rays_o, 'rays_o')
     if wants_graph(model):
         return _train_render(rays_o, rays_d, model, near=near, far=far, obj_bounding_radius=obj_bounding_radius,
@@ -136,6 +136,8 @@
     a.rays_o, a.rays_d, a.n_rays = L.ptr(ro), L.ptr(rd), n
     a.sdf, a.sdf_packed = ctypes.pointer(sdf_desc), L.ptr(sdf_packed)
     a.rad, a.rad_packed = ctypes.pointer(rad_desc), L.ptr(rad_packed)
+    fold_packed = model.radiance_net.nr_fold_packed(model.implicit_surface, dev) if fold_feature else None
+    a.fold_packed = L.ptr(fold_packed)
     a.alpha_net, a.beta_net = alpha_net, beta_net
     a.beta_plus_init = _beta_plus_init(far, N0, epsilon) if No == 0 else 0.0
     if No > 0:
```

Measured after the change: 720,600 (median of 6 runs). No clear change (+0.4%).
